# real-stanford/dgdm

Hardware: AMD Instinct MI355X
Metric: guided samples/sec (full DDIM chain) (higher is better)
Workload: dtype f32_split_f16x3; 1 GPU; 3d_guided BASELINE configs[2] (configs[3] at 8 GPUs): B=32 G=45 P=5 R=36000 sub_bs=512 N=512 T=15/S=5, fresh object per pair; contraction_flag=f32, fingers_per_pair=32, denoise_steps=5, rows_per_cond_fn=36000, cond_fn_per_chain_step=1, eps_net_form=f32_f16x3 batched, parallelism=pairs-sharded x1

## Files before the change

dgdm_amd/csrc/debug.hip:

```cpp
#include "common.h"
#include "mfma_chain.h"
#include "models.h"
#include "smallnet.h"

namespace dgdm {
__global__ __launch_bounds__(64, 1) void debug_chain_kernel(const float4 *__restrict__ Wimg, const float *__restrict__ bias,
                                                           const float *__restrict__ X, float *__restrict__ Y) {
    const int lane = threadIdx.x & 63, n = lane & 31, h4 = (lane >> 5) * 4;
    f32x16 in[8], out[8];
#pragma unroll
    for (int o = 0; o < 8; ++o)
#pragma unroll
        for (int q = 0; q < 4; ++q) {
            const float4 v = feat4(X + n * 256, o, q, h4);
            in[o][4 * q + 0] = v.x; in[o][4 * q + 1] = v.y; in[o][4 * q + 2] = v.z; in[o][4 * q + 3] = v.w;
        }
    chain_layer<8, 8, CHAIN_BIAS>(Wimg, bias, in, out, lane);
#pragma unroll
    for (int o = 0; o < 8; ++o)
#pragma unroll
        for (int q = 0; q < 4; ++q) {
            float4 v;
            v.x = out[o][4 * q + 0]; v.y = out[o][4 * q + 1]; v.z = out[o][4 * q + 2]; v.w = out[o][4 * q + 3];
            *reinterpret_cast<float4 *>(Y + n * 256 + 32 * o + 8 * q + h4) = v;
        }
}
}

extern "C" int dgdm_debug_chain_layer(const float *W_host, const float *bias_host, const float *X_dev, float *Y_dev, void *stream) {
    using namespace dgdm;
    std::vector<float> img = pack_chain(W_host, 256, 256);
    DevBuf dw, db;
    int rc;
    if ((rc = dw.upload(img.data(), img.size() * 4)) || (rc = db.upload(bias_host, 256 * 4))) return rc;
    hipLaunchKernelGGL(debug_chain_kernel, dim3(1), dim3(64), 0, (hipStream_t)stream, dw.as<float4>(), db.as<float>(), X_dev, Y_dev);
    DGDM_HIP_CHECK(hipGetLastError());
    DGDM_HIP_CHECK(hipStreamSynchronize((hipStream_t)stream));
    return DGDM_OK;
}

extern "C" int dgdm_debug_pointnet_indices(DgdmDynamics *m, const float *xyz_dev, int N, const int32_t *perm_dev, int perm_len,
                                           int32_t *fps512_dev, int32_t *fps128_dev, int32_t *fps128_flags_dev, int32_t *ball1_dev,
                                           int32_t *ball2_dev, int32_t *ball2_count_dev, int32_t *crowded_dev, void *stream) {
    using namespace dgdm;
    DGDM_REQUIRE(m && xyz_dev && perm_dev && fps512_dev && fps128_dev && fps128_flags_dev && ball1_dev && ball2_dev && ball2_count_dev && crowded_dev,
                 DGDM_EINVAL, "dgdm_debug_pointnet_indices: null argument");
    if (m->kind != 3) { set_error("model type not supported: PointNet++ belongs to the 3-D model"); return DGDM_EMODE; }
    DGDM_REQUIRE(N >= 128 && N <= 1024 && perm_len > 0 && perm_len <= N, DGDM_EINVAL, "dgdm_debug_pointnet_indices: N %d / perm_len %d unsupported", N, perm_len);
    hipStream_t s = (hipStream_t)stream;
    int rc;
    if ((rc = pn_fps_table(xyz_dev, N, N, 512, fps512_dev, nullptr, s))) return rc;
    if ((rc = pn_fps_table(xyz_dev, N, N, 128, fps128_dev, fps128_flags_dev, s))) return rc;
    return pn_debug_indices(xyz_dev, N, m->pn(), perm_dev, perm_len, ball1_dev, ball2_dev, ball2_count_dev, crowded_dev, s);
}

extern "C" int dgdm_farthest_point_sample(const float *xyz_dev, const int64_t *start_host, int B, int N, int npoint, int32_t *out_dev, void *stream) {
    using namespace dgdm;
    DGDM_REQUIRE(xyz_dev && start_host && out_dev && B >= 0 && npoint > 0, DGDM_EINVAL, "dgdm_farthest_point_sample: bad argument");
    DGDM_REQUIRE(N > 0 && N <= 1024, DGDM_EINVAL, "clouds of %d points unsupported (1..1024)", N);
    if (B == 0) return DGDM_OK;
    std::vector<int> st(B);
    for (int i = 0; i < B; ++i) {
        DGDM_REQUIRE(start_host[i] >= 0 && start_host[i] < N, DGDM_EINVAL, "FPS start %lld outside [0, %d)", (long long)start_host[i], N);
        st[i] = (int)start_host[i];
    }
    DevBuf d;
    int rc;
    if ((rc = d.upload(st.data(), sizeof(int) * B))) return rc;
    if ((rc = pn_fps_rows(xyz_dev, d.as<int>(), B, N, npoint, out_dev, (hipStream_t)stream))) return rc;
    DGDM_HIP_CHECK(hipStreamSynchronize((hipStream_t)stream));
    return DGDM_OK;
}

extern "C" int dgdm_query_ball_point(float radius_squared, int nsample, const float *xyz_dev, const float *new_xyz_dev, int B, int N, int S, int32_t *out_dev,
                                     void *stream) {
    using namespace dgdm;
    DGDM_REQUIRE(xyz_dev && new_xyz_dev && out_dev && B >= 0 && N > 0 && S >= 0 && nsample > 0, DGDM_EINVAL, "dgdm_query_ball_point: bad argument");
    if (B == 0 || S == 0) return DGDM_OK;
    return pn_ball_rows(xyz_dev, new_xyz_dev, B, N, S, radius_squared, nsample, out_dev, (hipStream_t)stream);
}

extern "C" int dgdm_square_distance(const float *src_dev, const float *dst_dev, int B, int S, int N, float *out_dev, void *stream) {
    using namespace dgdm;
    DGDM_REQUIRE(src_dev && dst_dev && out_dev && B >= 0 && S >= 0 && N >= 0, DGDM_EINVAL, "dgdm_square_distance: bad argument");
    if (B == 0 || S == 0 || N == 0) return DGDM_OK;
    return pn_sqdist_rows(src_dev, dst_dev, B, S, N, out_dev, (hipStream_t)stream);
}

extern "C" int dgdm_index_points(const float *points_dev, const int32_t *idx_dev, int B, int N, int M, int C, float *out_dev, void *stream) {
    using namespace dgdm;
    DGDM_REQUIRE(points_dev && idx_dev && out_dev && B >= 0 && N > 0 && M >= 0 && C > 0, DGDM_EINVAL, "dgdm_index_points: bad argument");
    if (B == 0 || M == 0) return DGDM_OK;
    return pn_index_rows(points_dev, idx_dev, B, N, M, C, out_dev, (hipStream_t)stream);
}


namespace dgdm {
__global__ void group_max_kernel(const float *__restrict__ x, int64_t G, int ns, int C, float *__restrict__ out) {
    const int64_t e = (int64_t)blockIdx.x * blockDim.x + threadIdx.x;
    if (e >= G * C) return;
    const int64_t g = e / C;
    const int c = (int)(e - g * C);
    const float *p = x + g * ns * C + c;
    float best = p[0];
    for (int n = 1; n < ns; ++n) best = fmaxf(best, p[(int64_t)n * C]);
    out[e] = best;
}
}

extern "C" int dgdm_linear_act(const float *x_dev, int ldx, const float *wt_dev, const float *bias_dev, float *y_dev, int ldy, int rows, int K, int N, int act,
                               void *stream) {
    using namespace dgdm;
    DGDM_REQUIRE(x_dev && wt_dev && y_dev && rows >= 0 && K > 0 && N > 0 && ldx >= K && ldy >= N, DGDM_EINVAL, "dgdm_linear_act: bad argument");
    DGDM_REQUIRE(act == ACT_NONE || act == ACT_RELU || act == ACT_SILU, DGDM_EINVAL, "dgdm_linear_act: activation %d", act);
    return linear(x_dev, ldx, wt_dev, bias_dev, nullptr, 1, y_dev, ldy, rows, K, N, act, false, (hipStream_t)stream);
}

extern "C" int dgdm_group_max(const float *x_dev, int64_t groups, int nsample, int C, float *out_dev, void *stream) {
    using namespace dgdm;
    DGDM_REQUIRE(x_dev && out_dev && groups >= 0 && nsample > 0 && C > 0, DGDM_EINVAL, "dgdm_group_max: bad argument");
    if (groups == 0) return DGDM_OK;
    hipLaunchKernelGGL(group_max_kernel, dim3((unsigned)((groups * C + 255) / 256)), dim3(256), 0, (hipStream_t)stream, x_dev, groups, nsample, C, out_dev);
    DGDM_HIP_CHECK(hipGetLastError());
    return DGDM_OK;
}
```

dgdm_amd/csrc/guidance_api.hip:

```cpp
#include "common.h"
#include "models.h"
#include <algorithm>
#include <cstring>
#include <unordered_map>
#include <atomic>
#include <thread>

using namespace dgdm;

namespace {

std::vector<float> linspace_f32(float start, float end, int steps) {
    std::vector<float> v(steps);
    if (steps == 1) { v[0] = start; return v; }
    const float step = (end - start) / (float)(steps - 1);
    const int half = steps / 2;
    for (int i = 0; i < steps; ++i) v[i] = i < half ? start + step * (float)i : end - step * (float)(steps - i - 1);
    return v;
}

struct ObjectTables {
    const float *xyz = nullptr;
    const int   *fps1 = nullptr;
    const int   *fps2 = nullptr;
    const int   *flags = nullptr;
    DevBuf Z;
    bool   fast_ok = false;
    int *crowded = nullptr, *clist = nullptr;
    DevBuf M0, cl2, cnt2;
    DevBuf cl2s;
    DevBuf cl2o;
    DevBuf pcf;
    DevBuf X, X16;
    bool   has_x = false, has_x16 = false;
    int    ncr = 0;
    DevBuf Z16, M0_16;
    bool   has16 = false;
};

struct PoseGrid {
    DevBuf tab, tiled;
    DevBuf pmax;
    int cells = 0, tiles_per_b = 0;
    int64_t rows = 0;
};

}

struct DgdmGuidance {
    DgdmDynamics *m = nullptr;
    DgdmGuidanceConfig cfg{};
    int B = 0;
    PoseGrid grid, sweep;
    DevBuf objpart;
    DevBuf objtmp;
    std::vector<std::unique_ptr<ObjectTables>> tables;
    bool bf16 = false;
    bool f32_mfma = false;
    static constexpr int NBUILD = 3;
    DevBuf pool_crowded, pool_clist, pool_off, pool_pairs, pool_rank, pool_F1, pool_U;
    DevBuf pool_xyz, pool_fps1, pool_fps2, pool_flags, pool_ncr;
    DevBuf tmpY[NBUILD], tmpL2[NBUILD], vlist;
    hipStream_t bstream[NBUILD] = {}, fstream = nullptr;
    hipEvent_t bev[NBUILD] = {}, bstart = nullptr, fstart = nullptr, fdone = nullptr, ldone = nullptr;
    DevBuf V, genc, atab, chainbias, timepart, ttmp, ttmp64, partial, objdev, objidx, xobj, xobj16, starts, order, xchains, todo, groupoff;
    DevBuf loopx[2], loopeps, loopgrad, loopxrep, loopts;
    DevBuf scorelogits;
    DevBuf sweep_ori, rollstate, rolllogits, rolltiles, rollpmax;
    int rolltiles_chains = 0;
    DevBuf xidx, xidxchains, xtabptrs;
    bool xtab_enabled = true;
    int xtab_policy = 0;
    int grads_since_set = 0;
    static constexpr int XTAB_AFTER = 5;
    int l2_gather_mode = 0;
    int xobj_mode = 0;
    int n_objects = 0;
    bool force_slow_xobj = false;
    void *pinned = nullptr; size_t pinned_bytes = 0; hipEvent_t pinned_ev = nullptr;
    int64_t todo_capacity = 0;
    int *ro_host = nullptr; size_t ro_ints = 0; hipEvent_t ro_ev = nullptr; bool ro_pending = false;
    int finish_objects();
    hipStream_t cstream = nullptr; hipEvent_t up_ready = nullptr, up_consumed = nullptr; bool consumed_recorded = false;
    ~DgdmGuidance() {
        if (pinned) (void)hipHostFree(pinned);
        if (pinned_ev) (void)hipEventDestroy(pinned_ev);
        if (ro_host) (void)hipHostFree(ro_host);
        if (ro_ev) (void)hipEventDestroy(ro_ev);
        if (cstream) (void)hipStreamDestroy(cstream);
        if (up_ready) (void)hipEventDestroy(up_ready);
        if (up_consumed) (void)hipEventDestroy(up_consumed);
        for (int i = 0; i < NBUILD; ++i) {
            if (bstream[i]) (void)hipStreamDestroy(bstream[i]);
            if (bev[i]) (void)hipEventDestroy(bev[i]);
        }
        if (bstart) (void)hipEventDestroy(bstart);
        if (ldone) (void)hipEventDestroy(ldone);
        if (fstart) (void)hipEventDestroy(fstart);
        if (fdone) (void)hipEventDestroy(fdone);
        if (fstream) (void)hipStreamDestroy(fstream);
    }
    int build_pose_table(const std::vector<float> &ori, const std::vector<float> &pos, PoseGrid *dst, hipStream_t s);
    void set_grid(dgdm::TrunkParams *p, const PoseGrid &g, int n_chains) const;
    int check_objects(const int *oidx, int n_chains) const;
    bool tables_wanted() const { return xtab_enabled && !force_slow_xobj && xobj_mode == 0; }
    int common_pre(const float *x_dev, float t_scaled, const int *objidx_host, int n_chains, hipStream_t s);
    int upload_starts(const int64_t *starts_host, int n_chains, int64_t rows, hipStream_t s, bool need_order = true, int n_calls = 1,
                      int64_t call_stride = 0);
    int ensure_rows(int n_chains, int64_t rows_per_chain);
    int use_xtab(const int *objidx_host, int n_chains, int64_t rows, bool want16, hipStream_t s);
    int build_object(int oi, int slot, hipStream_t s);
    int build_xtab(int oi, hipStream_t s);
    int run_xobj(const int *objidx_host, int n_chains, int64_t rows, bool want16, bool *used16, hipStream_t s);
    struct Embedded {
        bool tab = false, used16 = false;
        int64_t rows_per_chain = 0;
        void point(dgdm::TrunkParams *p, const DgdmGuidance &g, int call, int64_t rows_per_call) const;
    };
    int embed_rows(const int *objidx_host, int n_chains, const int64_t *starts_host, int64_t rows_per_call, int n_calls, int64_t call_stride,
                   bool want16, Embedded *e, hipStream_t s);
    int embed(const int *objidx_host, int n_chains, const int64_t *starts_host, int n_calls, int64_t call_stride, Embedded *e, hipStream_t s);
    int trunk_front(int kind, const float *x_dev, int timestep, const int *objidx_host, const int64_t *starts_host, int n_chains, const Embedded *emb,
                    int call, dgdm::TrunkParams *p, hipStream_t s);
};

int DgdmGuidance::build_pose_table(const std::vector<float> &ori, const std::vector<float> &pos, PoseGrid *dst, hipStream_t s) {
    const int n = (int)ori.size(), W1 = m->W1;
    dst->cells = n; dst->tiles_per_b = (n + 31) / 32; dst->rows = (int64_t)B * n;
    DevBuf d_ori, d_pos, d_emb;
    int rc;
    if ((rc = d_ori.upload(ori.data(), sizeof(float) * n))) return rc;
    if ((rc = d_pos.upload(pos.data(), sizeof(float) * 2 * n))) return rc;
    if ((rc = d_emb.alloc(sizeof(float) * 27 * n))) return rc;
    if ((rc = dst->tab.alloc(sizeof(float) * (size_t)W1 * n))) return rc;
    if ((rc = pose_embed(d_ori.as<float>(), d_pos.as<float>(), d_emb.as<float>(), n, s))) return rc;
    if ((rc = linear64(d_emb.as<float>(), nullptr, 27, m->blob64.at(m->off64.w1p_wt), nullptr, nullptr, 1, nullptr, dst->tab.as<float>(), W1, n, 27, W1, ACT_NONE, s))) return rc;
    if ((rc = dst->tiled.alloc(sizeof(float) * (size_t)W1 * dst->tiles_per_b * 32))) return rc;
    if ((rc = tile_table(dst->tab.as<float>(), n, W1, dst->tiled.as<float>(), s))) return rc;
    DGDM_HIP_CHECK(hipStreamSynchronize(s));
    return DGDM_OK;
}

void DgdmGuidance::set_grid(TrunkParams *p, const PoseGrid &g, int n_chains) const {
    p->Atab = atab.as<float>(); p->Ptab = g.tab.as<float>(); p->PtabT = g.tiled.as<float>(); p->Pmax = g.pmax.as<float>();
    p->B = B; p->C = g.cells; p->tiles_per_b = g.tiles_per_b; p->ntiles = n_chains * B * g.tiles_per_b; p->R = g.rows;
    p->xstride = g.rows;
}

int DgdmGuidance::check_objects(const int *oidx, int n_chains) const {
    DGDM_REQUIRE(n_objects > 0, DGDM_EINVAL, "dgdm_guidance_set_objects has not been called");
    for (int i = 0; i < n_chains; ++i)
        DGDM_REQUIRE(oidx[i] >= 0 && oidx[i] < n_objects, DGDM_EINVAL, "chain %d refers to object %d of %d", i, oidx[i], n_objects);
    return DGDM_OK;
}

extern "C" int dgdm_guidance_create(DgdmGuidance **out, DgdmDynamics *model, const DgdmGuidanceConfig *cfg) {
    DGDM_REQUIRE(out && model && cfg, DGDM_EINVAL, "dgdm_guidance_create: null argument");
    DGDM_REQUIRE(cfg->batch > 0 && cfg->grid_size > 0 && cfg->num_pos > 0 && cfg->max_chains > 0 && cfg->num_train_timesteps > 0,
                 DGDM_EINVAL, "dgdm_guidance_create: bad config");
    DGDM_REQUIRE(cfg->max_chains <= DGDM_MAX_CHAINS, DGDM_EINVAL, "max_chains %d > %d", cfg->max_chains, DGDM_MAX_CHAINS);
    if (model->kind == 3) {
        DGDM_REQUIRE(cfg->sub_batch_size > 0, DGDM_EINVAL, "3-D guidance needs sub_batch_size (it partitions the FPS start draws)");
        DGDM_REQUIRE(cfg->num_object_points > 0 && cfg->num_object_points <= 1024, DGDM_EINVAL, "object clouds of %d points unsupported (1..1024)", cfg->num_object_points);
    } else {
        DGDM_REQUIRE(2 * cfg->num_object_points == model->object_ch, DGDM_EINVAL, "2*num_object_points (%d) != object_ch (%d)", 2 * cfg->num_object_points, model->object_ch);
    }
    std::unique_ptr<DgdmGuidance> g(new DgdmGuidance());
    g->m = model; g->cfg = *cfg;
    g->B = cfg->batch;
    const int G = cfg->grid_size, P = cfg->num_pos, C = G * P * P;
    const std::vector<float> lo = linspace_f32(cfg->ori_lo, cfg->ori_hi, G), lp = linspace_f32(-1.f, 1.f, P);
    std::vector<float> ori(C), pos(2 * (size_t)C);
    for (int gi = 0; gi < G; ++gi)
        for (int a = 0; a < P; ++a)
            for (int b = 0; b < P; ++b) {
                const int c = (gi * P + a) * P + b;
                ori[c] = lo[gi]; pos[2 * c] = lp[a]; pos[2 * c + 1] = lp[b];
            }
    int rc;
    if ((rc = g->build_pose_table(ori, pos, &g->grid, nullptr))) return rc;
    {
        std::vector<float> tab((size_t)C * model->W1), mx(C, 0.f);
        DGDM_HIP_CHECK(hipMemcpy(tab.data(), g->grid.tab.p, tab.size() * sizeof(float), hipMemcpyDeviceToHost));
        for (int c = 0; c < C; ++c)
            for (int j = 0; j < model->W1; ++j) mx[c] = std::max(mx[c], std::fabs(tab[(size_t)c * model->W1 + j]));
        if ((rc = g->grid.pmax.upload(mx.data(), mx.size() * sizeof(float)))) return rc;
    }
    std::vector<float> pos0(2 * (size_t)G, 0.f);
    if ((rc = g->build_pose_table(lo, pos0, &g->sweep, nullptr))) return rc;
    if ((rc = g->sweep_ori.upload(lo.data(), lo.size() * sizeof(float)))) return rc;
    const int W1 = model->W1, nc = cfg->max_chains;
    const size_t rows = (size_t)nc * g->B;
    const int64_t R = g->grid.rows;
    if ((rc = g->V.alloc(rows * 256 * 8)) || (rc = g->genc.alloc(rows * 256 * 8)) || (rc = g->atab.alloc(rows * W1 * 4)) ||
        (rc = g->chainbias.alloc((size_t)nc * W1 * 8)) || (rc = g->timepart.alloc((size_t)W1 * 8)) || (rc = g->ttmp.alloc(768 * 4)) ||
        (rc = g->ttmp64.alloc(512 * 8)) ||
        (rc = g->partial.alloc(rows * g->grid.tiles_per_b * W1 * 4)) || (rc = g->objdev.alloc(sizeof(TrunkObjective) * nc)) ||
        (rc = g->objidx.alloc(sizeof(int) * nc)))
        return rc;
    if (model->kind == 2) {
        if ((rc = g->objpart.alloc((size_t)std::max(1, cfg->max_objects) * W1 * 8))) return rc;
    } else {
        if ((rc = g->starts.alloc((size_t)nc * R * 2 * sizeof(int))) ||
            (rc = g->order.alloc((size_t)nc * R * sizeof(int))) || (rc = g->xchains.alloc(sizeof(XobjChain) * nc)) ||
            (rc = g->todo.alloc(((size_t)nc * R + 1) * sizeof(int))))
            return rc;
        g->todo_capacity = (int64_t)nc * R;
        g->pinned_bytes = ((size_t)nc * R * 3 + (size_t)nc * (cfg->num_object_points + 1)) * sizeof(int);
        if ((rc = g->groupoff.alloc((size_t)nc * (cfg->num_object_points + 1) * sizeof(int))) || (rc = g->xidx.alloc((size_t)nc * R * sizeof(int))) ||
            (rc = g->xidxchains.alloc(sizeof(XidxChain) * nc)) || (rc = g->xtabptrs.alloc(sizeof(void *) * nc)))
            return rc;
        DGDM_HIP_CHECK(hipHostMalloc(&g->pinned, g->pinned_bytes, hipHostMallocDefault));
        DGDM_HIP_CHECK(hipEventCreateWithFlags(&g->pinned_ev, hipEventDisableTiming));
    }
    *out = g.release();
    return DGDM_OK;
}

extern "C" void dgdm_guidance_destroy(DgdmGuidance *g) { delete g; }

extern "C" int dgdm_guidance_set_contraction_dtype(DgdmGuidance *g, int dtype) {
    DGDM_REQUIRE(g, DGDM_EINVAL, "dgdm_guidance_set_contraction_dtype: null handle");
    DGDM_REQUIRE(dtype >= DGDM_DTYPE_F32 && dtype <= DGDM_DTYPE_F32_F16X3, DGDM_EINVAL,
                 "contraction dtype %d unsupported (0 = f32 (default form), 1 = bf16, 2 = f32 on the float32 MFMA, 3 = f32 as 3 f16 products = the default form)", dtype);
    g->bf16 = dtype == DGDM_DTYPE_BF16;
    g->f32_mfma = dtype == DGDM_DTYPE_F32_MFMA;
    return DGDM_OK;
}

extern "C" int dgdm_guidance_debug_fps_path(DgdmGuidance *g, int force_per_row, int32_t *out_fast_ok) {
    DGDM_REQUIRE(g, DGDM_EINVAL, "dgdm_guidance_debug_fps_path: null handle");
    g->force_slow_xobj = force_per_row == 1;
    g->xobj_mode = force_per_row == 2 ? 2 : 0;
    g->l2_gather_mode = force_per_row == 4 ? 1 : 0;
    g->xtab_enabled = force_per_row == 0 || force_per_row == 4 || force_per_row == 5;
    g->xtab_policy = force_per_row == 5 ? 1 : 0;
    if (force_per_row == 3) g->xobj_mode = 0;
    if (out_fast_ok) {
        int rc = g->finish_objects();
        if (rc) return rc;
        for (int i = 0; i < g->n_objects && i < (int)g->tables.size(); ++i) out_fast_ok[i] = g->tables[i]->fast_ok ? 1 : 0;
    }
    return DGDM_OK;
}
__global__ void partials_true_units_kernel(float *p, const float *unit, size_t n, int W1) {
    const size_t i = (size_t)blockIdx.x * blockDim.x + threadIdx.x;
    if (i < n) p[i] *= unit[i % W1];
}
extern "C" int dgdm_guidance_debug_partials(DgdmGuidance *g, int n_chains, float *out_dev, int32_t *tiles_per_finger, int32_t *width, void *stream) {
    DGDM_REQUIRE(g && n_chains > 0 && n_chains <= g->cfg.max_chains, DGDM_EINVAL, "dgdm_guidance_debug_partials: bad argument");
    if (tiles_per_finger) *tiles_per_finger = g->grid.tiles_per_b;
    if (width) *width = g->m->W1;
    if (out_dev) {
        const size_t n = (size_t)n_chains * g->B * g->grid.tiles_per_b * g->m->W1;
        DGDM_HIP_CHECK(hipMemcpyAsync(out_dev, g->partial.p, n * sizeof(float), hipMemcpyDeviceToDevice, (hipStream_t)stream));
        hipLaunchKernelGGL(partials_true_units_kernel, dim3((unsigned)((n + 255) / 256)), dim3(256), 0, (hipStream_t)stream, out_dev, g->m->z1_unit.as<float>(), n, g->m->W1);
        DGDM_HIP_CHECK(hipGetLastError());
    }
    return DGDM_OK;
}
extern "C" int64_t dgdm_guidance_rows(const DgdmGuidance *g) { return g ? g->grid.rows : 0; }
extern "C" int64_t dgdm_guidance_starts_per_call(const DgdmGuidance *g) { return (g && g->m->kind == 3) ? 2 * g->grid.rows : 0; }

int DgdmGuidance::build_object(int oi, int slot, hipStream_t s) {
    const int N = cfg.num_object_points;
    ObjectTables &t = *tables[oi];
    const PnWeights w = m->pn();
    int rc;
    if ((rc = t.Z.alloc((size_t)N * N * 256 * 4)) ||
        (rc = t.M0.alloc((size_t)N * 256 * 4)) || (rc = t.cl2.alloc((size_t)N * 128 * sizeof(int))) || (rc = t.cnt2.alloc((size_t)N * sizeof(int))) ||
        (rc = t.cl2s.alloc((size_t)N * 128 * sizeof(int))) || (rc = t.cl2o.alloc((size_t)N * 256 * sizeof(unsigned short))) ||
        (rc = t.pcf.alloc((size_t)N * 512 * sizeof(int))))
        return rc;
    t.has16 = bf16;
    if (bf16 && ((rc = t.Z16.alloc((size_t)N * N * 128 * 4)) || (rc = t.M0_16.alloc((size_t)N * 128 * 4)))) return rc;
    uint32_t *z16 = bf16 ? t.Z16.as<uint32_t>() : nullptr;
    DevBuf &tY = tmpY[slot], &tL2 = tmpL2[slot];
    if ((rc = tY.alloc((size_t)N * N * 256 * 4)) || (rc = tL2.alloc((size_t)N * N * 256 * 4))) return rc;
    const float *xyz = t.xyz;
    const int *off = pool_off.as<int>() + (size_t)oi * (N + 1), *pairs = pool_pairs.as<int>() + (size_t)oi * N * N;
    const short *rank = pool_rank.as<short>() + (size_t)oi * N * N;
    const char *U = static_cast<const char *>(pool_U.p) + (size_t)oi * N * 128 * (bf16 ? 4 : 8);
    if (bf16) {
        if ((rc = pn_pairs(xyz, N, reinterpret_cast<const float *>(U), w, pairs, off, tY.as<float>(), tY.as<uint32_t>(), s))) return rc;
        if ((rc = pn_l2(xyz, N, w, t.fps1, vlist.as<int>(), N, tY.as<float>(), tL2.as<float>(), t.clist, t.clist + N,
                        off, rank, true, s, l2_gather_mode ? 0 : 1))) return rc;
        if ((rc = pn_z16(xyz, N, N, w, tL2.as<uint32_t>(), t.Z.as<float>(), z16, t.clist, t.clist + N, s))) return rc;
    } else {
        const PnWeights64 w64 = m->pn64();
        if ((rc = pn_pairs64(xyz, N, reinterpret_cast<const double *>(U), w64, pairs, off, tY.as<float>(), s))) return rc;
        if ((rc = pn_l2(xyz, N, w, t.fps1, vlist.as<int>(), N, tY.as<float>(), tL2.as<float>(), t.clist, t.clist + N,
                        off, rank, false, s, l2_gather_mode ? 0 : 1))) return rc;
        if ((rc = pn_z64(xyz, N, N, w64, tL2.as<float>(), t.Z.as<float>(), t.clist, t.clist + N, s))) return rc;
    }
    DGDM_HIP_CHECK(hipStreamWaitEvent(s, fdone, 0));
    if ((rc = pn_m0(t.fps2, t.crowded, N, t.Z.as<float>(), t.M0.as<float>(), t.cl2.as<int>(), t.cnt2.as<int>(), z16,
                    bf16 ? t.M0_16.as<uint32_t>() : nullptr, t.clist, t.clist + N, t.cl2s.as<int>(), t.cl2o.as<unsigned short>(), s))) return rc;
    if ((rc = pn_pcf(t.fps1, t.cnt2.as<int>(), t.flags, N, t.pcf.as<int>(), s))) return rc;
    t.has_x = t.has_x16 = false;
    return xtab_policy == 1 ? build_xtab(oi, s) : DGDM_OK;
}

int DgdmGuidance::build_xtab(int oi, hipStream_t s) {
    const int N = cfg.num_object_points;
    ObjectTables &t = *tables[oi];
    if (N < 128) return DGDM_OK;
    const bool b16 = t.has16;
    int rc;
    if (b16) { if ((rc = t.X16.alloc((size_t)N * N * 128 * 4))) return rc; }
    else if ((rc = t.X.alloc((size_t)N * N * 256 * 4))) return rc;
    XtabObj xo{};
    xo.xyz = t.xyz; xo.fps1 = t.fps1; xo.Z = t.Z.as<float>(); xo.M0 = t.M0.as<float>();
    xo.Z16 = b16 ? t.Z16.as<uint32_t>() : nullptr; xo.M0_16 = b16 ? t.M0_16.as<uint32_t>() : nullptr;
    xo.clist = t.clist; xo.ncr = t.clist + N; xo.cl2s = t.cl2s.as<int>(); xo.cnt2 = t.cnt2.as<int>(); xo.flags = t.flags;
    xo.crowded = t.crowded; xo.X = b16 ? nullptr : t.X.as<float>(); xo.X16 = b16 ? t.X16.as<uint32_t>() : nullptr; xo.N = N;
    if ((rc = pn_xtab(xo, b16, s))) return rc;
    (b16 ? t.has_x16 : t.has_x) = true;
    return DGDM_OK;
}

extern "C" int dgdm_guidance_set_objects(DgdmGuidance *g, const float *objects_dev, int n_objects, void *stream) {
    DGDM_REQUIRE(g && objects_dev && n_objects > 0, DGDM_EINVAL, "dgdm_guidance_set_objects: bad argument");
    DGDM_REQUIRE(n_objects <= std::max(1, g->cfg.max_objects), DGDM_EINVAL, "%d objects > max_objects %d", n_objects, g->cfg.max_objects);
    hipStream_t s = (hipStream_t)stream;
    int rc;
    prof_begin(s, DGDM_STAGE_TABLES);
    if (g->m->kind == 2) {
        if ((rc = g->objtmp.alloc((size_t)n_objects * 512 * 8))) return rc;
        if ((rc = g->m->object_part_2d64(objects_dev, g->objtmp.as<double>(), g->objpart.as<double>(), n_objects, s))) return rc;
        prof_end(s, DGDM_STAGE_TABLES, 0.0);
    } else {
        while ((int)g->tables.size() < n_objects) g->tables.emplace_back(new ObjectTables());
        const int N = g->cfg.num_object_points;
        if (g->vlist.bytes < (size_t)N * sizeof(int)) {
            std::vector<int> v(N);
            for (int i = 0; i < N; ++i) v[i] = i;
            if ((rc = g->vlist.upload(v.data(), sizeof(int) * N))) return rc;
        }
        const int nb = std::min<int>(DgdmGuidance::NBUILD, n_objects);
        if (!g->bstart) DGDM_HIP_CHECK(hipEventCreateWithFlags(&g->bstart, hipEventDisableTiming));
        if (!g->ldone) DGDM_HIP_CHECK(hipEventCreateWithFlags(&g->ldone, hipEventDisableTiming));
        for (int i = 0; i < nb; ++i) {
            if (!g->bstream[i]) DGDM_HIP_CHECK(hipStreamCreateWithFlags(&g->bstream[i], hipStreamNonBlocking));
            if (!g->bev[i]) DGDM_HIP_CHECK(hipEventCreateWithFlags(&g->bev[i], hipEventDisableTiming));
        }
        const size_t no = (size_t)n_objects;
        if ((rc = g->pool_xyz.alloc(no * N * 3 * 4)) || (rc = g->pool_fps1.alloc(no * N * 512 * sizeof(int))) ||
            (rc = g->pool_fps2.alloc(no * N * 128 * sizeof(int))) || (rc = g->pool_flags.alloc(no * N * sizeof(int))) ||
            (rc = g->pool_ncr.alloc(no * sizeof(int))) || (rc = g->pool_crowded.alloc(no * N * sizeof(int))) ||
            (rc = g->pool_clist.alloc(no * (N + 1) * sizeof(int))) || (rc = g->pool_off.alloc(no * (N + 1) * sizeof(int))) ||
            (rc = g->pool_pairs.alloc(no * N * N * sizeof(int))) || (rc = g->pool_rank.alloc(no * N * N * sizeof(short))) ||
            (rc = g->pool_F1.alloc(no * N * 128 * 8)) || (rc = g->pool_U.alloc(no * N * 128 * 8)))
            return rc;
        if (!g->fstream) {
            DGDM_HIP_CHECK(hipStreamCreateWithFlags(&g->fstream, hipStreamNonBlocking));
            DGDM_HIP_CHECK(hipEventCreateWithFlags(&g->fstart, hipEventDisableTiming));
            DGDM_HIP_CHECK(hipEventCreateWithFlags(&g->fdone, hipEventDisableTiming));
        }
        DGDM_HIP_CHECK(hipMemcpyAsync(g->pool_xyz.p, objects_dev, no * N * 3 * 4, hipMemcpyDeviceToDevice, s));
        DGDM_HIP_CHECK(hipEventRecord(g->fstart, s));
        DGDM_HIP_CHECK(hipStreamWaitEvent(g->fstream, g->fstart, 0));
        if ((rc = pn_fps_table(g->pool_xyz.as<float>(), N, N, 128, g->pool_fps2.as<int>(), g->pool_flags.as<int>(), g->fstream, n_objects))) return rc;
        DGDM_HIP_CHECK(hipEventRecord(g->fdone, g->fstream));
        if ((rc = pn_fps_table(g->pool_xyz.as<float>(), N, N, 512, g->pool_fps1.as<int>(), nullptr, s, n_objects))) return rc;
        for (int i = 0; i < n_objects; ++i) {
            ObjectTables &t = *g->tables[i];
            t.xyz = g->pool_xyz.as<float>() + (size_t)i * N * 3; t.fps1 = g->pool_fps1.as<int>() + (size_t)i * N * 512;
            t.fps2 = g->pool_fps2.as<int>() + (size_t)i * N * 128; t.flags = g->pool_flags.as<int>() + (size_t)i * N;
            t.crowded = g->pool_crowded.as<int>() + (size_t)i * N; t.clist = g->pool_clist.as<int>() + (size_t)i * (N + 1);
        }
        {
            hipStream_t ls = g->bstream[0];
            DGDM_HIP_CHECK(hipStreamWaitEvent(ls, g->fstart, 0));
            const PnWeights w = g->m->pn();
            if ((rc = pn_crowd(g->pool_xyz.as<float>(), N, w, g->pool_crowded.as<int>(), g->pool_clist.as<int>(), g->pool_clist.as<int>() + N,
                               g->pool_off.as<int>(), g->pool_pairs.as<int>(), g->pool_rank.as<short>(), ls, g->pool_ncr.as<int>(), n_objects)))
                return rc;
            if (g->bf16) {
                if ((rc = pn_sa1(g->pool_xyz.as<float>(), N, w, g->pool_F1.as<float>(), ls, n_objects))) return rc;
                if ((rc = linear(g->pool_F1.as<float>(), 128, w.sa2_wf_t, w.sa2_b0, nullptr, 1, g->pool_U.as<float>(), 128, n_objects * N, 128, 128,
                                 ACT_NONE, false, ls))) return rc;
            } else {
                const PnWeights64 w64 = g->m->pn64();
                if ((rc = pn_sa1_64(g->pool_xyz.as<float>(), N, w.r1sq, w64, g->pool_F1.as<double>(), ls, n_objects))) return rc;
                if ((rc = linear64(nullptr, g->pool_F1.as<double>(), 128, w64.sa2_wf_t, w64.sa2_b0, nullptr, 1, g->pool_U.as<double>(), nullptr, 128,
                                   n_objects * N, 128, 128, ACT_NONE, ls))) return rc;
            }
            DGDM_HIP_CHECK(hipEventRecord(g->ldone, ls));
        }
        DGDM_HIP_CHECK(hipEventRecord(g->bstart, s));
        for (int i = 0; i < nb; ++i) {
            DGDM_HIP_CHECK(hipStreamWaitEvent(g->bstream[i], g->bstart, 0));
            DGDM_HIP_CHECK(hipStreamWaitEvent(g->bstream[i], g->ldone, 0));
        }
        for (int i = 0; i < n_objects; ++i)
            if ((rc = g->build_object(i, i % nb, g->bstream[i % nb]))) return rc;
        for (int i = 0; i < nb; ++i) {
            DGDM_HIP_CHECK(hipEventRecord(g->bev[i], g->bstream[i]));
            DGDM_HIP_CHECK(hipStreamWaitEvent(s, g->bev[i], 0));
        }
        DGDM_HIP_CHECK(hipStreamWaitEvent(s, g->fdone, 0));
        prof_end(s, DGDM_STAGE_TABLES, 0.0);
        const size_t need = no * N + no;
        if (need > g->ro_ints) {
            if (g->ro_host) DGDM_HIP_CHECK(hipHostFree(g->ro_host));
            g->ro_host = nullptr;
            DGDM_HIP_CHECK(hipHostMalloc(reinterpret_cast<void **>(&g->ro_host), need * sizeof(int), hipHostMallocDefault));
            g->ro_ints = need;
        }
        if (!g->ro_ev) DGDM_HIP_CHECK(hipEventCreateWithFlags(&g->ro_ev, hipEventDisableTiming));
        DGDM_HIP_CHECK(hipMemcpyAsync(g->ro_host, g->pool_flags.p, sizeof(int) * no * N, hipMemcpyDeviceToHost, s));
        DGDM_HIP_CHECK(hipMemcpyAsync(g->ro_host + no * N, g->pool_ncr.p, sizeof(int) * no, hipMemcpyDeviceToHost, s));
        DGDM_HIP_CHECK(hipEventRecord(g->ro_ev, s));
        g->ro_pending = true;
    }
    g->n_objects = n_objects;
    g->grads_since_set = 0;
    return DGDM_OK;
}

int DgdmGuidance::common_pre(const float *x_dev, float t_scaled, const int *objidx_host, int n_chains, hipStream_t s) {
    const int rows = n_chains * B, W1 = m->W1;
    int rc;
    if ((rc = m->gripper_forward64(x_dev, m->L, V.as<double>(), genc.as<double>(), rows, s))) return rc;
    if ((rc = m->time_part64(t_scaled, ttmp.as<float>(), ttmp64.as<double>(), timepart.as<double>(), s))) return rc;
    if (m->kind == 2) {
        DGDM_HIP_CHECK(hipMemcpyAsync(objidx.p, objidx_host, sizeof(int) * n_chains, hipMemcpyHostToDevice, s));
        if ((rc = gather_add64(objpart.as<double>(), objidx.as<int>(), timepart.as<double>(), chainbias.as<double>(), n_chains, W1, s))) return rc;
        return linear64(nullptr, genc.as<double>(), 256, m->blob64.at(m->off64.w1c_wt), nullptr, chainbias.as<double>(), B, nullptr, atab.as<float>(), W1, rows, 256, W1,
                        ACT_NONE, s);
    }
    return linear64(nullptr, genc.as<double>(), 256, m->blob64.at(m->off64.w1c_wt), timepart.as<double>(), nullptr, 1, nullptr, atab.as<float>(), W1, rows, 256, W1,
                    ACT_NONE, s);
}

int DgdmGuidance::finish_objects() {
    if (!ro_pending) return DGDM_OK;
    DGDM_HIP_CHECK(hipEventSynchronize(ro_ev));
    const int N = cfg.num_object_points;
    for (int i = 0; i < n_objects; ++i) {
        bool ok = N >= 128;
        for (int k = 0; k < N; ++k) ok = ok && ro_host[(size_t)i * N + k] == 0;
        tables[i]->fast_ok = ok;
        tables[i]->ncr = ro_host[(size_t)n_objects * N + i];
    }
    ro_pending = false;
    return DGDM_OK;
}

int DgdmGuidance::ensure_rows(int n_chains, int64_t rows_per_chain) {
    const int N = cfg.num_object_points;
    const size_t nr = (size_t)n_chains * rows_per_chain;
    int rc;
    if ((rc = starts.alloc(nr * 2 * sizeof(int))) || (rc = order.alloc(nr * sizeof(int))) ||
        (rc = todo.alloc((nr + 1) * sizeof(int))) || (rc = xidx.alloc(nr * sizeof(int))))
        return rc;
    todo_capacity = (int64_t)nr;
    const size_t need = (nr * 3 + (size_t)n_chains * (N + 1)) * sizeof(int);
    if (need > pinned_bytes) {
        if (pinned) { DGDM_HIP_CHECK(hipEventSynchronize(pinned_ev)); DGDM_HIP_CHECK(hipHostFree(pinned)); pinned = nullptr; pinned_bytes = 0; }
        DGDM_HIP_CHECK(hipHostMalloc(&pinned, need, hipHostMallocDefault));
        pinned_bytes = need;
    }
    return DGDM_OK;
}

int DgdmGuidance::upload_starts(const int64_t *starts_host, int n_chains, int64_t rows, hipStream_t s, bool need_order, int n_calls,
                                int64_t call_stride) {
    const int N = cfg.num_object_points;
    const int64_t sb = cfg.sub_batch_size;
    const int64_t rt = rows * n_calls;
    int rc;
    DGDM_REQUIRE(!need_order || rt < ((int64_t)1 << 22), DGDM_EINVAL, "%lld rows per chain in one gather launch (limit 4194303)", (long long)rt);
    if ((rc = ensure_rows(n_chains, rt))) return rc;
    DGDM_HIP_CHECK(hipEventSynchronize(pinned_ev));
    int *dst = static_cast<int *>(pinned);
    int *ord = dst + (size_t)n_chains * 2 * rt;
    int *goff = ord + (size_t)n_chains * rt;
    std::atomic<int> bad{0};
    auto work = [&](int c0, int c1) {
        std::vector<int> cnt(N + 1), cnt2(513), tmp;
        for (int c = c0; c < c1; ++c) {
            int *d = dst + (size_t)c * 2 * rt;
            for (int k = 0; k < n_calls; ++k) {
                const int64_t *src = starts_host + (size_t)k * call_stride + (size_t)c * 2 * rows;
                int *dk = d + 2 * (size_t)k * rows;
                for (int64_t r0 = 0; r0 < rows; r0 += sb) {
                    const int64_t n = std::min(sb, rows - r0);
                    const int64_t *s1 = src + 2 * r0, *s2 = s1 + n;
                    for (int64_t i = 0; i < n; ++i) {
                        const int64_t a = s1[i], b = s2[i];
                        if (!(a >= 0 && a < N && b >= 0 && b < 512)) { bad.store(1); return; }
                        dk[2 * (r0 + i)] = (int)a; dk[2 * (r0 + i) + 1] = (int)b;
                    }
                }
            }
            if (!need_order) continue;
            int *o = ord + (size_t)c * rt;
            tmp.resize((size_t)rt);
            std::fill(cnt2.begin(), cnt2.end(), 0);
            for (int64_t r = 0; r < rt; ++r) ++cnt2[d[2 * r + 1] + 1];
            for (int k = 0; k < 512; ++k) cnt2[k + 1] += cnt2[k];
            for (int64_t r = 0; r < rt; ++r) tmp[cnt2[d[2 * r + 1]]++] = (int)r;
            std::fill(cnt.begin(), cnt.end(), 0);
            for (int64_t r = 0; r < rt; ++r) ++cnt[d[2 * r] + 1];
            for (int k = 0; k < N; ++k) cnt[k + 1] += cnt[k];
            memcpy(goff + (size_t)c * (N + 1), cnt.data(), sizeof(int) * (N + 1));
            for (int64_t i = 0; i < rt; ++i) { const int r = tmp[i]; o[cnt[d[2 * r]]++] = r | (d[2 * r + 1] << 22); }
        }
    };
    const int hw = (int)std::max(2u, std::thread::hardware_concurrency());
    const int nthreads = (int)std::min<int64_t>(std::min(16, hw / 2), std::max<int64_t>(1, std::min<int64_t>(n_chains, (int64_t)n_chains * rt / 65536)));
    if (nthreads <= 1) {
        work(0, n_chains);
    } else {
        std::vector<std::thread> pool;
        for (int t = 0; t < nthreads; ++t) pool.emplace_back(work, (int)((int64_t)n_chains * t / nthreads), (int)((int64_t)n_chains * (t + 1) / nthreads));
        for (auto &th : pool) th.join();
    }
    DGDM_REQUIRE(!bad.load(), DGDM_EINVAL, "FPS start out of range (sa1 must be in [0, %d), sa2 in [0, 512))", N);
    if (!cstream) {
        DGDM_HIP_CHECK(hipStreamCreateWithFlags(&cstream, hipStreamNonBlocking));
        DGDM_HIP_CHECK(hipEventCreateWithFlags(&up_ready, hipEventDisableTiming));
        DGDM_HIP_CHECK(hipEventCreateWithFlags(&up_consumed, hipEventDisableTiming));
    }
    if (consumed_recorded) DGDM_HIP_CHECK(hipStreamWaitEvent(cstream, up_consumed, 0));
    DGDM_HIP_CHECK(hipMemcpyAsync(starts.p, pinned, (size_t)n_chains * rt * 2 * sizeof(int), hipMemcpyHostToDevice, cstream));
    if (need_order) {
        DGDM_HIP_CHECK(hipMemcpyAsync(order.p, ord, (size_t)n_chains * rt * sizeof(int), hipMemcpyHostToDevice, cstream));
        DGDM_HIP_CHECK(hipMemcpyAsync(groupoff.p, goff, (size_t)n_chains * (N + 1) * sizeof(int), hipMemcpyHostToDevice, cstream));
    }
    DGDM_HIP_CHECK(hipEventRecord(pinned_ev, cstream));
    DGDM_HIP_CHECK(hipEventRecord(up_ready, cstream));
    DGDM_HIP_CHECK(hipStreamWaitEvent(s, up_ready, 0));
    return DGDM_OK;
}

int DgdmGuidance::use_xtab(const int *objidx_host, int n_chains, int64_t rows, bool want16, hipStream_t s) {
    std::vector<XidxChain> xc(n_chains);
    std::vector<const void *> base(n_chains);
    for (int i = 0; i < n_chains; ++i) {
        const ObjectTables &t = *tables[objidx_host[i]];
        xc[i].fps1 = t.fps1; xc[i].N = cfg.num_object_points; xc[i].m0_only = t.ncr == 0;
        base[i] = want16 ? (t.ncr == 0 ? (const void *)t.M0_16.p : (const void *)t.X16.p) : (t.ncr == 0 ? (const void *)t.M0.p : (const void *)t.X.p);
    }
    DGDM_HIP_CHECK(hipMemcpyAsync(xidxchains.p, xc.data(), sizeof(XidxChain) * n_chains, hipMemcpyHostToDevice, s));
    DGDM_HIP_CHECK(hipMemcpyAsync(xtabptrs.p, base.data(), sizeof(void *) * n_chains, hipMemcpyHostToDevice, s));
    return pn_xidx(xidxchains.as<XidxChain>(), starts.as<int>(), rows, n_chains, xidx.as<int>(), s);
}

int DgdmGuidance::run_xobj(const int *objidx_host, int n_chains, int64_t rows, bool want16, bool *used16, hipStream_t s) {
    std::vector<XobjChain> ch(n_chains);
    for (int i = 0; i < n_chains; ++i) {
        const ObjectTables &t = *tables[objidx_host[i]];
        ch[i].xyz = t.xyz; ch[i].fps1 = t.fps1; ch[i].slot_of_start = nullptr; ch[i].Z = t.Z.as<float>();
        ch[i].fps2 = t.fps2; ch[i].flags = t.flags; ch[i].crowded = t.crowded; ch[i].N = cfg.num_object_points;
        ch[i].M0 = t.M0.as<float>(); ch[i].cl2 = t.cl2.as<int>(); ch[i].cnt2 = t.cnt2.as<int>();
        ch[i].Z16 = t.has16 ? t.Z16.as<uint32_t>() : nullptr; ch[i].M0_16 = t.has16 ? t.M0_16.as<uint32_t>() : nullptr;
        want16 = want16 && t.has16;
    }
    {
        const size_t nrows = (size_t)n_chains * rows;
        int rc = want16 ? xobj16.alloc(nrows * 512) : xobj.alloc(nrows * 256 * 4);
        if (rc) return rc;
    }
    *used16 = want16;
    XobjParams xp{};
    xp.chains = xchains.as<XobjChain>(); xp.starts = starts.as<int>(); xp.order = order.as<int>(); xp.xobj = xobj.as<float>();
    xp.xobj16 = want16 ? xobj16.as<uint32_t>() : nullptr;
    xp.R = rows; xp.total_rows = rows * n_chains; xp.use_table = force_slow_xobj ? 0 : 1;
    xp.todo = todo.as<int>(); xp.todo_count = todo.as<int>() + todo_capacity; xp.todo_capacity = todo_capacity;
    bool all_fast = true;
    for (int i = 0; i < n_chains; ++i) all_fast = all_fast && tables[objidx_host[i]]->fast_ok;
    bool groups = !force_slow_xobj && xobj_mode == 0 && cfg.num_object_points >= 128;
    for (int i = 0; i < n_chains && groups; ++i) {
        const ObjectTables &t = *tables[objidx_host[i]];
        const int lpr = xobj_rows_lpr(t.ncr, want16);
        groups = lpr > 0 && want16 == t.has16;
        ch[i].clist = t.clist; ch[i].cl2s = t.cl2s.as<int>(); ch[i].cl2o = t.cl2o.as<unsigned short>(); ch[i].pcf = t.pcf.as<int>(); ch[i].ncr = t.ncr; ch[i].lpr = lpr;
    }
    DGDM_HIP_CHECK(hipMemcpyAsync(xchains.p, ch.data(), sizeof(XobjChain) * n_chains, hipMemcpyHostToDevice, s));
    if (groups) {
        xp.group_off = groupoff.as<int>(); xp.nchain = n_chains; xp.group_N = cfg.num_object_points; xp.total_items = n_chains * xp.group_N; xp.use_table = 1;
        std::vector<int> rank(n_chains);
        for (int i = 0; i < n_chains; ++i) rank[i] = i;
        std::stable_sort(rank.begin(), rank.end(), [&](int a, int b) { return ch[a].ncr > ch[b].ncr; });
        for (int i = 0; i < n_chains; ++i) xp.chain_of_rank[i] = (unsigned char)rank[i];
        return pn_xobj_groups(xp, s);
    }
    return pn_xobj(xp, all_fast, s);
}

int DgdmGuidance::embed_rows(const int *oidx, int n_chains, const int64_t *starts_host, int64_t rows_per_call, int n_calls, int64_t call_stride,
                             bool want16, Embedded *e, hipStream_t s) {
    bool tab = tables_wanted();
    for (int i = 0; i < n_chains && tab; ++i) tab = want16 ? tables[oidx[i]]->has_x16 : tables[oidx[i]]->has_x;
    const int64_t rt = rows_per_call * n_calls;
    int rc;
    if ((rc = upload_starts(starts_host, n_chains, rows_per_call, s, !tab, n_calls, call_stride))) return rc;
    if ((rc = finish_objects())) return rc;
    e->tab = tab; e->used16 = want16; e->rows_per_chain = rt;
    if ((rc = tab ? use_xtab(oidx, n_chains, rt, want16, s) : run_xobj(oidx, n_chains, rt, want16, &e->used16, s))) return rc;
    DGDM_HIP_CHECK(hipEventRecord(up_consumed, s));
    consumed_recorded = true;
    return DGDM_OK;
}

void DgdmGuidance::Embedded::point(TrunkParams *p, const DgdmGuidance &g, int call, int64_t rows_per_call) const {
    const size_t row0 = (size_t)call * rows_per_call;
    p->xstride = rows_per_chain;
    if (tab) {
        p->xidx = g.xidx.as<int>() + row0;
        if (used16) p->xtab16 = g.xtabptrs.as<const uint32_t *>();
        else p->xtab = g.xtabptrs.as<const float *>();
    } else {
        p->xobj = g.xobj.as<float>() + row0 * 256;
        p->xobj16 = used16 ? g.xobj16.as<uint32_t>() + row0 * 128 : nullptr;
    }
}

int DgdmGuidance::embed(const int *oidx, int n_chains, const int64_t *starts_host, int n_calls, int64_t call_stride, Embedded *e, hipStream_t s) {
    DGDM_REQUIRE(starts_host, DGDM_EINVAL, "3-D guidance needs the FPS start indices");
    int rc;
    prof_begin(s, DGDM_STAGE_XOBJ);
    if (tables_wanted()) {
        const bool crosses = grads_since_set <= XTAB_AFTER && grads_since_set + n_calls > XTAB_AFTER;
        grads_since_set += n_calls;
        if (crosses)
            for (int i = 0; i < n_objects; ++i) {
                ObjectTables &t = *tables[i];
                if (!(t.has16 ? t.has_x16 : t.has_x) && (rc = build_xtab(i, s))) return rc;
            }
    }
    if ((rc = embed_rows(oidx, n_chains, starts_host, grid.rows, n_calls, call_stride, bf16, e, s))) return rc;
    prof_end(s, DGDM_STAGE_XOBJ, 0.0);
    return DGDM_OK;
}

int DgdmGuidance::trunk_front(int kind, const float *x_dev, int timestep, const int *oidx, const int64_t *starts_host, int n_chains, const Embedded *emb,
                              int call, TrunkParams *pp, hipStream_t s) {
    const float t_scaled = (float)timestep / (float)cfg.num_train_timesteps;
    int rc;
    if ((rc = check_objects(oidx, n_chains))) return rc;
    prof_begin(s, DGDM_STAGE_GUIDE_MISC);
    if ((rc = common_pre(x_dev, t_scaled, oidx, n_chains, s))) return rc;
    prof_end(s, DGDM_STAGE_GUIDE_MISC, 0.0);
    m->fill_trunk(pp);
    set_grid(pp, grid, n_chains);
    if (kind == 3) {
        Embedded own;
        if (!emb) {
            if ((rc = embed(oidx, n_chains, starts_host, 1, 0, &own, s))) return rc;
            emb = &own;
            call = 0;
        }
        emb->point(pp, *this, call, grid.rows);
    }
    return DGDM_OK;
}

static int guidance_grad(DgdmGuidance *g, int kind, const float *x_dev, int timestep, const DgdmObjective *objectives, const float *rowcoef_dev,
                         const int64_t *starts_host, int n_chains, float *grad_dev, hipStream_t s, const DgdmGuidance::Embedded *emb = nullptr,
                         int call = 0) {
    DGDM_REQUIRE(g && x_dev && objectives && grad_dev, DGDM_EINVAL, "guidance_grad: null argument");
    if (g->m->kind != kind) { set_error("model type not supported: %d-D entry point on a %d-D model", kind, g->m->kind); return DGDM_EMODE; }
    DGDM_REQUIRE(n_chains > 0 && n_chains <= g->cfg.max_chains, DGDM_EINVAL, "n_chains %d outside 1..%d", n_chains, g->cfg.max_chains);
    std::vector<int> oidx(n_chains);
    std::vector<TrunkObjective> tob(n_chains);
    for (int i = 0; i < n_chains; ++i) {
        oidx[i] = objectives[i].object;
        for (int j = 0; j < 3; ++j) { tob[i].lin[j] = objectives[i].lin[j]; tob[i].quad[j] = objectives[i].quad[j]; }
        tob[i].use_rowcoef = objectives[i].use_rowcoef; tob[i].pad = 0;
        DGDM_REQUIRE(!tob[i].use_rowcoef || rowcoef_dev, DGDM_EINVAL, "chain %d uses rowcoef but rowcoef_dev is null", i);
    }
    int rc;
    TrunkParams p;
    if ((rc = g->trunk_front(kind, x_dev, timestep, oidx.data(), starts_host, n_chains, emb, call, &p, s))) return rc;
    DGDM_HIP_CHECK(hipMemcpyAsync(g->objdev.p, tob.data(), sizeof(TrunkObjective) * n_chains, hipMemcpyHostToDevice, s));
    p.obj = g->objdev.as<TrunkObjective>(); p.rowcoef = rowcoef_dev;
    p.partial = g->partial.as<float>();
    if (g->bf16) {
        g->m->fill_trunk_bf16(&p);
        if ((rc = trunk_bf16_launch(kind, p, s))) return rc;
    } else if (g->f32_mfma) {
        if ((rc = trunk_launch(kind, false, false, p, s))) return rc;
    } else {
        TrunkF16Scales sc;
        g->m->fill_trunk_f16(&p, &sc);
        if ((rc = trunk_f16l_launch(kind, TrunkF16Mode::Grad, p, sc, s))) return rc;
    }
    prof_begin(s, DGDM_STAGE_GUIDE_MISC);
    rc = dyn_post64(g->m->W1, g->partial.as<float>(), g->grid.tiles_per_b, g->m->blob64.at(g->m->off64.w1c_w), g->m->blob64.at(g->m->off64.g2_w),
                    g->m->blob64.at(g->m->off64.g0_w), g->V.as<double>(), grad_dev, n_chains * g->B, g->m->L, s);
    prof_end(s, DGDM_STAGE_GUIDE_MISC, 0.0);
    return rc;
}

extern "C" int dgdm_dyn2d_guidance_grad(DgdmGuidance *g, const float *x_dev, int timestep, const DgdmObjective *objectives,
                                        const float *rowcoef_dev, int n_chains, float *grad_dev, void *stream) {
    return guidance_grad(g, 2, x_dev, timestep, objectives, rowcoef_dev, nullptr, n_chains, grad_dev, (hipStream_t)stream);
}

extern "C" int dgdm_dyn3d_guidance_grad(DgdmGuidance *g, const float *x_dev, int timestep, const DgdmObjective *objectives,
                                        const float *rowcoef_dev, const int64_t *starts_host, int n_chains, float *grad_dev, void *stream) {
    return guidance_grad(g, 3, x_dev, timestep, objectives, rowcoef_dev, starts_host, n_chains, grad_dev, (hipStream_t)stream);
}

extern "C" int dgdm_guidance_score(DgdmGuidance *g, const float *x_dev, int timestep, const int32_t *object_of_chain, const int64_t *starts_host,
                                   const float thr[3], int n_chains, float *logits_dev, int32_t *counts_dev, float *sums_dev, void *stream) {
    DGDM_REQUIRE(g && x_dev && object_of_chain && thr && counts_dev && sums_dev, DGDM_EINVAL, "dgdm_guidance_score: null argument");
    DGDM_REQUIRE(!g->bf16, DGDM_EINVAL, "dgdm_guidance_score: the bf16 trunk has no forward-only form (contraction dtypes f32 / f32_f16x3 / f32_mfma)");
    hipStream_t s = (hipStream_t)stream;
    const int kind = g->m->kind;
    DGDM_REQUIRE(kind == 2 || starts_host, DGDM_EINVAL, "3-D scoring needs the FPS start indices");
    DGDM_REQUIRE(n_chains > 0 && n_chains <= g->cfg.max_chains, DGDM_EINVAL, "n_chains %d outside 1..%d", n_chains, g->cfg.max_chains);
    int rc;
    if (!logits_dev) {
        if ((rc = g->scorelogits.alloc((size_t)n_chains * g->grid.rows * 3 * sizeof(float)))) return rc;
        logits_dev = g->scorelogits.as<float>();
    }
    const std::vector<int> oidx(object_of_chain, object_of_chain + n_chains);
    TrunkParams p;
    if ((rc = g->trunk_front(kind, x_dev, timestep, oidx.data(), starts_host, n_chains, nullptr, 0, &p, s))) return rc;
    p.logits = logits_dev;
    if (g->f32_mfma) {
        if ((rc = trunk_launch(kind, false, true, p, s))) return rc;
    } else {
        TrunkF16Scales sc;
        g->m->fill_trunk_f16(&p, &sc);
        if ((rc = trunk_f16l_launch(kind, TrunkF16Mode::Forward, p, sc, s))) return rc;
    }
    return score_tally(logits_dev, n_chains, g->B, g->grid.cells, thr, counts_dev, sums_dev, s);
}

namespace {
__global__ void fill_i32_kernel(int *p, int v, int n) {
    const int i = blockIdx.x * blockDim.x + threadIdx.x;
    if (i < n) p[i] = v;
}
__global__ void repeat_rows_kernel(const float *__restrict__ src, float *__restrict__ dst, int64_t n_src, int reps) {
    const int64_t i = (int64_t)blockIdx.x * blockDim.x + threadIdx.x;
    if (i < n_src * reps) dst[i] = src[i % n_src];
}
}

extern "C" int dgdm_guided_chains_run(DgdmUnet1d *unet, DgdmGuidance *g, const float *noise_dev, int n_chains, int n_grad,
                                      const DgdmObjective *objectives, const float *rowcoef_dev, const int64_t *starts_host,
                                      const int32_t *timesteps, const float *coef, const float *scales, int n_steps, float *x_out_dev,
                                      void *stream) {
    DGDM_REQUIRE(unet && g && noise_dev && objectives && timesteps && coef && scales && x_out_dev, DGDM_EINVAL, "dgdm_guided_chains_run: null argument");
    DGDM_REQUIRE(n_chains > 0 && n_grad > 0 && n_chains * n_grad <= g->cfg.max_chains && n_steps > 0, DGDM_EINVAL,
                 "dgdm_guided_chains_run: %d chains x %d gradients outside 1..%d", n_chains, n_grad, g->cfg.max_chains);
    hipStream_t s = (hipStream_t)stream;
    const int B = g->B, L = g->m->L, kind = g->m->kind;
    const size_t per_chain = (size_t)B * L, nx = per_chain * n_chains, ng = nx * n_grad;
    DGDM_REQUIRE(kind == 2 || starts_host, DGDM_EINVAL, "3-D guidance needs the FPS start indices");
    int rc;
    if ((rc = g->loopx[0].alloc(nx * 4)) || (rc = g->loopx[1].alloc(nx * 4)) || (rc = g->loopeps.alloc(nx * 4)) || (rc = g->loopgrad.alloc(ng * 4)) ||
        (rc = g->loopxrep.alloc(ng * 4)) || (rc = g->loopts.alloc((size_t)n_chains * B * sizeof(int))))
        return rc;
    hipLaunchKernelGGL(repeat_rows_kernel, dim3((unsigned)((nx + 255) / 256)), dim3(256), 0, s, noise_dev, g->loopx[0].as<float>(), (int64_t)per_chain, n_chains);
    bool same_scale = true;
    for (int c = 1; c < n_chains; ++c) same_scale = same_scale && scales[c] == scales[0];
    const int64_t spc = kind == 3 ? 2 * g->grid.rows : 0;
    DgdmGuidance::Embedded emb;
    std::vector<int> oidx(n_chains * n_grad);
    const int64_t call_stride = (int64_t)n_chains * n_grad * spc;
    int cpe = kind == 3 ? (int)std::min<int64_t>(n_steps, std::max<int64_t>(1, (((int64_t)1 << 22) - 1) / std::max<int64_t>(1, g->grid.rows))) : n_steps;
    if (const char *e = getenv("DGDM_EMBED_CALLS")) cpe = std::max(1, std::min(cpe, atoi(e)));
    if (kind == 3) {
        for (int i = 0; i < n_chains * n_grad; ++i) oidx[i] = objectives[i].object;
        if ((rc = g->check_objects(oidx.data(), n_chains * n_grad))) return rc;
    }
    for (int si = 0; si < n_steps; ++si) {
        float *x = g->loopx[si & 1].as<float>(), *xn = (si + 1 == n_steps) ? x_out_dev : g->loopx[(si + 1) & 1].as<float>();
        const int t = timesteps[si];
        if (kind == 3 && si % cpe == 0 &&
            (rc = g->embed(oidx.data(), n_chains * n_grad, starts_host + (size_t)si * call_stride, std::min(cpe, n_steps - si), call_stride, &emb, s))) return rc;
        const int nb = (si == 0 && n_chains > 1) ? B : n_chains * B;
        hipLaunchKernelGGL(fill_i32_kernel, dim3((nb + 255) / 256), dim3(256), 0, s, g->loopts.as<int>(), t, nb);
        if ((rc = dgdm_unet1d_forward(unet, x, g->loopts.as<int>(), g->loopeps.as<float>(), nb, L, s))) return rc;
        if (nb != n_chains * B) {
            hipLaunchKernelGGL(repeat_rows_kernel, dim3((unsigned)((nx + 255) / 256)), dim3(256), 0, s, g->loopeps.as<float>(), g->loopgrad.as<float>(), (int64_t)per_chain, n_chains);
            DGDM_HIP_CHECK(hipMemcpyAsync(g->loopeps.p, g->loopgrad.p, nx * 4, hipMemcpyDeviceToDevice, s));
        }
        const float *xg = x;
        if (n_grad > 1) {
            hipLaunchKernelGGL(repeat_rows_kernel, dim3((unsigned)((ng + 255) / 256)), dim3(256), 0, s, x, g->loopxrep.as<float>(), (int64_t)nx, n_grad);
            xg = g->loopxrep.as<float>();
        }
        if ((rc = guidance_grad(g, kind, xg, t, objectives, rowcoef_dev, nullptr, n_chains * n_grad, g->loopgrad.as<float>(), s,
                                kind == 3 ? &emb : nullptr, si % cpe))) return rc;
        const float *cf = coef + 4 * si;
        if (same_scale) {
            if ((rc = dgdm_ddim_guided_step(x, g->loopeps.as<float>(), g->loopgrad.as<float>(), n_grad, xn, (int64_t)nx, cf[0], cf[1], cf[2], cf[3], scales[0], s))) return rc;
        } else {
            DGDM_REQUIRE(n_grad == 1, DGDM_EINVAL, "per-chain guidance scales with averaged gradients are not supported");
            for (int c = 0; c < n_chains; ++c)
                if ((rc = dgdm_ddim_guided_step(x + c * per_chain, g->loopeps.as<float>() + c * per_chain, g->loopgrad.as<float>() + c * per_chain, 1,
                                                xn + c * per_chain, (int64_t)per_chain, cf[0], cf[1], cf[2], cf[3], scales[c], s))) return rc;
        }
    }
    DGDM_HIP_CHECK(hipGetLastError());
    return DGDM_OK;
}

extern "C" int dgdm_guidance_orientation_sweep(DgdmGuidance *g, const float *x_dev, const int32_t *object_of_chain, const int64_t *starts_host,
                                               int n_chains, float *logits_dev, void *stream) {
    DGDM_REQUIRE(g && x_dev && object_of_chain && logits_dev, DGDM_EINVAL, "dgdm_guidance_orientation_sweep: null argument");
    DGDM_REQUIRE(n_chains > 0 && n_chains <= g->cfg.max_chains, DGDM_EINVAL, "n_chains %d outside 1..%d", n_chains, g->cfg.max_chains);
    hipStream_t s = (hipStream_t)stream;
    const int kind = g->m->kind;
    int rc;
    if ((rc = g->check_objects(object_of_chain, n_chains))) return rc;
    if ((rc = g->common_pre(x_dev, 0.f, object_of_chain, n_chains, s))) return rc;
    TrunkParams p;
    g->m->fill_trunk(&p);
    g->set_grid(&p, g->sweep, n_chains);
    if (kind == 3) {
        DGDM_REQUIRE(starts_host, DGDM_EINVAL, "3-D sweep needs the FPS start indices");
        DgdmGuidance::Embedded emb;
        if ((rc = g->embed_rows(object_of_chain, n_chains, starts_host, g->sweep.rows, 1, 0, false, &emb, s))) return rc;
        emb.point(&p, *g, 0, g->sweep.rows);
    }
    p.logits = logits_dev;
    return trunk_launch(kind, false, true, p, s);
}

extern "C" int dgdm_guidance_rollout(DgdmGuidance *g, const float *x_dev, const int32_t *object_of_chain, const int64_t *starts_host,
                                     const double scale[3], int n_interactions, int n_chains, double *final_dev, float *first_logits_dev,
                                     int32_t *left_dev, double *traj_pose_dev, float *traj_logits_dev, void *stream) {
    DGDM_REQUIRE(g && x_dev && object_of_chain && scale && final_dev && first_logits_dev && left_dev, DGDM_EINVAL, "dgdm_guidance_rollout: null argument");
    DGDM_REQUIRE(!g->bf16, DGDM_EINVAL, "dgdm_guidance_rollout: the bf16 trunk has no forward-only form (contraction dtypes f32 / f32_f16x3)");
    DGDM_REQUIRE(!g->f32_mfma, DGDM_EINVAL, "dgdm_guidance_rollout: the float32 MFMA trunk has no per-row pose form (contraction dtypes f32 / f32_f16x3)");
    DGDM_REQUIRE(n_interactions >= 1, DGDM_EINVAL, "dgdm_guidance_rollout: %d interactions (at least 1)", n_interactions);
    DGDM_REQUIRE(n_chains > 0 && n_chains <= g->cfg.max_chains, DGDM_EINVAL, "n_chains %d outside 1..%d", n_chains, g->cfg.max_chains);
    int rc;
    if ((rc = g->check_objects(object_of_chain, n_chains))) return rc;
    hipStream_t s = (hipStream_t)stream;
    const int kind = g->m->kind, K = n_interactions, W1 = g->m->W1, G = g->sweep.cells;
    DGDM_REQUIRE(kind == 2 || starts_host, DGDM_EINVAL, "3-D roll-out needs the FPS start indices");
    const int64_t Rs = g->sweep.rows, rows = (int64_t)n_chains * Rs;
    const int ntiles = n_chains * g->B * g->sweep.tiles_per_b;
    if ((rc = g->rollstate.alloc((size_t)rows * 3 * sizeof(double))) || (rc = g->rolltiles.alloc((size_t)ntiles * 32 * W1 * sizeof(float))) ||
        (kind == 3 && (rc = g->rollpmax.alloc((size_t)ntiles * 32 * sizeof(float)))) ||
        (!traj_logits_dev && (rc = g->rolllogits.alloc((size_t)rows * 3 * sizeof(float)))))
        return rc;
    if ((rc = g->common_pre(x_dev, 0.f, object_of_chain, n_chains, s))) return rc;
    TrunkParams p;
    g->m->fill_trunk(&p);
    DgdmGuidance::Embedded emb;
    if (kind == 3 && (rc = g->embed_rows(object_of_chain, n_chains, starts_host, Rs, K, (int64_t)n_chains * 2 * Rs, false, &emb, s))) return rc;
    TrunkF16Scales sc;
    g->m->fill_trunk_f16(&p, &sc);
    g->set_grid(&p, g->sweep, n_chains);
    p.Ptab = nullptr; p.PtabT = g->rolltiles.as<float>(); p.Pmax = kind == 3 ? g->rollpmax.as<float>() : nullptr;
    double *state = g->rollstate.as<double>();
    if ((rc = rollout_start(g->sweep_ori.as<float>(), n_chains, g->B, G, state, left_dev, traj_pose_dev, s))) return rc;
    g->rolltiles_chains = n_chains;
    for (int k = 0; k < K; ++k) {
        if ((rc = rollout_pose_table(state, g->m->blob64.at(g->m->off64.w1p_wt), W1, n_chains, g->B, G, g->rolltiles.as<float>(), p.Pmax ? g->rollpmax.as<float>() : nullptr, s)))
            return rc;
        p.logits = traj_logits_dev ? traj_logits_dev + (size_t)k * rows * 3 : g->rolllogits.as<float>();
        if (kind == 3) emb.point(&p, *g, k, Rs);
        if ((rc = trunk_f16l_launch(kind, TrunkF16Mode::ForwardRowPose, p, sc, s))) return rc;
        if ((rc = rollout_update(p.logits, scale, k, rows, state, left_dev, traj_pose_dev ? traj_pose_dev + (size_t)(k + 1) * rows * 3 : nullptr,
                                 k == K - 1 ? final_dev : nullptr, k == 0 ? first_logits_dev : nullptr, s)))
            return rc;
    }
    return DGDM_OK;
}

extern "C" int dgdm_guidance_debug_rollout_table(DgdmGuidance *g, int n_chains, float *rollout_tiles_dev, float *sweep_tiles_dev,
                                                 int32_t *tiles_per_finger, int32_t *width, void *stream) {
    DGDM_REQUIRE(g && n_chains > 0 && n_chains <= g->cfg.max_chains, DGDM_EINVAL, "dgdm_guidance_debug_rollout_table: bad argument");
    if (tiles_per_finger) *tiles_per_finger = g->sweep.tiles_per_b;
    if (width) *width = g->m->W1;
    const size_t per_tile = (size_t)g->m->W1 * 32 * sizeof(float);
    if (rollout_tiles_dev) {
        DGDM_REQUIRE(n_chains <= g->rolltiles_chains, DGDM_EINVAL, "dgdm_guidance_debug_rollout_table: the last roll-out had %d chains", g->rolltiles_chains);
        DGDM_HIP_CHECK(hipMemcpyAsync(rollout_tiles_dev, g->rolltiles.p, (size_t)n_chains * g->B * g->sweep.tiles_per_b * per_tile, hipMemcpyDeviceToDevice, (hipStream_t)stream));
    }
    if (sweep_tiles_dev)
        DGDM_HIP_CHECK(hipMemcpyAsync(sweep_tiles_dev, g->sweep.tiled.p, (size_t)g->sweep.tiles_per_b * per_tile, hipMemcpyDeviceToDevice, (hipStream_t)stream));
    return DGDM_OK;
}

namespace {

struct CloudGroup { std::vector<int> rows; };

int pointnet_rows(DgdmDynamics *m, const float *xyz_dev , const int64_t *s1, const int64_t *s2, float *emb_dev, int rows,
                  int N, hipStream_t s) {
    DGDM_REQUIRE(N > 0 && N <= 1024, DGDM_EINVAL, "clouds of %d points unsupported (1..1024)", N);
    std::vector<float> host((size_t)rows * 3 * N);
    DGDM_HIP_CHECK(hipMemcpyAsync(host.data(), xyz_dev, host.size() * 4, hipMemcpyDeviceToHost, s));
    DGDM_HIP_CHECK(hipStreamSynchronize(s));
    std::unordered_map<std::string, int> seen;
    std::vector<CloudGroup> groups;
    std::vector<int> rep;
    for (int r = 0; r < rows; ++r) {
        std::string key(reinterpret_cast<const char *>(host.data() + (size_t)r * 3 * N), (size_t)3 * N * 4);
        auto it = seen.find(key);
        int gid;
        if (it == seen.end()) {
            gid = (int)groups.size();
            seen.emplace(std::move(key), gid);
            groups.emplace_back();
            rep.push_back(r);
        } else {
            gid = it->second;
        }
        groups[gid].rows.push_back(r);
    }
    const PnWeights w = m->pn();
    DevBuf xyz, fps1, F1, U, Y, L2, Z, vlist, slotmap, starts, chains, out, crowded, clist, poff, pairs, prank;
    int rc;
    const PnWeights64 w64 = m->pn64();
    if ((rc = xyz.alloc((size_t)N * 12)) || (rc = fps1.alloc((size_t)N * 512 * 4)) || (rc = F1.alloc((size_t)N * 128 * 8)) || (rc = U.alloc((size_t)N * 128 * 8)) ||
        (rc = Y.alloc((size_t)N * N * 1024)) || (rc = chains.alloc(sizeof(XobjChain))) || (rc = crowded.alloc((size_t)N * 4)) ||
        (rc = clist.alloc((size_t)(N + 1) * 4)) || (rc = poff.alloc((size_t)(N + 1) * 4)) || (rc = pairs.alloc((size_t)N * N * 4)) ||
        (rc = prank.alloc((size_t)N * N * 2)))
        return rc;
    for (size_t gi = 0; gi < groups.size(); ++gi) {
        const std::vector<int> &rws = groups[gi].rows;
        std::vector<float> pts((size_t)N * 3);
        const float *src = host.data() + (size_t)rep[gi] * 3 * N;
        for (int i = 0; i < N; ++i) { pts[3 * i] = src[i]; pts[3 * i + 1] = src[N + i]; pts[3 * i + 2] = src[2 * N + i]; }
        std::vector<int> slot_of(N, -1), vl, st(2 * rws.size());
        for (size_t k = 0; k < rws.size(); ++k) {
            const int64_t a = s1[rws[k]], b = s2[rws[k]];
            DGDM_REQUIRE(a >= 0 && a < N && b >= 0 && b < 512, DGDM_EINVAL, "FPS start out of range");
            if (slot_of[a] < 0) { slot_of[a] = (int)vl.size(); vl.push_back((int)a); }
            st[2 * k] = (int)a; st[2 * k + 1] = (int)b;
        }
        const int nv = (int)vl.size();
        if ((rc = xyz.upload(pts.data(), pts.size() * 4)) || (rc = vlist.upload(vl.data(), vl.size() * 4)) ||
            (rc = slotmap.upload(slot_of.data(), slot_of.size() * 4)) || (rc = starts.upload(st.data(), st.size() * 4)) ||
            (rc = L2.alloc((size_t)nv * N * 1024)) || (rc = Z.alloc((size_t)nv * N * 1024)) || (rc = out.alloc(rws.size() * 1024)))
            return rc;
        const float *x = xyz.as<float>();
        if ((rc = pn_fps_table(x, N, N, 512, fps1.as<int>(), nullptr, s))) return rc;
        if ((rc = pn_sa1_64(x, N, w.r1sq, w64, F1.as<double>(), s))) return rc;
        if ((rc = linear64(nullptr, F1.as<double>(), 128, w64.sa2_wf_t, w64.sa2_b0, nullptr, 1, U.as<double>(), nullptr, 128, N, 128, 128, ACT_NONE, s))) return rc;
        if ((rc = pn_crowd(x, N, w, crowded.as<int>(), clist.as<int>(), clist.as<int>() + N, poff.as<int>(), pairs.as<int>(), prank.as<short>(), s))) return rc;
        if ((rc = pn_pairs64(x, N, U.as<double>(), w64, pairs.as<int>(), poff.as<int>(), Y.as<float>(), s))) return rc;
        if ((rc = pn_l2(x, N, w, fps1.as<int>(), vlist.as<int>(), nv, Y.as<float>(), L2.as<float>(), clist.as<int>(), clist.as<int>() + N,
                        poff.as<int>(), prank.as<short>(), false, s))) return rc;
        if ((rc = pn_z64(x, N, nv, w64, L2.as<float>(), Z.as<float>(), clist.as<int>(), clist.as<int>() + N, s))) return rc;
        XobjChain ch{};
        ch.xyz = x; ch.fps1 = fps1.as<int>(); ch.slot_of_start = slotmap.as<int>(); ch.Z = Z.as<float>(); ch.fps2 = nullptr; ch.flags = nullptr; ch.crowded = crowded.as<int>(); ch.N = N;
        DGDM_HIP_CHECK(hipMemcpyAsync(chains.p, &ch, sizeof ch, hipMemcpyHostToDevice, s));
        XobjParams xp{};
        xp.chains = chains.as<XobjChain>(); xp.starts = starts.as<int>(); xp.xobj = out.as<float>(); xp.R = (int64_t)rws.size(); xp.total_rows = xp.R;
        if ((rc = pn_xobj(xp, false, s))) return rc;
        bool contiguous = true;
        for (size_t k = 1; k < rws.size(); ++k) contiguous = contiguous && rws[k] == rws[k - 1] + 1;
        if (contiguous) {
            DGDM_HIP_CHECK(hipMemcpyAsync(emb_dev + (size_t)rws[0] * 256, out.p, rws.size() * 1024, hipMemcpyDeviceToDevice, s));
        } else {
            for (size_t k = 0; k < rws.size(); ++k)
                DGDM_HIP_CHECK(hipMemcpyAsync(emb_dev + (size_t)rws[k] * 256, out.as<float>() + k * 256, 1024, hipMemcpyDeviceToDevice, s));
        }
        DGDM_HIP_CHECK(hipStreamSynchronize(s));
    }
    return DGDM_OK;
}

}

extern "C" int dgdm_pointnet2_forward(DgdmDynamics *m, const float *xyz_dev, const int64_t *start_sa1_host, const int64_t *start_sa2_host,
                                      float *emb_dev, int rows, int N, void *stream) {
    DGDM_REQUIRE(m && xyz_dev && start_sa1_host && start_sa2_host && emb_dev && rows >= 0, DGDM_EINVAL, "dgdm_pointnet2_forward: bad argument");
    if (m->kind != 3) { set_error("model type not supported: PointNet++ belongs to the 3-D model"); return DGDM_EMODE; }
    if (rows == 0) return DGDM_OK;
    return pointnet_rows(m, xyz_dev, start_sa1_host, start_sa2_host, emb_dev, rows, N, (hipStream_t)stream);
}

extern "C" int dgdm_dyn3d_forward(DgdmDynamics *m, const float *x_ctrl, const float *x_ori, const float *x_pos, const float *t,
                                  const float *xyz, const int64_t *start_sa1_host, const int64_t *start_sa2_host, float *logits, int rows,
                                  int N, void *stream) {
    DGDM_REQUIRE(m && x_ctrl && x_ori && x_pos && t && xyz && start_sa1_host && start_sa2_host && logits && rows >= 0, DGDM_EINVAL,
                 "dgdm_dyn3d_forward: bad argument");
    if (m->kind != 3) { set_error("model type not supported: dgdm_dyn3d_forward on a 2-D model"); return DGDM_EMODE; }
    if (rows == 0) return DGDM_OK;
    hipStream_t s = (hipStream_t)stream;
    int rc;
    const size_t need = (size_t)rows * (256 + 256 + 32 + 768 + 512 + 256) * sizeof(float);
    if ((rc = m->ws.alloc(need))) return rc;
    float *V = m->ws.as<float>(), *genc = V + (size_t)rows * 256, *pose = genc + (size_t)rows * 256, *tmp = pose + (size_t)rows * 32,
          *z1 = tmp + (size_t)rows * 768, *xo = z1 + (size_t)rows * 512;
    if ((rc = pointnet_rows(m, xyz, start_sa1_host, start_sa2_host, xo, rows, N, s))) return rc;
    if ((rc = m->time_part(t, 0.f, tmp, z1, rows, s))) return rc;
    if ((rc = m->gripper_forward(x_ctrl + m->L, 3 * m->L, V, genc, rows, s))) return rc;
    if ((rc = linear(genc, 256, m->blob.at(m->off.w1c_wt), nullptr, nullptr, 1, z1, 512, rows, 256, 512, ACT_NONE, true, s))) return rc;
    if ((rc = pose_embed(x_ori, x_pos, pose, rows, s))) return rc;
    if ((rc = linear(pose, 27, m->blob.at(m->off.w1p_wt), nullptr, nullptr, 1, z1, 512, rows, 27, 512, ACT_NONE, true, s))) return rc;
    TrunkParams p;
    m->fill_trunk(&p);
    p.Atab = z1; p.xobj = xo; p.logits = logits; p.C = rows; p.R = rows; p.xstride = rows; p.B = 1; p.tiles_per_b = 1; p.ntiles = (rows + 31) / 32;
    return trunk_launch(3, true, true, p, s);
}
```

dgdm_amd/csrc/pointnet.h:

```cpp
#pragma once
#include "common.h"

namespace dgdm {

struct PnWeights {
    float r1sq, r2sq;
    const float *sa1_w0t;
    const float *sa1_b0;
    const float *sa1_w1;
    const float *sa1_b1;
    const float *sa2_wf_t;
    const float *sa2_b0;
    const float *sa2_vx;
    const float4 *sa2_w1_img;
    const float *sa2_b1;
    const float4 *sa3_w_img16;
    const float *sa3_wx;
    const float *sa3_b;
};

struct PnWeights64 {
    const double *sa1_w0t, *sa1_b0, *sa1_w1, *sa1_b1;
    const double *sa2_wf_t, *sa2_b0, *sa2_vx;
    const double *sa2_w1_img, *sa2_b1;
    const double *sa3_w_img, *sa3_wx, *sa3_b;
};

struct XobjChain {
    const float *xyz;
    const int   *fps1;
    const int   *slot_of_start;
    const float *Z;
    const uint32_t *Z16, *M0_16;
    const int   *fps2;
    const int   *flags;
    const int   *crowded;
    const float *M0;
    const int   *cl2;
    const int   *cnt2;
    int          N;
    const int   *clist;
    const int   *cl2s;
    const unsigned short *cl2o;
    int          ncr;
    const int   *pcf;
    int          lpr;
};

struct XobjParams {
    const XobjChain *chains;
    const int       *starts;
    const int       *order;
    float           *xobj;
    uint32_t        *xobj16;
    int64_t          R, total_rows;
    int              use_table;
    int              skip_fast;
    int             *todo;
    int             *todo_count;
    int64_t          todo_capacity;
    const int       *group_off;
    int              nchain, total_items;
    int              group_N;
    unsigned char    chain_of_rank[DGDM_MAX_CHAINS];
};

struct XtabObj {
    const float *xyz; const int *fps1;
    const float *Z, *M0; const uint32_t *Z16, *M0_16;
    const int *clist, *ncr;
    const int *cl2s, *cnt2, *flags, *crowded;
    float *X; uint32_t *X16;
    int N;
};
int pn_xtab(const XtabObj &o, bool bf16, hipStream_t s);
struct XidxChain { const int *fps1; int N; int m0_only; };
int pn_xidx(const XidxChain *chains_dev, const int *starts, int64_t R, int nchain, int *idx, hipStream_t s);

int pn_fps_rows(const float *xyz, const int *start, int B, int N, int npoint, int *out, hipStream_t s);
int pn_ball_rows(const float *xyz, const float *centres, int B, int N, int S, float r2, int nsample, int *out, hipStream_t s);
int pn_sqdist_rows(const float *src, const float *dst, int B, int S, int N, float *out, hipStream_t s);
int pn_index_rows(const float *points, const int *idx, int B, int N, int M, int C, float *out, hipStream_t s);

int pn_fps_table(const float *xyz, int N, int nv, int npoint, int *out, int *flags, hipStream_t s, int nobj = 1);
int pn_sa1(const float *xyz, int N, const PnWeights &w, float *F1, hipStream_t s, int nobj = 1);
int pn_crowd(const float *xyz, int N, const PnWeights &w, int *crowded, int *clist, int *ncr, int *off, int *pairs, short *rank, hipStream_t s,
             int *ncr_copy = nullptr, int nobj = 1);
int pn_pairs(const float *xyz, int N, const float *U, const PnWeights &w, const int *pairs, const int *off, float *Y, uint32_t *Y16, hipStream_t s);
int pn_l2(const float *xyz, int N, const PnWeights &w, const int *fps1, const int *vlist, int nv, const float *Y, float *L2,
          const int *clist, const int *ncr, const int *off, const short *rank, bool bf16 , hipStream_t s,
          int crowded_mode = 0);
int pn_z16(const float *xyz, int N, int nv, const PnWeights &w, const uint32_t *L2_16, float *Z, uint32_t *Z16, const int *clist, const int *ncr,
           hipStream_t s);
int pn_sa1_64(const float *xyz, int N, float r1sq, const PnWeights64 &w, double *F1_64, hipStream_t s, int nobj = 1);
int pn_pairs64(const float *xyz, int N, const double *U64, const PnWeights64 &w, const int *pairs, const int *off, float *Y, hipStream_t s);
int pn_z64(const float *xyz, int N, int nv, const PnWeights64 &w, const float *L2, float *Z, const int *clist, const int *ncr, hipStream_t s);
int pn_m0(const int *fps2, const int *crowded, int N, const float *Z0, float *M0, int *cl2, int *cnt2, const uint32_t *Z0_16, uint32_t *M0_16,
          const int *clist, const int *ncr, int *cl2s, unsigned short *cl2o, hipStream_t s);
__host__ __device__ inline int xobj_rows_lpr(int ncr, bool bf16) {
    for (int lpr = bf16 ? 32 : 64; lpr >= 8; lpr >>= 1)
        if (ncr * lpr * 16 <= 65536) return lpr;
    return 0;
}
int pn_xobj_groups(const XobjParams &p, hipStream_t s);
int pn_pcf(const int *fps1, const int *cnt2, const int *flags, int N, int *pcf, hipStream_t s);
int pn_debug_indices(const float *xyz, int N, const PnWeights &w, const int *perm, int M, int *ball1, int *ball2, int *ball2_cnt, int *crowded,
                     hipStream_t s);
int pn_xobj(const XobjParams &p, bool all_fast, hipStream_t s);

}
```

dgdm_amd/csrc/pointnet.hip:

```cpp
#include "common.h"
#include "mfma_chain.h"
#include <type_traits>
#include "pointnet.h"
#include "pointnet_dev.h"

#pragma clang fp contract(off)

namespace dgdm {

template <class T, class Op>
__device__ __forceinline__ T dpp_reduce(T v, Op op) {
    auto step = [&](auto ctrl, auto rmask) {
        constexpr int C = decltype(ctrl)::value, M = decltype(rmask)::value;
        const int o = __builtin_amdgcn_update_dpp(__builtin_bit_cast(int, v), __builtin_bit_cast(int, v), C, M, 0xf, false);
        v = op(v, __builtin_bit_cast(T, o));
    };
    step(std::integral_constant<int, 0xB1>{}, std::integral_constant<int, 0xf>{});
    step(std::integral_constant<int, 0x4E>{}, std::integral_constant<int, 0xf>{});
    step(std::integral_constant<int, 0x141>{}, std::integral_constant<int, 0xf>{});
    step(std::integral_constant<int, 0x140>{}, std::integral_constant<int, 0xf>{});
    step(std::integral_constant<int, 0x142>{}, std::integral_constant<int, 0xa>{});
    step(std::integral_constant<int, 0x143>{}, std::integral_constant<int, 0xc>{});
    return __builtin_bit_cast(T, __builtin_amdgcn_readlane(__builtin_bit_cast(int, v), 63));
}

__device__ __forceinline__ void wave_argmax(float &v, int &i) {
    const float m = dpp_reduce(v, [](float a, float b) { return fmaxf(a, b); });
    const unsigned cand = (v == m) ? (unsigned)i : 0xffffffffu;
    i = (int)dpp_reduce(cand, [](unsigned a, unsigned b) { return a < b ? a : b; });
    v = m;
}

template <int PPL, bool TIES>
__device__ bool fps_wave(const float *lx, const float *ly, const float *lz, int M, int start, int npoint, int *out, int lane) {
    float px[PPL], py[PPL], pz[PPL], dist[PPL];
#pragma unroll
    for (int i = 0; i < PPL; ++i) {
        const int j = lane + 64 * i;
        const bool ok = j < M;
        px[i] = ok ? lx[j] : 0.f; py[i] = ok ? ly[j] : 0.f; pz[i] = ok ? lz[j] : 0.f;
        dist[i] = ok ? 1e10f : -1.f;
    }
    int far = start;
    bool ambiguous = false;
    for (int it = 0; it < npoint; ++it) {
        if (lane == 0) out[it] = far;
        const float cx = lx[far], cy = ly[far], cz = lz[far];
        float bv = -2.f;
        int bi = 0;
#pragma unroll
        for (int i = 0; i < PPL; ++i) {
            const float d = sq3(px[i] - cx, py[i] - cy, pz[i] - cz);
            if (d < dist[i]) dist[i] = d;
            if (dist[i] > bv) { bv = dist[i]; bi = lane + 64 * i; }
        }
        wave_argmax(bv, bi);
        far = bi;
        if (TIES && it + 1 < npoint) {
            const float wx = lx[far], wy = ly[far], wz = lz[far];
            bool t = bv == 0.f;
#pragma unroll
            for (int i = 0; i < PPL; ++i) t = t || (dist[i] == bv && (px[i] != wx || py[i] != wy || pz[i] != wz));
            ambiguous = ambiguous || t;
        }
    }
    return TIES ? (__ballot(ambiguous) != 0ull) : false;
}

__global__ __launch_bounds__(256) void fps_table_kernel(const float *__restrict__ xyz, int N, int nv, int npoint, int *__restrict__ out,
                                                        int *__restrict__ flags) {
    extern __shared__ float lds[];
    float *lx = lds, *ly = lds + N, *lz = lds + 2 * N;
    xyz += (size_t)blockIdx.y * N * 3;
    out += (size_t)blockIdx.y * nv * npoint;
    if (flags) flags += (size_t)blockIdx.y * nv;
    for (int i = threadIdx.x; i < N; i += blockDim.x) { lx[i] = xyz[3 * i]; ly[i] = xyz[3 * i + 1]; lz[i] = xyz[3 * i + 2]; }
    __syncthreads();
    const int v = blockIdx.x * 4 + (threadIdx.x >> 6), lane = threadIdx.x & 63;
    if (v >= nv) return;
    bool amb;
    if (flags) {
        amb = N <= 512 ? fps_wave<8, true>(lx, ly, lz, N, v, npoint, out + (size_t)v * npoint, lane)
                       : fps_wave<16, true>(lx, ly, lz, N, v, npoint, out + (size_t)v * npoint, lane);
        if (lane == 0) flags[v] = amb ? 1 : 0;
    } else {
        if (N <= 512) fps_wave<8, false>(lx, ly, lz, N, v, npoint, out + (size_t)v * npoint, lane);
        else fps_wave<16, false>(lx, ly, lz, N, v, npoint, out + (size_t)v * npoint, lane);
    }
}

__global__ __launch_bounds__(128) void sa1_kernel(const float *xyz, int N, float r2, const float *__restrict__ w0t ,
                                                  const float *__restrict__ b0, const float *__restrict__ w1 ,
                                                  const float *__restrict__ b1, float *F1 ) {
    __shared__ int nbr[32];
    __shared__ __attribute__((aligned(16))) float h1[32][64];
    const int t = threadIdx.x, lane = t & 63;
    xyz += (size_t)blockIdx.y * 3 * N; F1 += (size_t)blockIdx.y * N * 128;
    float wrow[64];
#pragma unroll
    for (int k = 0; k < 64; ++k) wrow[k] = w1[t * 64 + k];
    const float bias1 = b1[t];
    for (int p = blockIdx.x; p < N; p += gridDim.x) {
        const float cx = xyz[3 * p], cy = xyz[3 * p + 1], cz = xyz[3 * p + 2];
        const float cn = sq3(cx, cy, cz);
        if (t < 64) ball_first32(xyz, N, p, cx, cy, cz, cn, r2, nbr, lane);
        __syncthreads();
        for (int i = t; i < 32 * 64; i += 128) {
            const int s = i >> 6, c = i & 63, k = nbr[s];
            const float dx = xyz[3 * k] - cx, dy = xyz[3 * k + 1] - cy, dz = xyz[3 * k + 2] - cz;
            const float v = fmaf(w0t[128 + c], dz, fmaf(w0t[64 + c], dy, fmaf(w0t[c], dx, 0.f))) + b0[c];
            h1[s][c] = fmaxf(v, 0.f);
        }
        __syncthreads();
        float best = 0.f;
        for (int s = 0; s < 32; ++s) {
            float acc = 0.f;
#pragma unroll
            for (int k = 0; k < 64; k += 4) {
                const float4 h = *reinterpret_cast<const float4 *>(&h1[s][k]);
                acc = fmaf(wrow[k + 3], h.w, fmaf(wrow[k + 2], h.z, fmaf(wrow[k + 1], h.y, fmaf(wrow[k], h.x, acc))));
            }
            best = fmaxf(best, fmaxf(acc + bias1, 0.f));
        }
        F1[(size_t)p * 128 + t] = best;
        __syncthreads();
    }
}

__global__ __launch_bounds__(256, 1) void pair_kernel(const float *__restrict__ xyz, int N, const float *__restrict__ U ,
                                                      const float *__restrict__ vx , const float4 *__restrict__ Wimg,
                                                      const float *__restrict__ bias, const int *__restrict__ pairs,
                                                      const int *__restrict__ off , float *__restrict__ Y, uint32_t *__restrict__ Y16) {
    const int lane = threadIdx.x & 63, n = lane & 31, h4 = (lane >> 5) * 4;
    const int wave = __builtin_amdgcn_readfirstlane(threadIdx.x >> 6);
    const int total = off[N];
    const int tile = blockIdx.x * 4 + wave;
    if (tile * 32 >= total) return;
    const int p = min(tile * 32 + n, total - 1);
    const int ck = pairs[p], c = ck >> 16, k = ck & 0xffff;
    const float dx = xyz[3 * k] - xyz[3 * c], dy = xyz[3 * k + 1] - xyz[3 * c + 1], dz = xyz[3 * k + 2] - xyz[3 * c + 2];
    f32x16 in[4], out[8];
    const float *urow = U + (size_t)k * 128;
#pragma unroll
    for (int o = 0; o < 4; ++o) {
#pragma unroll
        for (int q = 0; q < 4; ++q) {
            const float4 u = feat4(urow, o, q, h4);
            const float4 a = feat4(vx, o, q, h4), b = feat4(vx + 128, o, q, h4), d = feat4(vx + 256, o, q, h4);
            in[o][4 * q + 0] = fmaxf(fmaf(d.x, dz, fmaf(b.x, dy, fmaf(a.x, dx, u.x))), 0.f);
            in[o][4 * q + 1] = fmaxf(fmaf(d.y, dz, fmaf(b.y, dy, fmaf(a.y, dx, u.y))), 0.f);
            in[o][4 * q + 2] = fmaxf(fmaf(d.z, dz, fmaf(b.z, dy, fmaf(a.z, dx, u.z))), 0.f);
            in[o][4 * q + 3] = fmaxf(fmaf(d.w, dz, fmaf(b.w, dy, fmaf(a.w, dx, u.w))), 0.f);
        }
    }
    chain_layer<4, 8, CHAIN_BIAS>(Wimg, bias, in, out, lane);
    if (Y16) {
        if (tile * 32 + n < total) {
            uint4 *d16 = reinterpret_cast<uint4 *>(Y16 + (size_t)p * 128) + (h4 >> 1);
#pragma unroll
            for (int o = 0; o < 8; ++o) {
                uint32_t pk[8];
#pragma unroll
                for (int d = 0; d < 8; ++d) pk[d] = pack_bf16(fmaxf(out[o][2 * d], 0.f), fmaxf(out[o][2 * d + 1], 0.f));
                d16[4 * o] = make_uint4(pk[0], pk[1], pk[2], pk[3]);
                d16[4 * o + 1] = make_uint4(pk[4], pk[5], pk[6], pk[7]);
            }
        }
        return;
    }
    if (tile * 32 + n < total) {
        float *dst = Y + (size_t)p * 256;
#pragma unroll
        for (int o = 0; o < 8; ++o) {
#pragma unroll
            for (int q = 0; q < 4; ++q) {
                float4 v;
                v.x = fmaxf(out[o][4 * q + 0], 0.f); v.y = fmaxf(out[o][4 * q + 1], 0.f);
                v.z = fmaxf(out[o][4 * q + 2], 0.f); v.w = fmaxf(out[o][4 * q + 3], 0.f);
                *reinterpret_cast<float4 *>(dst + 32 * o + 8 * q + h4) = v;
            }
        }
    }
}

__global__ __launch_bounds__(1024) void crowd_kernel(const float *xyz, int N, float r2, int *crowded,
                                                     int *clist, int *ncr, int *off ,
                                                     int *ncr_copy ) {
    __shared__ int wcount[16], wsum[16];
    const int c = threadIdx.x, lane = c & 63, wave = c >> 6;
    const size_t ob = blockIdx.y;
    xyz += ob * 3 * N; crowded += ob * N; clist += ob * (N + 1); ncr += ob * (N + 1); off += ob * (N + 1);
    if (ncr_copy) ncr_copy += ob;
    bool cr = false;
    int cnt = 0;
    if (c < N) {
        const float cx = xyz[3 * c], cy = xyz[3 * c + 1], cz = xyz[3 * c + 2];
        const float cn = sq3(cx, cy, cz);
        for (int k = 0; k < N; ++k) {
            const float x = xyz[3 * k], y = xyz[3 * k + 1], z = xyz[3 * k + 2];
            cnt += !(sqdist_expanded(cx, cy, cz, cn, x, y, z, sq3(x, y, z)) > r2);
        }
        cr = cnt > 64;
        crowded[c] = cr ? 1 : 0;
    }
    const unsigned long long m = __ballot(cr);
    int incl = cnt;
#pragma unroll
    for (int d = 1; d < 64; d <<= 1) {
        const int t = __shfl_up(incl, d);
        if (lane >= d) incl += t;
    }
    if (lane == 63) wsum[wave] = incl;
    if (lane == 0) wcount[wave] = __popcll(m);
    __syncthreads();
    int base = 0, sbase = 0;
    for (int w = 0; w < wave; ++w) { base += wcount[w]; sbase += wsum[w]; }
    if (cr) clist[base + __popcll(m & ((1ull << lane) - 1ull))] = c;
    if (c < N) off[c] = sbase + incl - cnt;
    if (c == 0) {
        int tot = 0, stot = 0;
        for (int w = 0; w < 16; ++w) { tot += wcount[w]; stot += wsum[w]; }
        *ncr = tot;
        if (ncr_copy) *ncr_copy = tot;
        off[N] = stot;
    }
}

__global__ __launch_bounds__(256) void nbr_fill_kernel(const float *xyz, int N, float r2, const int *off,
                                                       int *pairs, short *rank ) {
    const int lane = threadIdx.x & 63, c = blockIdx.x * 4 + (threadIdx.x >> 6);
    if (c >= N) return;
    const size_t ob = blockIdx.y;
    xyz += ob * 3 * N; off += ob * (N + 1); pairs += ob * N * N; rank += ob * N * N;
    const float cx = xyz[3 * c], cy = xyz[3 * c + 1], cz = xyz[3 * c + 2];
    const float cn = sq3(cx, cy, cz);
    const int o = off[c];
    int seen = 0;
    for (int k0 = 0; k0 < N; k0 += 64) {
        const int k = k0 + lane;
        bool in = false;
        if (k < N) {
            const float x = xyz[3 * k], y = xyz[3 * k + 1], z = xyz[3 * k + 2];
            in = !(sqdist_expanded(cx, cy, cz, cn, x, y, z, sq3(x, y, z)) > r2);
        }
        const unsigned long long m = __ballot(in);
        const int r = seen + __popcll(m & ((1ull << lane) - 1ull));
        if (k < N) rank[(size_t)c * N + k] = in ? (short)r : (short)-1;
        if (in) pairs[o + r] = (c << 16) | k;
        seen += __popcll(m);
    }
}

__device__ __forceinline__ int l2_select(const short *rks, const int *__restrict__ perm, int M, int *sel, int lane) {
    int cnt = 0;
    for (int base = 0; base < M && cnt < 64; base += 64) {
        const int j = base + lane;
        const int r = j < M ? rks[perm[j]] : -1;
        const bool in = r >= 0;
        const unsigned long long m = __ballot(in);
        const int pos = cnt + __popcll(m & ((1ull << lane) - 1ull));
        if (in && pos < 64) sel[pos] = r;
        cnt += __popcll(m);
    }
    __builtin_amdgcn_wave_barrier();
    return min(cnt, 64);
}

template <bool BF16>
__global__ __launch_bounds__(256) void l2_kernel(const float *__restrict__ xyz, int N, float r2, const int *__restrict__ fps1 ,
                                                 const int *__restrict__ vlist, int nv, const float *__restrict__ Y,
                                                 float *__restrict__ L2 , int mode, const int *__restrict__ clist,
                                                 const int *__restrict__ ncr, const int *__restrict__ off, const short *__restrict__ rank) {
    __shared__ int sel[4][64];
    __shared__ short rks[4][1024];
    const int lane = threadIdx.x & 63, wave = threadIdx.x >> 6;
    int c, slot;
    if (mode == 0) {
        c = blockIdx.y * 4 + wave;
        slot = 0;
        if (c >= N) return;
    } else {
        const int nvg = (nv - 1 + 3) / 4;
        const int xcd = blockIdx.x & 7, j = blockIdx.x >> 3;
        const int ci = (j / nvg) * 8 + xcd;
        if (ci >= *ncr) return;
        c = clist[ci];
        slot = 1 + (j % nvg) * 4 + wave;
        if (slot >= nv) return;
    }
    const int *perm = fps1 + (size_t)vlist[slot] * 512;
    const short *rk = rank + (size_t)c * N;
    for (int i = lane; i < N; i += 64) rks[wave][i] = rk[i];
    __builtin_amdgcn_wave_barrier();
    const int cnt = l2_select(rks[wave], perm, 512, sel[wave], lane);
    if (BF16) {
        const uint2 *slab = reinterpret_cast<const uint2 *>(reinterpret_cast<const uint32_t *>(Y) + (size_t)off[c] * 128) + lane;
        uint2 best = make_uint2(0u, 0u);
        int i = 0;
        for (; i + 8 <= cnt; i += 8) {
            uint2 v[8];
#pragma unroll
            for (int k = 0; k < 8; ++k) v[k] = slab[(size_t)sel[wave][i + k] * 64];
#pragma unroll
            for (int k = 0; k < 8; ++k) { best.x = pkmax_u16(best.x, v[k].x); best.y = pkmax_u16(best.y, v[k].y); }
        }
        for (; i < cnt; ++i) {
            const uint2 a = slab[(size_t)sel[wave][i] * 64];
            best.x = pkmax_u16(best.x, a.x); best.y = pkmax_u16(best.y, a.y);
        }
        reinterpret_cast<uint2 *>(reinterpret_cast<uint32_t *>(L2) + ((size_t)slot * N + c) * 128)[lane] = best;
        return;
    }
    const float *slab = Y + (size_t)off[c] * 256 + lane * 4;
    float4 best = make_float4(0.f, 0.f, 0.f, 0.f);
    int i = 0;
    for (; i + 8 <= cnt; i += 8) {
        float4 v[8];
#pragma unroll
        for (int k = 0; k < 8; ++k) v[k] = *reinterpret_cast<const float4 *>(slab + (size_t)sel[wave][i + k] * 256);
#pragma unroll
        for (int k = 0; k < 8; ++k) {
            best.x = fmaxf(best.x, v[k].x); best.y = fmaxf(best.y, v[k].y); best.z = fmaxf(best.z, v[k].z); best.w = fmaxf(best.w, v[k].w);
        }
    }
    for (; i < cnt; ++i) {
        const float4 a = *reinterpret_cast<const float4 *>(slab + (size_t)sel[wave][i] * 256);
        best.x = fmaxf(best.x, a.x); best.y = fmaxf(best.y, a.y); best.z = fmaxf(best.z, a.z); best.w = fmaxf(best.w, a.w);
    }
    *reinterpret_cast<float4 *>(L2 + ((size_t)slot * N + c) * 256 + lane * 4) = best;
}

constexpr int L2C_YBYTES = 120 * 1024, L2C_THREADS = 1024;

template <bool BF16, int LPR>
__device__ __forceinline__ void l2c_reduce(const uint32_t *ych, const unsigned char *selv, int cnt, uint32_t *dst, int lane) {
    typedef uint32_t u4 __attribute__((ext_vector_type(4)));
    constexpr int RPW = 64 / LPR;
    const int sg = lane / LPR, fl = lane % LPR;
    u4 best = {0u, 0u, 0u, 0u};
    auto vmax4 = [](u4 a, u4 b) {
        u4 o;
        if (BF16) { o.x = pkmax_u16(a.x, b.x); o.y = pkmax_u16(a.y, b.y); o.z = pkmax_u16(a.z, b.z); o.w = pkmax_u16(a.w, b.w); }
        else {
            o.x = __float_as_uint(fmaxf(__uint_as_float(a.x), __uint_as_float(b.x))); o.y = __float_as_uint(fmaxf(__uint_as_float(a.y), __uint_as_float(b.y)));
            o.z = __float_as_uint(fmaxf(__uint_as_float(a.z), __uint_as_float(b.z))); o.w = __float_as_uint(fmaxf(__uint_as_float(a.w), __uint_as_float(b.w)));
        }
        return o;
    };
    for (int j = 0; j < cnt; j += 4 * RPW) {
        const uint32_t four = *reinterpret_cast<const uint32_t *>(selv + min(j + 4 * sg, 60));
        u4 v[4];
#pragma unroll
        for (int e = 0; e < 4; ++e) v[e] = *reinterpret_cast<const u4 *>(ych + ((size_t)((four >> (8 * e)) & 255u) * LPR + fl) * 4);
        if (BF16) {
#pragma unroll
            for (int e = 0; e < 4; ++e) best = vmax4(best, v[e]);
        } else {
#pragma unroll
            for (int e = 0; e < 4; e += 2) {
                best.x = max(max(best.x, v[e].x), v[e + 1].x); best.y = max(max(best.y, v[e].y), v[e + 1].y);
                best.z = max(max(best.z, v[e].z), v[e + 1].z); best.w = max(max(best.w, v[e].w), v[e + 1].w);
            }
        }
    }
    if (RPW > 1) {
#pragma unroll
        for (int o = 32; o >= LPR; o >>= 1) {
            u4 t;
            t.x = __shfl_xor(best.x, o); t.y = __shfl_xor(best.y, o); t.z = __shfl_xor(best.z, o); t.w = __shfl_xor(best.w, o);
            best = vmax4(best, t);
        }
    }
    if (sg == 0) *reinterpret_cast<u4 *>(dst + fl * 4) = best;
}

template <bool BF16>
__device__ __forceinline__ void l2c_centre(int c, int N, const int *__restrict__ fps1 , int nv, const uint32_t *__restrict__ Y,
                                           uint32_t *__restrict__ L2 , const int *__restrict__ off, const short *__restrict__ rank,
                                           int (*selw)[64]) {
    constexpr int W = BF16 ? 128 : 256;
    extern __shared__ uint32_t l2c_lds[];
    short *rks = reinterpret_cast<short *>(l2c_lds);
    unsigned char *sel = reinterpret_cast<unsigned char *>(l2c_lds + 512);
    unsigned char *cnts = sel + 512 * 64;
    uint32_t *ych = l2c_lds + 512 + 512 * 16 + 128;
    const int K = off[c + 1] - off[c];
    const int lane = threadIdx.x & 63, wave = threadIdx.x >> 6, nwave = L2C_THREADS / 64;
    const int vlo = 1 + (int)(((int64_t)(nv - 1) * blockIdx.y) / gridDim.y), vhi = 1 + (int)(((int64_t)(nv - 1) * (blockIdx.y + 1)) / gridDim.y);
    for (int i = threadIdx.x; i < N; i += L2C_THREADS) rks[i] = rank[(size_t)c * N + i];
    __syncthreads();
    if (K > 255) {
        constexpr int D = W / 64;
        for (int v = vlo + wave; v < vhi; v += nwave) {
            const int cnt = l2_select(rks, fps1 + (size_t)v * 512, 512, selw[wave], lane);
            uint32_t best[D];
#pragma unroll
            for (int d = 0; d < D; ++d) best[d] = 0u;
            for (int i = 0; i < cnt; ++i) {
                const uint32_t *row = Y + ((size_t)off[c] + selw[wave][i]) * W + lane * D;
#pragma unroll
                for (int d = 0; d < D; ++d)
                    best[d] = BF16 ? pkmax_u16(best[d], row[d]) : __float_as_uint(fmaxf(__uint_as_float(best[d]), __uint_as_float(row[d])));
            }
            uint32_t *dst = L2 + ((size_t)v * N + c) * W + lane * D;
#pragma unroll
            for (int d = 0; d < D; ++d) dst[d] = best[d];
            __builtin_amdgcn_wave_barrier();
        }
        return;
    }
    {
        int pv[8], pn[8];
        const int v0 = vlo + wave;
#pragma unroll
        for (int i = 0; i < 8; ++i) pn[i] = v0 < vhi ? fps1[(size_t)v0 * 512 + 64 * i + lane] : 0;
        for (int v = v0; v < vhi; v += nwave) {
#pragma unroll
            for (int i = 0; i < 8; ++i) pv[i] = pn[i];
            const int vn = v + nwave;
            if (vn < vhi) {
#pragma unroll
                for (int i = 0; i < 8; ++i) pn[i] = fps1[(size_t)vn * 512 + 64 * i + lane];
            }
            int cnt = 0;
#pragma unroll
            for (int i = 0; i < 8; ++i) {
                if (cnt >= 64) break;
                const int r = rks[pv[i]];
                const bool in = r >= 0;
                const unsigned long long m = __ballot(in);
                const int pos = cnt + __popcll(m & ((1ull << lane) - 1ull));
                if (in && pos < 64) selw[wave][pos] = r;
                cnt += __popcll(m);
            }
            cnt = min(cnt, 64);
            __builtin_amdgcn_wave_barrier();
            sel[(size_t)v * 64 + lane] = (unsigned char)selw[wave][lane < cnt ? lane : max(cnt - 1, 0)];
            if (lane == 0) cnts[v] = (unsigned char)cnt;
            __builtin_amdgcn_wave_barrier();
        }
    }
    int lpr = W / 4;
    while ((size_t)K * lpr * 16 > (size_t)L2C_YBYTES) lpr >>= 1;
    const uint32_t *Yc = Y + (size_t)off[c] * W;
    for (int f0 = 0; f0 < W; f0 += 4 * lpr) {
        __syncthreads();
        const int pieces = K * lpr;
        for (int i = threadIdx.x; i < pieces; i += L2C_THREADS)
            *reinterpret_cast<uint4 *>(ych + (size_t)i * 4) = *reinterpret_cast<const uint4 *>(Yc + (size_t)(i / lpr) * W + f0 + (i % lpr) * 4);
        __syncthreads();
        for (int v = vlo + wave; v < vhi; v += nwave) {
            uint32_t *dst = L2 + ((size_t)v * N + c) * W + f0;
            const unsigned char *sv = sel + (size_t)v * 64;
            const int cnt = cnts[v];
            switch (lpr) {
                case 64: if (!BF16) l2c_reduce<BF16, (BF16 ? 32 : 64)>(ych, sv, cnt, dst, lane); break;
                case 32: l2c_reduce<BF16, 32>(ych, sv, cnt, dst, lane); break;
                case 16: l2c_reduce<BF16, 16>(ych, sv, cnt, dst, lane); break;
                default: l2c_reduce<BF16, 8>(ych, sv, cnt, dst, lane); break;
            }
        }
    }
}

template <bool BF16>
__global__ __launch_bounds__(L2C_THREADS, 1) void l2c_kernel(int N, const int *__restrict__ fps1 , int nv, const uint32_t *__restrict__ Y,
                                                             uint32_t *__restrict__ L2 , const int *__restrict__ clist,
                                                             const int *__restrict__ ncr, const int *__restrict__ off,
                                                             const short *__restrict__ rank) {
    __shared__ int selw[L2C_THREADS / 64][64];
    const int n = *ncr;
    for (int ci = blockIdx.x; ci < n; ci += gridDim.x) {
        l2c_centre<BF16>(clist[ci], N, fps1, nv, Y, L2, off, rank, selw);
        __syncthreads();
    }
}

typedef __bf16 zbf16x8 __attribute__((ext_vector_type(8)));
__global__ __launch_bounds__(256, 1) void z16_kernel(const float *__restrict__ xyz, int N, int nv, const uint32_t *__restrict__ L2_16,
                                                     const float4 *__restrict__ Wimg16, const float *__restrict__ w3x ,
                                                     const float *__restrict__ bias, float *__restrict__ Z, uint32_t *__restrict__ Z16,
                                                     int mode, const int *__restrict__ clist, const int *__restrict__ ncr) {
    const int lane = threadIdx.x & 63, n = lane & 31, h4 = (lane >> 5) * 4;
    const int wave = __builtin_amdgcn_readfirstlane(threadIdx.x >> 6);
    const int64_t tile0 = ((int64_t)blockIdx.x * 4 + wave) * 2;
    const int ncrv = mode ? *ncr : N;
    const int64_t items = mode ? (int64_t)(nv - 1) * ncrv : N;
    if (tile0 * 32 >= items) return;
    int64_t row[2];
    float cx[2], cy[2], cz[2];
    bool live[2];
    typedef uint32_t u4 __attribute__((ext_vector_type(4)));
    u4 in[2][8][2];
#pragma unroll
    for (int t = 0; t < 2; ++t) {
        const int64_t idx = (tile0 + t) * 32 + n;
        live[t] = idx < items;
        const int64_t item = min(idx, items - 1);
        const int c = mode ? clist[item % ncrv] : (int)item;
        row[t] = mode ? (1 + item / ncrv) * N + c : c;
        cx[t] = xyz[3 * c]; cy[t] = xyz[3 * c + 1]; cz[t] = xyz[3 * c + 2];
        const u4 *src = reinterpret_cast<const u4 *>(L2_16 + (size_t)row[t] * 128) + (h4 >> 1);
#pragma unroll
        for (int o = 0; o < 8; ++o) { in[t][o][0] = src[4 * o]; in[t][o][1] = src[4 * o + 1]; }
    }
    const wrsrc_t rs = weight_rsrc(Wimg16, 128 * 1024);
    float4 ring[CONT_DEPTH];
    ring_fill(rs, lane * 16, 0, ring);
#pragma unroll
    for (int o = 0; o < 8; ++o) {
        f32x16 acc[2];
#pragma unroll
        for (int q = 0; q < 4; ++q) {
            const float4 b = feat4(bias, o, q, h4);
            const float4 a0 = feat4(w3x, o, q, h4), a1 = feat4(w3x + 256, o, q, h4), a2 = feat4(w3x + 512, o, q, h4);
#pragma unroll
            for (int t = 0; t < 2; ++t) {
                acc[t][4 * q + 0] = fmaf(a2.x, cz[t], fmaf(a1.x, cy[t], fmaf(a0.x, cx[t], b.x)));
                acc[t][4 * q + 1] = fmaf(a2.y, cz[t], fmaf(a1.y, cy[t], fmaf(a0.y, cx[t], b.y)));
                acc[t][4 * q + 2] = fmaf(a2.z, cz[t], fmaf(a1.z, cy[t], fmaf(a0.z, cx[t], b.z)));
                acc[t][4 * q + 3] = fmaf(a2.w, cz[t], fmaf(a1.w, cy[t], fmaf(a0.w, cx[t], b.w)));
            }
        }
#pragma unroll
        for (int i = 0; i < 16; ++i) {
            const int e = o * 16 + i;
            const float4 a = ring[e % CONT_DEPTH];
            ring[e % CONT_DEPTH] = wload(rs, lane * 16, (e + CONT_DEPTH) * 1024);
            const zbf16x8 av = __builtin_bit_cast(zbf16x8, a);
            acc[0] = __builtin_amdgcn_mfma_f32_32x32x16_bf16(av, __builtin_bit_cast(zbf16x8, in[0][i / 2][i % 2]), acc[0], 0, 0, 0);
            acc[1] = __builtin_amdgcn_mfma_f32_32x32x16_bf16(av, __builtin_bit_cast(zbf16x8, in[1][i / 2][i % 2]), acc[1], 0, 0, 0);
            __builtin_amdgcn_sched_barrier(0);
            asm volatile("" ::: "memory");
        }
#pragma unroll
        for (int t = 0; t < 2; ++t) {
            if (!live[t]) continue;
            float *dst = Z + (size_t)row[t] * 256;
            uint32_t pk[8];
#pragma unroll
            for (int q = 0; q < 4; ++q) {
                float4 v;
                v.x = fmaxf(acc[t][4 * q + 0], 0.f); v.y = fmaxf(acc[t][4 * q + 1], 0.f);
                v.z = fmaxf(acc[t][4 * q + 2], 0.f); v.w = fmaxf(acc[t][4 * q + 3], 0.f);
                *reinterpret_cast<float4 *>(dst + 32 * o + 8 * q + h4) = v;
                pk[2 * q] = pack_bf16(v.x, v.y); pk[2 * q + 1] = pack_bf16(v.z, v.w);
            }
            uint4 *d16 = reinterpret_cast<uint4 *>(Z16 + (size_t)row[t] * 128) + (h4 >> 1);
            d16[4 * o] = make_uint4(pk[0], pk[1], pk[2], pk[3]);
            d16[4 * o + 1] = make_uint4(pk[4], pk[5], pk[6], pk[7]);
        }
    }
}

__global__ __launch_bounds__(256) void m0_kernel(const int *__restrict__ fps2 , const int *__restrict__ crowded, int N,
                                                 const float *__restrict__ Z0 , float *__restrict__ M0, int *__restrict__ cl2,
                                                 int *__restrict__ cnt2, const uint32_t *__restrict__ Z0_16, uint32_t *__restrict__ M0_16,
                                                 const int *__restrict__ clist, const int *__restrict__ ncr, int *__restrict__ cl2s,
                                                 unsigned short *__restrict__ cl2o, int bf16) {
    __shared__ short slot_of[1024];
    for (int i = threadIdx.x; i < *ncr; i += blockDim.x) slot_of[clist[i]] = (short)i;
    __syncthreads();
    const int lane = threadIdx.x & 63, q = blockIdx.x * 4 + (threadIdx.x >> 6);
    if (q >= N) return;
    const int idA = fps2[(size_t)q * 128 + lane], idB = fps2[(size_t)q * 128 + 64 + lane];
    const bool crA = crowded[idA] != 0, crB = crowded[idB] != 0;
    const unsigned long long mA = __ballot(crA), mB = __ballot(crB);
    const int nA = __popcll(mA), cnt = nA + __popcll(mB);
    int *dst = cl2 + (size_t)q * 128;
    const unsigned long long below = (1ull << lane) - 1ull;
    if (crA) dst[__popcll(mA & below)] = idA;
    if (crB) dst[nA + __popcll(mB & below)] = idB;
    int last = 0;
    if (cnt > 0) last = mB ? __shfl(idB, 63 - __clzll(mB)) : __shfl(idA, 63 - __clzll(mA));
    for (int j = cnt + lane; j < 128; j += 64) dst[j] = last;
    if (lane == 0) cnt2[q] = cnt;
    {
        int *ds = cl2s + (size_t)q * 128;
        if (crA) ds[__popcll(mA & below)] = slot_of[idA];
        if (crB) ds[nA + __popcll(mB & below)] = slot_of[idB];
        const int ls = cnt > 0 ? slot_of[last] : 0;
        for (int j = cnt + lane; j < 128; j += 64) ds[j] = ls;
        const int sc = xobj_rows_lpr(*ncr, bf16 != 0) * 16;
        const int sA = crA ? slot_of[idA] : 0, sB = crB ? slot_of[idB] : 0;
        const unsigned long long mAe = __ballot(crA && !(sA & 1)), mAo = __ballot(crA && (sA & 1)), mBe = __ballot(crB && !(sB & 1)), mBo = __ballot(crB && (sB & 1));
        const int ne = __popcll(mAe) + __popcll(mBe), no = cnt - ne;
        unsigned short *dz = cl2o + (size_t)q * 256;
        if (crA) {
            const int pe = (sA & 1) ? ne + __popcll(mAo & below) : __popcll(mAe & below);
            dz[pe] = (unsigned short)(sA * sc);
            dz[128 + ((sA & 1) ? pe - ne : no + pe)] = (unsigned short)(sA * sc);
        }
        if (crB) {
            const int pe = (sB & 1) ? ne + __popcll(mAo) + __popcll(mBo & below) : __popcll(mAe) + __popcll(mBe & below);
            dz[pe] = (unsigned short)(sB * sc);
            dz[128 + ((sB & 1) ? pe - ne : no + pe)] = (unsigned short)(sB * sc);
        }
        for (int j = cnt + lane; j < 128; j += 64) { dz[j] = (unsigned short)(ls * sc); dz[128 + j] = (unsigned short)(ls * sc); }
    }
    __shared__ int nlist[4][136];
    int *nl = nlist[threadIdx.x >> 6];
    const int nnA = 64 - nA, nn = 128 - cnt;
    if (!crA) nl[__popcll(~mA & below)] = idA;
    if (!crB) nl[nnA + __popcll(~mB & below)] = idB;
    __builtin_amdgcn_wave_barrier();
    if (nn > 0 && lane < 8) nl[nn + lane] = nl[0];
    __builtin_amdgcn_wave_barrier();
    const float *zt = Z0 + lane * 4;
    float4 best = make_float4(0.f, 0.f, 0.f, 0.f);
    for (int i = 0; i < nn; i += 8) {
        float4 v[8];
#pragma unroll
        for (int k = 0; k < 8; ++k) v[k] = *reinterpret_cast<const float4 *>(zt + (size_t)nl[i + k] * 256);
#pragma unroll
        for (int k = 0; k < 8; ++k) { best.x = fmaxf(best.x, v[k].x); best.y = fmaxf(best.y, v[k].y); best.z = fmaxf(best.z, v[k].z); best.w = fmaxf(best.w, v[k].w); }
    }
    *reinterpret_cast<float4 *>(M0 + (size_t)q * 256 + lane * 4) = best;
    if (M0_16) {
        uint2 b16 = make_uint2(0u, 0u);
        for (int i = 0; i < nn; i += 8) {
            uint2 v[8];
#pragma unroll
            for (int k = 0; k < 8; ++k) v[k] = reinterpret_cast<const uint2 *>(Z0_16 + (size_t)nl[i + k] * 128)[lane];
#pragma unroll
            for (int k = 0; k < 8; ++k) { b16.x = pkmax_u16(b16.x, v[k].x); b16.y = pkmax_u16(b16.y, v[k].y); }
        }
        reinterpret_cast<uint2 *>(M0_16 + (size_t)q * 128)[lane] = b16;
    }
}

__device__ __forceinline__ int64_t xcd_contiguous(int64_t block, int64_t nblocks) {
    const int64_t q = nblocks / 8, rem = nblocks % 8, x = block % 8, i = block / 8;
    return (x < rem ? x * (q + 1) : rem * (q + 1) + (x - rem) * q) + i;
}

template <bool BF16> struct RowOps;
template <> struct RowOps<false> {
    typedef float4 V;
    static __device__ __forceinline__ V zero() { return make_float4(0.f, 0.f, 0.f, 0.f); }
    static __device__ __forceinline__ V load(const XobjChain &ch, bool m0, size_t row, int lane) {
        return reinterpret_cast<const float4 *>((m0 ? ch.M0 : ch.Z) + row * 256)[lane];
    }
    static __device__ __forceinline__ V vmax(V a, V b) { return make_float4(fmaxf(a.x, b.x), fmaxf(a.y, b.y), fmaxf(a.z, b.z), fmaxf(a.w, b.w)); }
    static __device__ __forceinline__ void store(const XobjParams &p, size_t row, int lane, V v) { reinterpret_cast<float4 *>(p.xobj + row * 256)[lane] = v; }
};
template <> struct RowOps<true> {
    typedef uint2 V;
    static __device__ __forceinline__ V zero() { return make_uint2(0u, 0u); }
    static __device__ __forceinline__ V load(const XobjChain &ch, bool m0, size_t row, int lane) {
        return reinterpret_cast<const uint2 *>((m0 ? ch.M0_16 : ch.Z16) + row * 128)[lane];
    }
    static __device__ __forceinline__ V vmax(V a, V b) { return make_uint2(pkmax_u16(a.x, b.x), pkmax_u16(a.y, b.y)); }
    static __device__ __forceinline__ void store(const XobjParams &p, size_t row, int lane, V v) { reinterpret_cast<uint2 *>(p.xobj16 + row * 128)[lane] = v; }
};

template <bool BF16>
__global__ __launch_bounds__(256) void xobj_fast_kernel(const XobjParams p) {
    typedef RowOps<BF16> R;
    const int lane = threadIdx.x & 63, wave = threadIdx.x >> 6;
    int64_t w = xcd_contiguous(blockIdx.x, gridDim.x) * 4 + wave;
    if (w >= p.total_rows) return;
    if (p.order) w = (w / p.R) * p.R + (p.order[w] & 0x3fffff);
    const int chain = (int)(w / p.R);
    const int64_t r = w - (int64_t)chain * p.R;
    const XobjChain ch = p.chains[chain];
    auto leave = [&]() {
        if (lane == 0) p.todo[atomicAdd(p.todo_count, 1)] = w;
    };
    if (!ch.M0 || !ch.fps2) { leave(); return; }
    const int *st = p.starts + (size_t)chain * 2 * p.R;
    const int s1 = __builtin_amdgcn_readfirstlane(st[2 * r]), s2 = __builtin_amdgcn_readfirstlane(st[2 * r + 1]);
    const int slot = ch.slot_of_start ? ch.slot_of_start[s1] : s1;
    const int q = __builtin_amdgcn_readfirstlane(ch.fps1[(size_t)s1 * 512 + s2]);
    if (ch.flags[q] != 0) { leave(); return; }
    const int cnt = __builtin_amdgcn_readfirstlane(ch.cnt2[q]);
    const int rowA = slot * ch.N + ch.cl2[(size_t)q * 128 + lane], rowB = slot * ch.N + ch.cl2[(size_t)q * 128 + 64 + lane];
    typename R::V best = R::load(ch, true, (size_t)q, lane);
    for (int i = 0; i < cnt; i += 8) {
        const int src = i < 64 ? rowA : rowB, j = i & 63;
        typename R::V v[8];
#pragma unroll
        for (int k = 0; k < 8; ++k) v[k] = R::load(ch, false, (size_t)__builtin_amdgcn_readlane(src, j + k), lane);
#pragma unroll
        for (int k = 0; k < 8; ++k) best = R::vmax(best, v[k]);
    }
    R::store(p, (size_t)w, lane, best);
}

template <bool BF16>
__device__ __forceinline__ void xobj_row(const XobjParams &p, int64_t w, float (*coords)[3][512], int (*centres)[128], int lane, int wave) {
    typedef RowOps<BF16> R;
    const int chain = (int)(w / p.R);
    const int64_t r = w - (int64_t)chain * p.R;
    const XobjChain ch = p.chains[chain];
    const int *st = p.starts + (size_t)chain * 2 * p.R;
    const int s1 = __builtin_amdgcn_readfirstlane(st[2 * r]), s2 = __builtin_amdgcn_readfirstlane(st[2 * r + 1]);
    const int slot = ch.slot_of_start ? ch.slot_of_start[s1] : s1;
    const int *perm = ch.fps1 + (size_t)s1 * 512;
    int idA, idB;
    const int q = __builtin_amdgcn_readfirstlane(perm[s2]);
    if (p.use_table && ch.fps2 && ch.flags[q] == 0) {
        if (ch.M0) {
            const int cnt = __builtin_amdgcn_readfirstlane(ch.cnt2[q]);
            const int rowA = slot * ch.N + ch.cl2[(size_t)q * 128 + lane], rowB = slot * ch.N + ch.cl2[(size_t)q * 128 + 64 + lane];
            typename R::V best = R::load(ch, true, (size_t)q, lane);
            for (int i = 0; i < cnt; i += 4) {
                const int src = i < 64 ? rowA : rowB, j = i & 63;
                const int c0 = __shfl(src, j), c1 = __shfl(src, j + 1), c2 = __shfl(src, j + 2), c3 = __shfl(src, j + 3);
                const typename R::V a = R::load(ch, false, (size_t)c0, lane), b = R::load(ch, false, (size_t)c1, lane);
                const typename R::V d = R::load(ch, false, (size_t)c2, lane), e = R::load(ch, false, (size_t)c3, lane);
                best = R::vmax(R::vmax(best, R::vmax(a, b)), R::vmax(d, e));
            }
            R::store(p, (size_t)w, lane, best);
            return;
        }
        idA = ch.fps2[(size_t)q * 128 + lane];
        idB = ch.fps2[(size_t)q * 128 + 64 + lane];
    } else {
        float *lx = coords[wave][0], *ly = coords[wave][1], *lz = coords[wave][2];
#pragma unroll
        for (int i = 0; i < 8; ++i) {
            const int j = lane + 64 * i, pid = perm[j];
            lx[j] = ch.xyz[3 * pid]; ly[j] = ch.xyz[3 * pid + 1]; lz[j] = ch.xyz[3 * pid + 2];
        }
        __builtin_amdgcn_wave_barrier();
        fps_wave<8, false>(lx, ly, lz, 512, s2, 128, centres[wave], lane);
        __builtin_amdgcn_wave_barrier();
        idA = perm[centres[wave][lane]];
        idB = perm[centres[wave][64 + lane]];
    }
    const int rowA = (ch.crowded[idA] ? slot * ch.N : 0) + idA, rowB = (ch.crowded[idB] ? slot * ch.N : 0) + idB;
    typename R::V best = R::zero();
#pragma unroll 4
    for (int i = 0; i < 64; i += 2) {
        const int c0 = __shfl(rowA, i), c1 = __shfl(rowA, i + 1), c2 = __shfl(rowB, i), c3 = __shfl(rowB, i + 1);
        const typename R::V a = R::load(ch, false, (size_t)c0, lane), b = R::load(ch, false, (size_t)c1, lane);
        const typename R::V d = R::load(ch, false, (size_t)c2, lane), e = R::load(ch, false, (size_t)c3, lane);
        best = R::vmax(R::vmax(best, R::vmax(a, b)), R::vmax(d, e));
    }
    R::store(p, (size_t)w, lane, best);
}

template <bool BF16>
__global__ __launch_bounds__(256) void xobj_kernel(const XobjParams p) {
    __shared__ float coords[4][3][512];
    __shared__ int centres[4][128];
    const int lane = threadIdx.x & 63, wave = threadIdx.x >> 6;
    if (p.skip_fast) {
        const int n = *p.todo_count;
        for (int i = blockIdx.x * 4 + wave; i < n; i += gridDim.x * 4) xobj_row<BF16>(p, p.todo[i], coords, centres, lane, wave);
        return;
    }
    int64_t w = xcd_contiguous(blockIdx.x, gridDim.x) * 4 + wave;
    if (w >= p.total_rows) return;
    if (p.order) w = (w / p.R) * p.R + (p.order[w] & 0x3fffff);
    xobj_row<BF16>(p, w, coords, centres, lane, wave);
}

template <class T> __device__ __forceinline__ __attribute__((address_space(1))) T *as_global(T *p) {
    return (__attribute__((address_space(1))) T *)p;
}

constexpr int XR_WAVES = 8;
constexpr int XR_PASS = 1024;
constexpr int XR_SLAB_BYTES = 64 * 1024;
constexpr int XR_LDS_BYTES = XR_SLAB_BYTES + XR_PASS * 10 + 16;

__global__ __launch_bounds__(256) void pcf_kernel(const int *__restrict__ fps1, const int *__restrict__ cnt2, const int *__restrict__ flags, int N,
                                                  int *__restrict__ pcf) {
    const int i = blockIdx.x * 256 + threadIdx.x;
    if (i >= N * 512) return;
    const int q = fps1[i];
    pcf[i] = q | (cnt2[q] << 10) | (flags[q] ? 1 << 18 : 0);
}

template <bool BF16, int LPR>
__device__ __forceinline__ void xobj_rows_body(const XobjParams &p, const XobjChain &ch, int chain, int s1, unsigned char *lds) {
    typedef uint32_t u4 __attribute__((ext_vector_type(4)));
    typedef const __attribute__((address_space(1))) u4 *gu4;
    constexpr int W = BF16 ? 128 : 256, F = 4 * LPR, RPW = 64 / LPR, NG = XR_WAVES * RPW, NT = 64 * XR_WAVES, RPT = XR_PASS / NT, NCHUNK = W / F;
    int *rid = reinterpret_cast<int *>(lds + XR_SLAB_BYTES);
    unsigned short *qs = reinterpret_cast<unsigned short *>(rid + XR_PASS);
    unsigned short *cfs = qs + XR_PASS, *lead = cfs + XR_PASS;
    int *nlead = reinterpret_cast<int *>(lead + XR_PASS);
    const int tid = threadIdx.x, lane = tid & 63, wave = tid >> 6;
    const int *goff = p.group_off + (size_t)chain * (ch.N + 1);
    const int g0 = goff[s1], gn = goff[s1 + 1] - g0;
    if (gn == 0) return;
    const auto *Zg = as_global((BF16 ? ch.Z16 : reinterpret_cast<const uint32_t *>(ch.Z)) + ((size_t)(ch.slot_of_start ? ch.slot_of_start[s1] : s1) * ch.N) * W);
    const auto *clist = as_global(ch.clist);
    const auto *ord = as_global(p.order + (size_t)chain * p.R + g0);
    const int sg = lane / LPR, fl = lane % LPR;
    const auto *M0 = as_global((BF16 ? ch.M0_16 : reinterpret_cast<const uint32_t *>(ch.M0)) + fl * 4);
    auto *out = as_global((BF16 ? p.xobj16 : reinterpret_cast<uint32_t *>(p.xobj)) + (size_t)chain * p.R * W + fl * 4);
    const unsigned char *mine = lds + fl * 16;
    const auto *pcf = as_global(ch.pcf + (size_t)s1 * 512);
    const gu4 lists = reinterpret_cast<gu4>(as_global(ch.cl2o)) + (LPR == 8 ? ((sg >> 1) & 1) * 16 : 0);
    const int pieces = ch.ncr * LPR;
    auto mx3 = [](u4 a, u4 b, u4 c) {
        u4 o;
        if (BF16) { o.x = pkmax_u16(pkmax_u16(a.x, b.x), c.x); o.y = pkmax_u16(pkmax_u16(a.y, b.y), c.y); o.z = pkmax_u16(pkmax_u16(a.z, b.z), c.z); o.w = pkmax_u16(pkmax_u16(a.w, b.w), c.w); }
        else { o.x = max(max(a.x, b.x), c.x); o.y = max(max(a.y, b.y), c.y); o.z = max(max(a.z, b.z), c.z); o.w = max(max(a.w, b.w), c.w); }
        return o;
    };
    for (int kb = 0; kb < gn; kb += XR_PASS) {
        const int np = min(XR_PASS, gn - kb);
        int o_v[RPT], op_v[RPT];
#pragma unroll
        for (int u = 0; u < RPT; ++u) {
            const int k = tid + NT * u;
            o_v[u] = 0; op_v[u] = -1;
            if (k < np) { o_v[u] = ord[kb + k]; if (k) op_v[u] = ord[kb + k - 1]; }
        }
        int n = 0;
        for (int chunk = 0; chunk < NCHUNK; ++chunk) {
            const int f0 = chunk * F;
            int ci[8];
#pragma unroll
            for (int k = 0; k < 8; ++k) {
                const int i = tid + NT * k;
                ci[k] = i < pieces ? clist[i / LPR] : 0;
            }
            int pc_v[RPT];
#pragma unroll
            for (int u = 0; u < RPT; ++u) pc_v[u] = chunk == 0 ? pcf[(unsigned)o_v[u] >> 22] : 0;
            u4 v[8];
#pragma unroll
            for (int k = 0; k < 8; ++k) {
                const int i = tid + NT * k;
                if (i < pieces) v[k] = *reinterpret_cast<gu4>(Zg + (size_t)ci[k] * W + f0 + (i % LPR) * 4);
            }
            __syncthreads();
            if (chunk == 0) {
                if (tid == 0) *nlead = 0;
#pragma unroll
                for (int u = 0; u < RPT; ++u) {
                    const int k = tid + NT * u;
                    if (k < np) {
                        const bool head = ((unsigned)o_v[u] >> 22) != ((unsigned)op_v[u] >> 22);
                        rid[k] = o_v[u] & 0x3fffff; qs[k] = (unsigned short)(pc_v[u] & 1023);
                        cfs[k] = (unsigned short)(((pc_v[u] >> 10) & 511) | (head ? 512 : 0));
                    }
                }
            }
#pragma unroll
            for (int k = 0; k < 8; ++k) {
                const int i = tid + NT * k;
                if (i < pieces) *reinterpret_cast<u4 *>(lds + (size_t)i * 16) = v[k];
            }
            __syncthreads();
            if (chunk == 0) {
#pragma unroll
                for (int u = 0; u < RPT; ++u) {
                    const int k = tid + NT * u;
                    if (k < np && (cfs[k] & 512)) lead[atomicAdd(nlead, 1)] = (unsigned short)k;
                }
                __syncthreads();
                n = *nlead;
            }
            int li = wave * RPW + sg;
            bool have = li < n;
            int kk = have ? lead[li] : 0;
            int q = qs[kk], cf = cfs[kk];
            u4 m0 = *reinterpret_cast<gu4>(M0 + (size_t)q * W + f0);
            u4 cur = lists[q * 32], nx1 = lists[q * 32 + 1];
            while (have) {
                const int li2 = li + NG;
                const bool have2 = li2 < n;
                const int kk2 = have2 ? lead[li2] : kk;
                const int q2 = qs[kk2], cf2 = cfs[kk2];
                const u4 m02 = *reinterpret_cast<gu4>(M0 + (size_t)q2 * W + f0);
                const u4 cur2 = lists[q2 * 32], nx12 = lists[q2 * 32 + 1];
                const int cnt = cf & 255, slow = cf & 256;
                u4 best = m0;
                if (!slow) {
                    const gu4 lp = lists + q * 32;
                    for (int j = 0; j < cnt; j += 8) {
                        u4 nx2 = nx1;
                        if (j + 16 < cnt) nx2 = lp[(j >> 3) + 2];
                        const u4 a0 = *reinterpret_cast<const u4 *>(mine + (cur.x & 0xffffu)), a1 = *reinterpret_cast<const u4 *>(mine + (cur.x >> 16));
                        const u4 a2 = *reinterpret_cast<const u4 *>(mine + (cur.y & 0xffffu)), a3 = *reinterpret_cast<const u4 *>(mine + (cur.y >> 16));
                        if (j + 4 < cnt) {
                            const u4 b0 = *reinterpret_cast<const u4 *>(mine + (cur.z & 0xffffu)), b1 = *reinterpret_cast<const u4 *>(mine + (cur.z >> 16));
                            const u4 b2 = *reinterpret_cast<const u4 *>(mine + (cur.w & 0xffffu)), b3 = *reinterpret_cast<const u4 *>(mine + (cur.w >> 16));
                            best = mx3(best, b0, b1); best = mx3(best, b2, b3);
                        }
                        best = mx3(best, a0, a1); best = mx3(best, a2, a3);
                        cur = nx1; nx1 = nx2;
                    }
                }
                int k2 = kk;
                do {
                    const int r = rid[k2];
                    if (!slow) *reinterpret_cast<__attribute__((address_space(1))) u4 *>(out + (size_t)r * W + f0) = best;
                    else if (chunk == 0 && fl == 0) p.todo[atomicAdd(p.todo_count, 1)] = (int)((int64_t)chain * p.R + r);
                    ++k2;
                } while (k2 < np && !(cfs[k2] & 512));
                li = li2; have = have2; kk = kk2; q = q2; cf = cf2; m0 = m02; cur = cur2; nx1 = nx12;
            }
        }
    }
}

template <bool BF16>
__global__ __launch_bounds__(64 * XR_WAVES, 4) void xobj_rows_kernel(const XobjParams p) {
    extern __shared__ unsigned char xr_lds[];
    const int N = p.group_N;
    const int chain = p.chain_of_rank[blockIdx.x / N], s1 = blockIdx.x % N;
    const XobjChain ch = p.chains[chain];
    switch (ch.lpr) {
        case 64: if (!BF16) xobj_rows_body<BF16, (BF16 ? 32 : 64)>(p, ch, chain, s1, xr_lds); break;
        case 32: xobj_rows_body<BF16, 32>(p, ch, chain, s1, xr_lds); break;
        case 16: xobj_rows_body<BF16, 16>(p, ch, chain, s1, xr_lds); break;
        default: xobj_rows_body<BF16, 8>(p, ch, chain, s1, xr_lds); break;
    }
}

int pn_pcf(const int *fps1, const int *cnt2, const int *flags, int N, int *pcf, hipStream_t s) {
    hipLaunchKernelGGL(pcf_kernel, dim3((unsigned)((N * 512 + 255) / 256)), dim3(256), 0, s, fps1, cnt2, flags, N, pcf);
    DGDM_HIP_CHECK(hipGetLastError());
    return DGDM_OK;
}

int pn_xobj_groups(const XobjParams &p, hipStream_t s) {
    if (p.total_items <= 0) return DGDM_OK;
    static bool attr_set = false;
    if (!attr_set) {
        DGDM_HIP_CHECK(hipFuncSetAttribute((const void *)xobj_rows_kernel<false>, hipFuncAttributeMaxDynamicSharedMemorySize, XR_LDS_BYTES));
        DGDM_HIP_CHECK(hipFuncSetAttribute((const void *)xobj_rows_kernel<true>, hipFuncAttributeMaxDynamicSharedMemorySize, XR_LDS_BYTES));
        attr_set = true;
    }
    DGDM_HIP_CHECK(hipMemsetAsync(p.todo_count, 0, sizeof(int), s));
    if (p.xobj16) hipLaunchKernelGGL(xobj_rows_kernel<true>, dim3((unsigned)p.total_items), dim3(64 * XR_WAVES), XR_LDS_BYTES, s, p);
    else hipLaunchKernelGGL(xobj_rows_kernel<false>, dim3((unsigned)p.total_items), dim3(64 * XR_WAVES), XR_LDS_BYTES, s, p);
    DGDM_HIP_CHECK(hipGetLastError());
    XobjParams q = p;
    q.skip_fast = 1;
    const int64_t cap = std::min<int64_t>(std::min<int64_t>(p.total_rows, p.todo_capacity), 8192);
    if (p.xobj16) hipLaunchKernelGGL(xobj_kernel<true>, dim3((unsigned)((cap + 3) / 4)), dim3(256), 0, s, q);
    else hipLaunchKernelGGL(xobj_kernel<false>, dim3((unsigned)((cap + 3) / 4)), dim3(256), 0, s, q);
    DGDM_HIP_CHECK(hipGetLastError());
    return DGDM_OK;
}

constexpr int XG_LDS_BYTES = 78 * 1024;

template <bool BF16, int LPR>
__device__ __forceinline__ void xtab_body(const XtabObj &o, int ncr, int s1, int chunk, uint32_t *slab) {
    typedef uint32_t u4 __attribute__((ext_vector_type(4)));
    constexpr int W = BF16 ? 128 : 256, F = 4 * LPR, RPW = 64 / LPR;
    const int lane = threadIdx.x & 63, wave = __builtin_amdgcn_readfirstlane(threadIdx.x >> 6);
    const int f0 = chunk * F, N = o.N;
    const uint32_t *Zs = (BF16 ? o.Z16 : reinterpret_cast<const uint32_t *>(o.Z)) + ((size_t)s1 * N) * W + f0;
    const int pieces = ncr * LPR;
    for (int i0 = threadIdx.x; i0 < pieces; i0 += 256 * 8) {
        u4 v[8];
#pragma unroll
        for (int k = 0; k < 8; ++k) {
            const int i = i0 + 256 * k;
            if (i < pieces) v[k] = *reinterpret_cast<const u4 *>(Zs + (size_t)o.clist[i / LPR] * W + (i % LPR) * 4);
        }
#pragma unroll
        for (int k = 0; k < 8; ++k) {
            const int i = i0 + 256 * k;
            if (i < pieces) *reinterpret_cast<u4 *>(slab + (size_t)i * 4) = v[k];
        }
    }
    __syncthreads();
    const int sg = lane / LPR, fl = lane % LPR;
    const uint32_t *M0 = (BF16 ? o.M0_16 : reinterpret_cast<const uint32_t *>(o.M0)) + f0 + fl * 4;
    uint32_t *out = (BF16 ? o.X16 : reinterpret_cast<uint32_t *>(o.X)) + ((size_t)s1 * N) * W + f0 + fl * 4;
    auto vmax4 = [](u4 a, u4 b) {
        u4 r;
        if (BF16) { r.x = pkmax_u16(a.x, b.x); r.y = pkmax_u16(a.y, b.y); r.z = pkmax_u16(a.z, b.z); r.w = pkmax_u16(a.w, b.w); }
        else {
            r.x = __float_as_uint(fmaxf(__uint_as_float(a.x), __uint_as_float(b.x))); r.y = __float_as_uint(fmaxf(__uint_as_float(a.y), __uint_as_float(b.y)));
            r.z = __float_as_uint(fmaxf(__uint_as_float(a.z), __uint_as_float(b.z))); r.w = __float_as_uint(fmaxf(__uint_as_float(a.w), __uint_as_float(b.w)));
        }
        return r;
    };
    for (int kb = 0; kb < N; kb += 256) {
        const int myq = kb + wave + 4 * lane;
        const int cnt_v = myq < N ? o.cnt2[myq] : 0;
        const int slow_v = myq < N ? o.flags[myq] : 1;
        const int nmine = min(64, (N - kb - wave + 3) / 4);
        for (int i0 = 0; i0 < nmine; i0 += 4) {
            int SA[4], SB[4];
            u4 m0[4];
#pragma unroll
            for (int u = 0; u < 4; ++u) {
                const int qn = kb + wave + 4 * min(i0 + u, nmine - 1);
                SA[u] = o.cl2s[(size_t)qn * 128 + lane]; SB[u] = o.cl2s[(size_t)qn * 128 + 64 + lane];
                m0[u] = *reinterpret_cast<const u4 *>(M0 + (size_t)qn * W);
            }
#pragma unroll
            for (int u = 0; u < 4; ++u) {
                const int i = i0 + u;
                if (i >= nmine) break;
                const int q = kb + wave + 4 * i;
                const int cnt = __builtin_amdgcn_readlane(cnt_v, i), slow = __builtin_amdgcn_readlane(slow_v, i);
                if (slow) continue;
                const int sa = SA[u], sb = SB[u];
                u4 best = m0[u];
                for (int j = 0; j < cnt; j += 4 * RPW) {
                    u4 v[4];
#pragma unroll
                    for (int e = 0; e < 4; ++e) {
                        const int jj = j + e * RPW;
                        int slot;
                        if (RPW == 1) slot = jj < 64 ? __builtin_amdgcn_readlane(sa, jj & 63) : __builtin_amdgcn_readlane(sb, jj & 63);
                        else slot = __shfl(jj < 64 ? sa : sb, (jj & 63) + sg);
                        v[e] = *reinterpret_cast<const u4 *>(slab + ((size_t)slot * LPR + fl) * 4);
                    }
#pragma unroll
                    for (int e = 0; e < 4; ++e) best = vmax4(best, v[e]);
                }
                if (RPW > 1 && cnt > 0) {
#pragma unroll
                    for (int x = 32; x >= LPR; x >>= 1) {
                        u4 t;
                        t.x = __shfl_xor(best.x, x); t.y = __shfl_xor(best.y, x); t.z = __shfl_xor(best.z, x); t.w = __shfl_xor(best.w, x);
                        best = vmax4(best, t);
                    }
                }
                if (sg == 0) *reinterpret_cast<u4 *>(out + (size_t)q * W) = best;
            }
        }
    }
}

template <bool BF16>
__global__ __launch_bounds__(256, 2) void xtab_kernel(const XtabObj o) {
    extern __shared__ uint32_t xt_slab[];
    constexpr int W = BF16 ? 128 : 256, MAXCH = W / 32;
    const int ncr = *o.ncr;
    if (ncr == 0) return;
    int lpr = W / 4;
    while (lpr > 8 && (size_t)ncr * lpr * 16 > (size_t)XG_LDS_BYTES) lpr >>= 1;
    const int nchunk = (W / 4) / lpr;
    const int s1 = blockIdx.x / MAXCH, chunk = blockIdx.x % MAXCH;
    if (chunk >= nchunk) return;
    switch (lpr) {
        case 64: if (!BF16) xtab_body<BF16, (BF16 ? 32 : 64)>(o, ncr, s1, chunk, xt_slab); break;
        case 32: xtab_body<BF16, 32>(o, ncr, s1, chunk, xt_slab); break;
        case 16: xtab_body<BF16, 16>(o, ncr, s1, chunk, xt_slab); break;
        default: xtab_body<BF16, 8>(o, ncr, s1, chunk, xt_slab); break;
    }
}

template <bool BF16>
__global__ __launch_bounds__(256) void xtab_slow_kernel(const XtabObj o) {
    typedef RowOps<BF16> R;
    __shared__ float coords[4][3][512];
    __shared__ int centres[4][128];
    const int lane = threadIdx.x & 63, wave = threadIdx.x >> 6, s1 = blockIdx.x, N = o.N;
    if (*o.ncr == 0) return;
    const int *perm = o.fps1 + (size_t)s1 * 512;
    XobjChain ch{};
    ch.Z = o.Z; ch.Z16 = o.Z16;
    int seen = 0;
    for (int q = 0; q < N; ++q) {
        if (o.flags[q] == 0) continue;
        if ((seen++ & 3) != wave) continue;
        int s2 = -1;
        for (int base = 0; base < 512 && s2 < 0; base += 64) {
            const unsigned long long m = __ballot(perm[base + lane] == q);
            if (m) s2 = base + __ffsll((long long)m) - 1;
        }
        if (s2 < 0) continue;
        float *lx = coords[wave][0], *ly = coords[wave][1], *lz = coords[wave][2];
#pragma unroll
        for (int i = 0; i < 8; ++i) {
            const int j = lane + 64 * i, pid = perm[j];
            lx[j] = o.xyz[3 * pid]; ly[j] = o.xyz[3 * pid + 1]; lz[j] = o.xyz[3 * pid + 2];
        }
        __builtin_amdgcn_wave_barrier();
        fps_wave<8, false>(lx, ly, lz, 512, s2, 128, centres[wave], lane);
        __builtin_amdgcn_wave_barrier();
        const int idA = perm[centres[wave][lane]], idB = perm[centres[wave][64 + lane]];
        const int rowA = (o.crowded[idA] ? s1 * N : 0) + idA, rowB = (o.crowded[idB] ? s1 * N : 0) + idB;
        typename R::V best = R::zero();
#pragma unroll 4
        for (int i = 0; i < 64; i += 2) {
            const int c0 = __shfl(rowA, i), c1 = __shfl(rowA, i + 1), c2 = __shfl(rowB, i), c3 = __shfl(rowB, i + 1);
            const typename R::V a = R::load(ch, false, (size_t)c0, lane), b = R::load(ch, false, (size_t)c1, lane);
            const typename R::V d = R::load(ch, false, (size_t)c2, lane), e = R::load(ch, false, (size_t)c3, lane);
            best = R::vmax(R::vmax(best, R::vmax(a, b)), R::vmax(d, e));
        }
        if (BF16) reinterpret_cast<uint2 *>(o.X16 + ((size_t)s1 * N + q) * 128)[lane] = *reinterpret_cast<uint2 *>(&best);
        else reinterpret_cast<float4 *>(o.X + ((size_t)s1 * N + q) * 256)[lane] = *reinterpret_cast<float4 *>(&best);
        __builtin_amdgcn_wave_barrier();
    }
}

int pn_xtab(const XtabObj &o, bool bf16, hipStream_t s) {
    static bool attr_set = false;
    if (!attr_set) {
        DGDM_HIP_CHECK(hipFuncSetAttribute((const void *)xtab_kernel<false>, hipFuncAttributeMaxDynamicSharedMemorySize, XG_LDS_BYTES));
        DGDM_HIP_CHECK(hipFuncSetAttribute((const void *)xtab_kernel<true>, hipFuncAttributeMaxDynamicSharedMemorySize, XG_LDS_BYTES));
        attr_set = true;
    }
    if (bf16) {
        hipLaunchKernelGGL(xtab_kernel<true>, dim3(o.N * 4), dim3(256), XG_LDS_BYTES, s, o);
        hipLaunchKernelGGL(xtab_slow_kernel<true>, dim3(o.N), dim3(256), 0, s, o);
    } else {
        hipLaunchKernelGGL(xtab_kernel<false>, dim3(o.N * 8), dim3(256), XG_LDS_BYTES, s, o);
        hipLaunchKernelGGL(xtab_slow_kernel<false>, dim3(o.N), dim3(256), 0, s, o);
    }
    DGDM_HIP_CHECK(hipGetLastError());
    return DGDM_OK;
}

__global__ __launch_bounds__(256) void xidx_kernel(const XidxChain *__restrict__ chains, const int *__restrict__ starts, int64_t R, int64_t total,
                                                   int *__restrict__ idx) {
    const int64_t w = (int64_t)blockIdx.x * 256 + threadIdx.x;
    if (w >= total) return;
    const int chain = (int)(w / R);
    const XidxChain ch = chains[chain];
    const int s1 = starts[2 * w], s2 = starts[2 * w + 1];
    const int q = ch.fps1[(size_t)s1 * 512 + s2];
    idx[w] = ch.m0_only ? q : s1 * ch.N + q;
}

int pn_xidx(const XidxChain *chains_dev, const int *starts, int64_t R, int nchain, int *idx, hipStream_t s) {
    const int64_t total = R * nchain;
    if (total <= 0) return DGDM_OK;
    hipLaunchKernelGGL(xidx_kernel, dim3((unsigned)((total + 255) / 256)), dim3(256), 0, s, chains_dev, starts, R, total, idx);
    DGDM_HIP_CHECK(hipGetLastError());
    return DGDM_OK;
}

__global__ __launch_bounds__(256) void fps_rows_kernel(const float *__restrict__ xyz , const int *__restrict__ start , int B, int N,
                                                       int npoint, int *__restrict__ out ) {
    extern __shared__ float lds[];
    const int wave = threadIdx.x >> 6, lane = threadIdx.x & 63;
    const int b = blockIdx.x * 4 + wave;
    float *lx = lds + (size_t)wave * 3 * N, *ly = lx + N, *lz = ly + N;
    if (b < B) {
        const float *c = xyz + (size_t)b * N * 3;
        for (int i = lane; i < N; i += 64) { lx[i] = c[3 * i]; ly[i] = c[3 * i + 1]; lz[i] = c[3 * i + 2]; }
    }
    __builtin_amdgcn_wave_barrier();
    if (b >= B) return;
    if (N <= 512) fps_wave<8, false>(lx, ly, lz, N, start[b], npoint, out + (size_t)b * npoint, lane);
    else fps_wave<16, false>(lx, ly, lz, N, start[b], npoint, out + (size_t)b * npoint, lane);
}

__global__ __launch_bounds__(256) void ball_rows_kernel(const float *__restrict__ xyz , const float *__restrict__ centres , int B,
                                                        int N, int S, float r2, int nsample, int *__restrict__ out ) {
    const int lane = threadIdx.x & 63;
    const int64_t g = (int64_t)blockIdx.x * 4 + (threadIdx.x >> 6);
    if (g >= (int64_t)B * S) return;
    const int b = (int)(g / S);
    const float *c = xyz + (size_t)b * N * 3;
    const float cx = centres[3 * g], cy = centres[3 * g + 1], cz = centres[3 * g + 2];
    const float cn = sq3(cx, cy, cz);
    int *dst = out + (size_t)g * nsample;
    int cnt = 0, first = N;
    for (int base = 0; base < N && cnt < nsample; base += 64) {
        const int k = base + lane;
        bool in = false;
        if (k < N) {
            const float x = c[3 * k], y = c[3 * k + 1], z = c[3 * k + 2];
            in = !(sqdist_expanded(cx, cy, cz, cn, x, y, z, sq3(x, y, z)) > r2);
        }
        const unsigned long long m = __ballot(in);
        if (m && first == N) first = base + __ffsll((long long)m) - 1;
        const int rank = cnt + __popcll(m & ((1ull << lane) - 1ull));
        if (in && rank < nsample) dst[rank] = k;
        cnt += __popcll(m);
    }
    cnt = min(cnt, nsample);
    for (int i = cnt + lane; i < nsample; i += 64) dst[i] = first;
}

__global__ void sqdist_rows_kernel(const float *__restrict__ src , const float *__restrict__ dst , int B, int S, int N,
                                   float *__restrict__ out ) {
    const int64_t i = (int64_t)blockIdx.x * blockDim.x + threadIdx.x;
    if (i >= (int64_t)B * S * N) return;
    const int n = (int)(i % N);
    const int64_t bs = i / N;
    const int b = (int)(bs / S);
    const float *a = src + 3 * bs, *p = dst + ((size_t)b * N + n) * 3;
    out[i] = sqdist_expanded(a[0], a[1], a[2], sq3(a[0], a[1], a[2]), p[0], p[1], p[2], sq3(p[0], p[1], p[2]));
}

__global__ void index_rows_kernel(const float *__restrict__ points , const int *__restrict__ idx , int B, int N, int M, int C,
                                  float *__restrict__ out ) {
    const int64_t i = (int64_t)blockIdx.x * blockDim.x + threadIdx.x;
    if (i >= (int64_t)B * M * C) return;
    const int c = (int)(i % C);
    const int64_t bm = i / C;
    const int b = (int)(bm / M);
    const int id = idx[bm];
    out[i] = (id >= 0 && id < N) ? points[((size_t)b * N + id) * C + c] : __builtin_nanf("");
}

int pn_fps_rows(const float *xyz, const int *start, int B, int N, int npoint, int *out, hipStream_t s) {
    hipLaunchKernelGGL(fps_rows_kernel, dim3((B + 3) / 4), dim3(256), (size_t)4 * 3 * N * sizeof(float), s, xyz, start, B, N, npoint, out);
    DGDM_HIP_CHECK(hipGetLastError());
    return DGDM_OK;
}
int pn_ball_rows(const float *xyz, const float *centres, int B, int N, int S, float r2, int nsample, int *out, hipStream_t s) {
    hipLaunchKernelGGL(ball_rows_kernel, dim3((unsigned)(((int64_t)B * S + 3) / 4)), dim3(256), 0, s, xyz, centres, B, N, S, r2, nsample, out);
    DGDM_HIP_CHECK(hipGetLastError());
    return DGDM_OK;
}
int pn_sqdist_rows(const float *src, const float *dst, int B, int S, int N, float *out, hipStream_t s) {
    const int64_t n = (int64_t)B * S * N;
    hipLaunchKernelGGL(sqdist_rows_kernel, dim3((unsigned)((n + 255) / 256)), dim3(256), 0, s, src, dst, B, S, N, out);
    DGDM_HIP_CHECK(hipGetLastError());
    return DGDM_OK;
}
int pn_index_rows(const float *points, const int *idx, int B, int N, int M, int C, float *out, hipStream_t s) {
    const int64_t n = (int64_t)B * M * C;
    hipLaunchKernelGGL(index_rows_kernel, dim3((unsigned)((n + 255) / 256)), dim3(256), 0, s, points, idx, B, N, M, C, out);
    DGDM_HIP_CHECK(hipGetLastError());
    return DGDM_OK;
}

int pn_fps_table(const float *xyz, int N, int nv, int npoint, int *out, int *flags, hipStream_t s, int nobj) {
    hipLaunchKernelGGL(fps_table_kernel, dim3((nv + 3) / 4, nobj), dim3(256), (size_t)3 * N * sizeof(float), s, xyz, N, nv, npoint, out, flags);
    DGDM_HIP_CHECK(hipGetLastError());
    return DGDM_OK;
}

int pn_sa1(const float *xyz, int N, const PnWeights &w, float *F1, hipStream_t s, int nobj) {
    hipLaunchKernelGGL(sa1_kernel, dim3(std::min(N, 1024), nobj), dim3(128), 0, s, xyz, N, w.r1sq, w.sa1_w0t, w.sa1_b0, w.sa1_w1, w.sa1_b1, F1);
    DGDM_HIP_CHECK(hipGetLastError());
    return DGDM_OK;
}

int pn_pairs(const float *xyz, int N, const float *U, const PnWeights &w, const int *pairs, const int *off, float *Y, uint32_t *Y16, hipStream_t s) {
    const int tiles = N * ((N + 31) / 32);
    hipLaunchKernelGGL(pair_kernel, dim3((tiles + 3) / 4), dim3(256), 0, s, xyz, N, U, w.sa2_vx, w.sa2_w1_img, w.sa2_b1, pairs, off, Y, Y16);
    DGDM_HIP_CHECK(hipGetLastError());
    return DGDM_OK;
}

int pn_crowd(const float *xyz, int N, const PnWeights &w, int *crowded, int *clist, int *ncr, int *off, int *pairs, short *rank, hipStream_t s,
             int *ncr_copy, int nobj) {
    hipLaunchKernelGGL(crowd_kernel, dim3(1, nobj), dim3(1024), 0, s, xyz, N, w.r2sq, crowded, clist, ncr, off, ncr_copy);
    hipLaunchKernelGGL(nbr_fill_kernel, dim3((N + 3) / 4, nobj), dim3(256), 0, s, xyz, N, w.r2sq, off, pairs, rank);
    DGDM_HIP_CHECK(hipGetLastError());
    return DGDM_OK;
}

int pn_l2c(int N, const int *fps1, int nv, const float *Y, float *L2, const int *clist, const int *ncr, const int *off, const short *rank, bool bf16,
           hipStream_t s) {
    static bool attr_set = false;
    const size_t lds = (size_t)(512 + 512 * 16 + 128) * 4 + L2C_YBYTES;
    if (!attr_set) {
        DGDM_HIP_CHECK(hipFuncSetAttribute((const void *)l2c_kernel<false>, hipFuncAttributeMaxDynamicSharedMemorySize, (int)lds));
        DGDM_HIP_CHECK(hipFuncSetAttribute((const void *)l2c_kernel<true>, hipFuncAttributeMaxDynamicSharedMemorySize, (int)lds));
        attr_set = true;
    }
    constexpr int split = 4, gx = 64;
    const dim3 grid(std::min(N, gx), std::min(split, std::max(nv - 1, 1)));
    if (bf16) hipLaunchKernelGGL(l2c_kernel<true>, grid, dim3(L2C_THREADS), lds, s, N, fps1, nv, reinterpret_cast<const uint32_t *>(Y),
                                 reinterpret_cast<uint32_t *>(L2), clist, ncr, off, rank);
    else hipLaunchKernelGGL(l2c_kernel<false>, grid, dim3(L2C_THREADS), lds, s, N, fps1, nv, reinterpret_cast<const uint32_t *>(Y),
                            reinterpret_cast<uint32_t *>(L2), clist, ncr, off, rank);
    DGDM_HIP_CHECK(hipGetLastError());
    return DGDM_OK;
}

int pn_l2(const float *xyz, int N, const PnWeights &w, const int *fps1, const int *vlist, int nv, const float *Y, float *L2,
          const int *clist, const int *ncr, const int *off, const short *rank, bool bf16, hipStream_t s, int crowded_mode) {
    const dim3 g0(1, (N + 3) / 4), g1((unsigned)(((nv - 1 + 3) / 4) * ((N + 7) / 8) * 8));
    if (crowded_mode == 1 && N <= 1024 && nv <= 512) {
        if (bf16) hipLaunchKernelGGL(l2_kernel<true>, g0, dim3(256), 0, s, xyz, N, w.r2sq, fps1, vlist, nv, Y, L2, 0, clist, ncr, off, rank);
        else hipLaunchKernelGGL(l2_kernel<false>, g0, dim3(256), 0, s, xyz, N, w.r2sq, fps1, vlist, nv, Y, L2, 0, clist, ncr, off, rank);
        DGDM_HIP_CHECK(hipGetLastError());
        return nv > 1 ? pn_l2c(N, fps1, nv, Y, L2, clist, ncr, off, rank, bf16, s) : DGDM_OK;
    }
    if (bf16) {
        hipLaunchKernelGGL(l2_kernel<true>, g0, dim3(256), 0, s, xyz, N, w.r2sq, fps1, vlist, nv, Y, L2, 0, clist, ncr, off, rank);
        if (nv > 1) hipLaunchKernelGGL(l2_kernel<true>, g1, dim3(256), 0, s, xyz, N, w.r2sq, fps1, vlist, nv, Y, L2, 1, clist, ncr, off, rank);
    } else {
        hipLaunchKernelGGL(l2_kernel<false>, g0, dim3(256), 0, s, xyz, N, w.r2sq, fps1, vlist, nv, Y, L2, 0, clist, ncr, off, rank);
        if (nv > 1) hipLaunchKernelGGL(l2_kernel<false>, g1, dim3(256), 0, s, xyz, N, w.r2sq, fps1, vlist, nv, Y, L2, 1, clist, ncr, off, rank);
    }
    DGDM_HIP_CHECK(hipGetLastError());
    return DGDM_OK;
}

int pn_z16(const float *xyz, int N, int nv, const PnWeights &w, const uint32_t *L2_16, float *Z, uint32_t *Z16, const int *clist, const int *ncr,
           hipStream_t s) {
    const int64_t t0 = (N + 63) / 64;
    hipLaunchKernelGGL(z16_kernel, dim3((unsigned)((t0 + 3) / 4)), dim3(256), 0, s, xyz, N, nv, L2_16, w.sa3_w_img16, w.sa3_wx, w.sa3_b, Z, Z16, 0, clist, ncr);
    if (nv > 1) {
        const int64_t t1 = ((int64_t)(nv - 1) * N + 63) / 64;
        hipLaunchKernelGGL(z16_kernel, dim3((unsigned)((t1 + 3) / 4)), dim3(256), 0, s, xyz, N, nv, L2_16, w.sa3_w_img16, w.sa3_wx, w.sa3_b, Z, Z16, 1, clist, ncr);
    }
    DGDM_HIP_CHECK(hipGetLastError());
    return DGDM_OK;
}

int pn_m0(const int *fps2, const int *crowded, int N, const float *Z0, float *M0, int *cl2, int *cnt2, const uint32_t *Z0_16, uint32_t *M0_16,
          const int *clist, const int *ncr, int *cl2s, unsigned short *cl2o, hipStream_t s) {
    hipLaunchKernelGGL(m0_kernel, dim3((N + 3) / 4), dim3(256), 0, s, fps2, crowded, N, Z0, M0, cl2, cnt2, Z0_16, M0_16, clist, ncr, cl2s, cl2o,
                       M0_16 ? 1 : 0);
    DGDM_HIP_CHECK(hipGetLastError());
    return DGDM_OK;
}

__global__ __launch_bounds__(64) void debug_ball1_kernel(const float *__restrict__ xyz, int N, float r2, int *__restrict__ out ) {
    __shared__ int nbr[32];
    const int p = blockIdx.x, lane = threadIdx.x;
    const float cx = xyz[3 * p], cy = xyz[3 * p + 1], cz = xyz[3 * p + 2];
    ball_first32(xyz, N, p, cx, cy, cz, sq3(cx, cy, cz), r2, nbr, lane);
    __builtin_amdgcn_wave_barrier();
    if (lane < 32) out[(size_t)p * 32 + lane] = nbr[lane];
}

__global__ __launch_bounds__(64) void debug_ball2_kernel(int N, const int *__restrict__ perm, int M, const int *__restrict__ off,
                                                         const int *__restrict__ pairs, const short *__restrict__ rank,
                                                         int *__restrict__ out , int *__restrict__ cnt_out ) {
    __shared__ int sel[64];
    __shared__ short rks[1024];
    const int c = blockIdx.x, lane = threadIdx.x;
    for (int i = lane; i < N; i += 64) rks[i] = rank[(size_t)c * N + i];
    __builtin_amdgcn_wave_barrier();
    const int cnt = l2_select(rks, perm, M, sel, lane);
    out[(size_t)c * 64 + lane] = lane < cnt ? (pairs[off[c] + sel[lane]] & 0xffff) : -1;
    if (lane == 0) cnt_out[c] = cnt;
}

int pn_debug_indices(const float *xyz, int N, const PnWeights &w, const int *perm, int M, int *ball1, int *ball2, int *ball2_cnt, int *crowded,
                     hipStream_t s) {
    DevBuf clist, off, pairs, rank;
    int rc;
    if ((rc = clist.alloc((size_t)(N + 1) * 4)) || (rc = off.alloc((size_t)(N + 1) * 4)) || (rc = pairs.alloc((size_t)N * N * 4)) ||
        (rc = rank.alloc((size_t)N * N * 2)))
        return rc;
    hipLaunchKernelGGL(debug_ball1_kernel, dim3(N), dim3(64), 0, s, xyz, N, w.r1sq, ball1);
    if ((rc = pn_crowd(xyz, N, w, crowded, clist.as<int>(), clist.as<int>() + N, off.as<int>(), pairs.as<int>(), rank.as<short>(), s))) return rc;
    hipLaunchKernelGGL(debug_ball2_kernel, dim3(N), dim3(64), 0, s, N, perm, M, off.as<int>(), pairs.as<int>(), rank.as<short>(), ball2, ball2_cnt);
    DGDM_HIP_CHECK(hipGetLastError());
    DGDM_HIP_CHECK(hipStreamSynchronize(s));
    return DGDM_OK;
}

template <bool BF16>
static int xobj_launch(XobjParams p, bool all_fast, hipStream_t s) {
    p.skip_fast = 0;
    if (p.use_table && p.todo) {
        DGDM_HIP_CHECK(hipMemsetAsync(p.todo_count, 0, sizeof(int), s));
        hipLaunchKernelGGL(xobj_fast_kernel<BF16>, dim3((unsigned)((p.total_rows + 3) / 4)), dim3(256), 0, s, p);
        DGDM_HIP_CHECK(hipGetLastError());
        if (all_fast) return DGDM_OK;
        p.skip_fast = 1;
        const int64_t cap = std::min<int64_t>(std::min<int64_t>(p.total_rows, p.todo_capacity), 65536);
        hipLaunchKernelGGL(xobj_kernel<BF16>, dim3((unsigned)((cap + 3) / 4)), dim3(256), 0, s, p);
        DGDM_HIP_CHECK(hipGetLastError());
        return DGDM_OK;
    }
    hipLaunchKernelGGL(xobj_kernel<BF16>, dim3((unsigned)((p.total_rows + 3) / 4)), dim3(256), 0, s, p);
    DGDM_HIP_CHECK(hipGetLastError());
    return DGDM_OK;
}

int pn_xobj(const XobjParams &p, bool all_fast, hipStream_t s) {
    if (p.total_rows <= 0) return DGDM_OK;
    return p.xobj16 ? xobj_launch<true>(p, all_fast, s) : xobj_launch<false>(p, all_fast, s);
}

}
```

dgdm_amd/csrc/pointnet64.hip:

```cpp
#include "common.h"
#include <algorithm>
#include <cstdlib>
#include "mfma_chain.h"
#include "pointnet.h"
#include "pointnet_dev.h"

#pragma clang fp contract(off)

namespace dgdm {

typedef double f64x4 __attribute__((ext_vector_type(4)));

template <int D>
__device__ __forceinline__ void ring64_fill(wrsrc_t rs, int voff, int base_off, float4 (&ring)[D]) {
#pragma unroll
    for (int i = 0; i < D; ++i) ring[i] = wload(rs, voff, base_off + i * 1024);
}

template <int TOTAL, int D, class Body>
__device__ __forceinline__ void ring64_stream(wrsrc_t rs, int voff, int base_off, float4 (&ring)[D], Body &&body) {
    static_assert(TOTAL % D == 0, "pass length must be a multiple of the ring depth");
#pragma unroll
    for (int i = 0; i < TOTAL; ++i) {
        const float4 a = ring[i % D];
        ring[i % D] = wload(rs, voff, base_off + (i + D) * 1024);
        body(i, a);
        __builtin_amdgcn_sched_barrier(0);
    }
}

constexpr int RING64 = 8;
constexpr int PN64_GRID = 1024;

template <int CTRL>
__device__ __forceinline__ double dpp_max64(double v) {
    const uint64_t b = __builtin_bit_cast(uint64_t, v);
    const uint32_t lo = (uint32_t)__builtin_amdgcn_update_dpp(0, (int)(uint32_t)b, CTRL, 0xf, 0xf, false);
    const uint32_t hi = (uint32_t)__builtin_amdgcn_update_dpp(0, (int)(uint32_t)(b >> 32), CTRL, 0xf, 0xf, false);
    return fmax(v, __builtin_bit_cast(double, ((uint64_t)hi << 32) | lo));
}

constexpr int SA1_LDS_BYTES = (128 * 64 + 128) * 8;
__global__ __launch_bounds__(256) void sa1_64_kernel(const float *xyz_all, int N, int nobj, float r2, const double *__restrict__ w0t ,
                                                     const double *__restrict__ b0, const double *__restrict__ w1 ,
                                                     const double *__restrict__ b1, double *F1_all ) {
    extern __shared__ __attribute__((aligned(16))) double sa1_w[];
    __shared__ int nbr_all[4][2][32];
    const int lane = threadIdx.x & 63, wave = __builtin_amdgcn_readfirstlane(threadIdx.x >> 6);
    for (int i = threadIdx.x; i < 128 * 64; i += 256) sa1_w[i] = w1[i];
    if (threadIdx.x < 128) sa1_w[128 * 64 + threadIdx.x] = b1[threadIdx.x];
    __syncthreads();
    int (*nbr)[32] = nbr_all[wave];
    const int half = lane >> 5, sl = lane & 31;
    const int ppo = (N + 1) / 2;
    for (int task = blockIdx.x * 4 + wave; task < nobj * ppo; task += gridDim.x * 4) {
        const int ob = task / ppo, pp = task - ob * ppo;
        const float *xyz = xyz_all + (size_t)ob * 3 * N;
        double *F1 = F1_all + (size_t)ob * N * 128;
        const int p0 = 2 * pp, p1 = min(2 * pp + 1, N - 1);
#pragma unroll
        for (int c = 0; c < 2; ++c) {
            const int pc = c ? p1 : p0;
            const float cx = xyz[3 * pc], cy = xyz[3 * pc + 1], cz = xyz[3 * pc + 2];
            ball_first32(xyz, N, pc, cx, cy, cz, sq3(cx, cy, cz), r2, nbr[c], lane);
        }
        __builtin_amdgcn_wave_barrier();
        const int p = half ? p1 : p0, k = nbr[half][sl];
        const double dx = (double)xyz[3 * k] - (double)xyz[3 * p], dy = (double)xyz[3 * k + 1] - (double)xyz[3 * p + 1],
                     dz = (double)xyz[3 * k + 2] - (double)xyz[3 * p + 2];
        double h[64];
#pragma unroll
        for (int c = 0; c < 64; ++c) h[c] = fmax(fma(w0t[128 + c], dz, fma(w0t[64 + c], dy, fma(w0t[c], dx, b0[c]))), 0.0);
        double res[4] = {0.0, 0.0, 0.0, 0.0};
#pragma nounroll
        for (int f = 0; f < 128; ++f) {
            const double *wf = sa1_w + f * 64;
            double acc = sa1_w[128 * 64 + f];
#pragma unroll
            for (int kk = 0; kk < 64; ++kk) acc = fma(wf[kk], h[kk], acc);
            acc = dpp_max64<0xB1>(acc); acc = dpp_max64<0x4E>(acc); acc = dpp_max64<0x141>(acc); acc = dpp_max64<0x140>(acc);
            acc = fmax(acc, __shfl_xor(acc, 16));
            acc = fmax(acc, 0.0);
            if (sl == (f & 31)) res[f >> 5] = acc;
        }
        if (half == 0 || 2 * pp + 1 < N) {
#pragma unroll
            for (int j = 0; j < 4; ++j) F1[(size_t)p * 128 + 32 * j + sl] = res[j];
        }
        __builtin_amdgcn_wave_barrier();
    }
}

__global__ __launch_bounds__(256, 2) void pair64_kernel(const float *__restrict__ xyz, int N, const double *__restrict__ U ,
                                                     const double *__restrict__ vx , const double *__restrict__ img,
                                                     const double *__restrict__ bias, const int *__restrict__ pairs,
                                                     const int *__restrict__ off , float *__restrict__ Y) {
    const int lane = threadIdx.x & 63, n = lane & 15, kq = lane >> 4;
    const int wave = __builtin_amdgcn_readfirstlane(threadIdx.x >> 6);
    const int total = off[N];
    struct D2 { double lo, hi; };
    const wrsrc_t rs = weight_rsrc(reinterpret_cast<const float4 *>(img), 256 * 1024);
    const double *v = vx + kq * 32;
#pragma nounroll
    for (int tile = blockIdx.x * 4 + wave; tile * 16 < total; tile += gridDim.x * 4) {
        asm volatile("" ::: "memory");
        const int p = min(tile * 16 + n, total - 1);
        const int ck = pairs[p], c = ck >> 16, k = ck & 0xffff;
        const double dx = (double)xyz[3 * k] - (double)xyz[3 * c], dy = (double)xyz[3 * k + 1] - (double)xyz[3 * c + 1],
                     dz = (double)xyz[3 * k + 2] - (double)xyz[3 * c + 2];
        const double *urow = U + (size_t)k * 128 + kq * 32;
        f64x4 acc[16];
#pragma unroll
        for (int mt = 0; mt < 16; ++mt) {
#pragma unroll
            for (int i = 0; i < 4; ++i) acc[mt][i] = bias[16 * mt + 4 * kq + i];
        }
        float4 ring[RING64];
        ring64_fill<RING64>(rs, lane * 16, 0, ring);
#pragma nounroll
        for (int ch = 0; ch < 2; ++ch) {
            double in[16];
#pragma unroll
            for (int j = 0; j < 16; ++j) {
                const int f = 16 * ch + j;
                in[j] = fmax(fma(v[256 + f], dz, fma(v[128 + f], dy, fma(v[f], dx, urow[f]))), 0.0);
            }
            ring64_stream<128, RING64>(rs, lane * 16, ch * 128 * 1024, ring, [&](int e, const float4 a) {
                const int ks = e / 8, mp = e % 8;
                const D2 w = __builtin_bit_cast(D2, a);
                const double b = in[ks];
                acc[2 * mp] = __builtin_amdgcn_mfma_f64_16x16x4f64(w.lo, b, acc[2 * mp], 0, 0, 0);
                acc[2 * mp + 1] = __builtin_amdgcn_mfma_f64_16x16x4f64(w.hi, b, acc[2 * mp + 1], 0, 0, 0);
            });
        }
        if (tile * 16 + n < total) {
            float *dst = Y + (size_t)p * 256 + 4 * kq;
#pragma unroll
            for (int mt = 0; mt < 16; ++mt)
                *reinterpret_cast<float4 *>(dst + 16 * mt) = make_float4(fmaxf((float)acc[mt][0], 0.f), fmaxf((float)acc[mt][1], 0.f),
                                                                          fmaxf((float)acc[mt][2], 0.f), fmaxf((float)acc[mt][3], 0.f));
        }
    }
}

__global__ __launch_bounds__(256, 2) void z64_kernel(const float *__restrict__ xyz, int N, int nv, const float *__restrict__ L2,
                                                  const double *__restrict__ img, const double *__restrict__ w3x ,
                                                  const double *__restrict__ bias, float *__restrict__ Z,
                                                  const int *__restrict__ clist, const int *__restrict__ ncr) {
    const int lane = threadIdx.x & 63, n = lane & 15, kq = lane >> 4;
    const int wave = __builtin_amdgcn_readfirstlane(threadIdx.x >> 6);
    const int ncrv = nv > 1 ? *ncr : 0;
    const int items = N + (nv - 1) * ncrv;
    struct D2 { double lo, hi; };
    const wrsrc_t rs = weight_rsrc(reinterpret_cast<const float4 *>(img), 512 * 1024);
#pragma nounroll
    for (int tile = blockIdx.x * 4 + wave; tile * 16 < items; tile += gridDim.x * 4) {
        asm volatile("" ::: "memory");
        const int item = min(tile * 16 + n, items - 1);
        const int j = item - N;
        const int c = j < 0 ? item : clist[j % ncrv];
        const int row = j < 0 ? c : (1 + j / ncrv) * N + c;
        const double x = xyz[3 * c], y = xyz[3 * c + 1], z = xyz[3 * c + 2];
        const float4 *src = reinterpret_cast<const float4 *>(L2 + (size_t)row * 256 + kq * 64);
        f64x4 acc[16];
#pragma unroll
        for (int mt = 0; mt < 16; ++mt) {
#pragma unroll
            for (int i = 0; i < 4; ++i) {
                const int f = 16 * mt + 4 * kq + i;
                acc[mt][i] = fma(w3x[512 + f], z, fma(w3x[256 + f], y, fma(w3x[f], x, bias[f])));
            }
        }
        float4 ring[RING64];
        ring64_fill<RING64>(rs, lane * 16, 0, ring);
        float4 cur[4], nxt[4];
#pragma unroll
        for (int j4 = 0; j4 < 4; ++j4) cur[j4] = src[j4];
#pragma nounroll
        for (int ch = 0; ch < 4; ++ch) {
            const int cn = min(ch + 1, 3);
#pragma unroll
            for (int j4 = 0; j4 < 4; ++j4) nxt[j4] = src[4 * cn + j4];
            float in[16];
#pragma unroll
            for (int j4 = 0; j4 < 4; ++j4) { in[4 * j4] = cur[j4].x; in[4 * j4 + 1] = cur[j4].y; in[4 * j4 + 2] = cur[j4].z; in[4 * j4 + 3] = cur[j4].w; }
            ring64_stream<128, RING64>(rs, lane * 16, ch * 128 * 1024, ring, [&](int e, const float4 a) {
                const int ks = e / 8, mp = e % 8;
                const D2 w = __builtin_bit_cast(D2, a);
                const double b = (double)in[ks];
                acc[2 * mp] = __builtin_amdgcn_mfma_f64_16x16x4f64(w.lo, b, acc[2 * mp], 0, 0, 0);
                acc[2 * mp + 1] = __builtin_amdgcn_mfma_f64_16x16x4f64(w.hi, b, acc[2 * mp + 1], 0, 0, 0);
            });
#pragma unroll
            for (int j4 = 0; j4 < 4; ++j4) cur[j4] = nxt[j4];
        }
        if (tile * 16 + n < items) {
            float *dst = Z + (size_t)row * 256 + 4 * kq;
#pragma unroll
            for (int mt = 0; mt < 16; ++mt)
                *reinterpret_cast<float4 *>(dst + 16 * mt) = make_float4(fmaxf((float)acc[mt][0], 0.f), fmaxf((float)acc[mt][1], 0.f),
                                                                          fmaxf((float)acc[mt][2], 0.f), fmaxf((float)acc[mt][3], 0.f));
        }
    }
}

int pn_sa1_64(const float *xyz, int N, float r1sq, const PnWeights64 &w, double *F1_64, hipStream_t s, int nobj) {
    static bool attr_set = false;
    if (!attr_set) {
        DGDM_HIP_CHECK(hipFuncSetAttribute((const void *)sa1_64_kernel, hipFuncAttributeMaxDynamicSharedMemorySize, SA1_LDS_BYTES));
        attr_set = true;
    }
    const int tasks = nobj * ((N + 1) / 2);
    hipLaunchKernelGGL(sa1_64_kernel, dim3(std::min((tasks + 3) / 4, 512)), dim3(256), SA1_LDS_BYTES, s, xyz, N, nobj, r1sq, w.sa1_w0t, w.sa1_b0, w.sa1_w1,
                       w.sa1_b1, F1_64);
    DGDM_HIP_CHECK(hipGetLastError());
    return DGDM_OK;
}

int pn_pairs64(const float *xyz, int N, const double *U64, const PnWeights64 &w, const int *pairs, const int *off, float *Y, hipStream_t s) {
    const int tiles = N * ((N + 15) / 16);
    hipLaunchKernelGGL(pair64_kernel, dim3(std::min((tiles + 3) / 4, PN64_GRID)), dim3(256), 0, s, xyz, N, U64, w.sa2_vx, w.sa2_w1_img, w.sa2_b1, pairs, off, Y);
    DGDM_HIP_CHECK(hipGetLastError());
    return DGDM_OK;
}

int pn_z64(const float *xyz, int N, int nv, const PnWeights64 &w, const float *L2, float *Z, const int *clist, const int *ncr, hipStream_t s) {
    const int64_t tiles = ((int64_t)nv * N + 15) / 16;
    hipLaunchKernelGGL(z64_kernel, dim3((unsigned)std::min<int64_t>((tiles + 3) / 4, PN64_GRID)), dim3(256), 0, s, xyz, N, nv, L2, w.sa3_w_img, w.sa3_wx,
                       w.sa3_b, Z, clist, ncr);
    DGDM_HIP_CHECK(hipGetLastError());
    return DGDM_OK;
}

}
```

Before: 18640 samples/s.

## Share crowded L2 selections, dedupe z64 work, fuse FPS tables, index M0 directly

Adds a selection kernel that finds crowded centres whose grouped L2 inputs repeat across viewpoints. The z64 pass then processes only the unique items, and a zfill kernel copies the results to the duplicate rows. FPS-512 and FPS-128 tables now come from one dual-output kernel instead of two kernels on separate streams. Chains with no crowded points read M0 tables directly through an index path instead of materialising xobj. This cuts redundant per-object table-building work at the cost of extra scratch buffers, a memset and more kernel launches.

Result: faster. 19380 samples/s (median of 6 runs) (+4.0%).

```diff
diff --git a/dgdm_amd/csrc/debug.hip b/dgdm_amd/csrc/debug.hip
--- a/dgdm_amd/csrc/debug.hip
+++ b/dgdm_amd/csrc/debug.hip
@@ -49,8 +49,7 @@
     DGDM_REQUIRE(N >= 128 && N <= 1024 && perm_len > 0 && perm_len <= N, DGDM_EINVAL, "dgdm_debug_pointnet_indices: N %d / perm_len %d unsupported", N, perm_len);
     hipStream_t s = (hipStream_t)stream;
     int rc;
-    if ((rc = pn_fps_table(xyz_dev, N, N, 512, fps512_dev, nullptr, s))) return rc;
-    if ((rc = pn_fps_table(xyz_dev, N, N, 128, fps128_dev, fps128_flags_dev, s))) return rc;
+    if ((rc = pn_fps_tables(xyz_dev, N, N, fps512_dev, fps128_dev, fps128_flags_dev, s))) return rc;
     return pn_debug_indices(xyz_dev, N, m->pn(), perm_dev, perm_len, ball1_dev, ball2_dev, ball2_count_dev, crowded_dev, s);
 }
 
diff --git a/dgdm_amd/csrc/guidance_api.hip b/dgdm_amd/csrc/guidance_api.hip
--- a/dgdm_amd/csrc/guidance_api.hip
+++ b/dgdm_amd/csrc/guidance_api.hip
@@ -61,8 +61,9 @@
     DevBuf pool_crowded, pool_clist, pool_off, pool_pairs, pool_rank, pool_F1, pool_U;
     DevBuf pool_xyz, pool_fps1, pool_fps2, pool_flags, pool_ncr;
     DevBuf tmpY[NBUILD], tmpL2[NBUILD], vlist;
-    hipStream_t bstream[NBUILD] = {}, fstream = nullptr;
-    hipEvent_t bev[NBUILD] = {}, bstart = nullptr, fstart = nullptr, fdone = nullptr, ldone = nullptr;
+    DevBuf tmpShare[NBUILD];
+    hipStream_t bstream[NBUILD] = {};
+    hipEvent_t bev[NBUILD] = {}, bstart = nullptr, pooled = nullptr, ldone = nullptr;
     DevBuf V, genc, atab, chainbias, timepart, ttmp, ttmp64, partial, objdev, objidx, xobj, xobj16, starts, order, xchains, todo, groupoff;
     DevBuf loopx[2], loopeps, loopgrad, loopxrep, loopts;
     DevBuf scorelogits;
@@ -96,9 +97,7 @@
         }
         if (bstart) (void)hipEventDestroy(bstart);
         if (ldone) (void)hipEventDestroy(ldone);
-        if (fstart) (void)hipEventDestroy(fstart);
-        if (fdone) (void)hipEventDestroy(fdone);
-        if (fstream) (void)hipStreamDestroy(fstream);
+        if (pooled) (void)hipEventDestroy(pooled);
     }
     int build_pose_table(const std::vector<float> &ori, const std::vector<float> &pos, PoseGrid *dst, hipStream_t s);
     void set_grid(dgdm::TrunkParams *p, const PoseGrid &g, int n_chains) const;
@@ -111,7 +110,7 @@
     int use_xtab(const int *objidx_host, int n_chains, int64_t rows, bool want16, hipStream_t s);
     int build_object(int oi, int slot, hipStream_t s);
     int build_xtab(int oi, hipStream_t s);
-    int run_xobj(const int *objidx_host, int n_chains, int64_t rows, bool want16, bool *used16, hipStream_t s);
+    int run_xobj(const int *objidx_host, int n_chains, int64_t rows, bool want16, bool *used16, bool *via_tab, hipStream_t s);
     struct Embedded {
         bool tab = false, used16 = false;
         int64_t rows_per_chain = 0;
@@ -289,11 +288,25 @@
     } else {
         const PnWeights64 w64 = m->pn64();
         if ((rc = pn_pairs64(xyz, N, reinterpret_cast<const double *>(U), w64, pairs, off, tY.as<float>(), s))) return rc;
+        const bool shared = !l2_gather_mode && N <= 512;
+        L2Share sh{};
+        if (shared) {
+            const size_t NN = (size_t)N * N;
+            if ((rc = tmpShare[slot].alloc(NN * 64 + NN + NN * sizeof(short) + NN * sizeof(int) + (2 * (size_t)N + 4) * sizeof(int)))) return rc;
+            char *b = static_cast<char *>(tmpShare[slot].p);
+            sh.sel = reinterpret_cast<unsigned char *>(b); b += NN * 64;
+            sh.items = reinterpret_cast<int *>(b); b += NN * sizeof(int);
+            sh.coff = reinterpret_cast<int *>(b); b += N * sizeof(int);
+            sh.ccnt = reinterpret_cast<int *>(b); b += N * sizeof(int);
+            sh.nitems = reinterpret_cast<int *>(b); b += 4 * sizeof(int);
+            sh.rep = reinterpret_cast<short *>(b); b += NN * sizeof(short);
+            sh.cnt = reinterpret_cast<unsigned char *>(b);
+        }
         if ((rc = pn_l2(xyz, N, w, t.fps1, vlist.as<int>(), N, tY.as<float>(), tL2.as<float>(), t.clist, t.clist + N,
-                        off, rank, false, s, l2_gather_mode ? 0 : 1))) return rc;
-        if ((rc = pn_z64(xyz, N, N, w64, tL2.as<float>(), t.Z.as<float>(), t.clist, t.clist + N, s))) return rc;
-    }
-    DGDM_HIP_CHECK(hipStreamWaitEvent(s, fdone, 0));
+                        off, rank, false, s, shared ? 1 : 0, shared ? &sh : nullptr))) return rc;
+        if ((rc = pn_z64(xyz, N, N, w64, tL2.as<float>(), t.Z.as<float>(), t.clist, t.clist + N, s, sh.items, sh.nitems))) return rc;
+        if (shared && N > 1 && (rc = pn_zfill(N, N, t.Z.as<float>(), t.clist, t.clist + N, sh.rep, s))) return rc;
+    }
     if ((rc = pn_m0(t.fps2, t.crowded, N, t.Z.as<float>(), t.M0.as<float>(), t.cl2.as<int>(), t.cnt2.as<int>(), z16,
                     bf16 ? t.M0_16.as<uint32_t>() : nullptr, t.clist, t.clist + N, t.cl2s.as<int>(), t.cl2o.as<unsigned short>(), s))) return rc;
     if ((rc = pn_pcf(t.fps1, t.cnt2.as<int>(), t.flags, N, t.pcf.as<int>(), s))) return rc;
@@ -352,17 +365,11 @@
             (rc = g->pool_pairs.alloc(no * N * N * sizeof(int))) || (rc = g->pool_rank.alloc(no * N * N * sizeof(short))) ||
             (rc = g->pool_F1.alloc(no * N * 128 * 8)) || (rc = g->pool_U.alloc(no * N * 128 * 8)))
             return rc;
-        if (!g->fstream) {
-            DGDM_HIP_CHECK(hipStreamCreateWithFlags(&g->fstream, hipStreamNonBlocking));
-            DGDM_HIP_CHECK(hipEventCreateWithFlags(&g->fstart, hipEventDisableTiming));
-            DGDM_HIP_CHECK(hipEventCreateWithFlags(&g->fdone, hipEventDisableTiming));
-        }
+        if (!g->pooled) DGDM_HIP_CHECK(hipEventCreateWithFlags(&g->pooled, hipEventDisableTiming));
         DGDM_HIP_CHECK(hipMemcpyAsync(g->pool_xyz.p, objects_dev, no * N * 3 * 4, hipMemcpyDeviceToDevice, s));
-        DGDM_HIP_CHECK(hipEventRecord(g->fstart, s));
-        DGDM_HIP_CHECK(hipStreamWaitEvent(g->fstream, g->fstart, 0));
-        if ((rc = pn_fps_table(g->pool_xyz.as<float>(), N, N, 128, g->pool_fps2.as<int>(), g->pool_flags.as<int>(), g->fstream, n_objects))) return rc;
-        DGDM_HIP_CHECK(hipEventRecord(g->fdone, g->fstream));
-        if ((rc = pn_fps_table(g->pool_xyz.as<float>(), N, N, 512, g->pool_fps1.as<int>(), nullptr, s, n_objects))) return rc;
+        DGDM_HIP_CHECK(hipEventRecord(g->pooled, s));
+        if ((rc = pn_fps_tables(g->pool_xyz.as<float>(), N, N, g->pool_fps1.as<int>(), g->pool_fps2.as<int>(), g->pool_flags.as<int>(), s, n_objects)))
+            return rc;
         for (int i = 0; i < n_objects; ++i) {
             ObjectTables &t = *g->tables[i];
             t.xyz = g->pool_xyz.as<float>() + (size_t)i * N * 3; t.fps1 = g->pool_fps1.as<int>() + (size_t)i * N * 512;
@@ -371,7 +378,7 @@
         }
         {
             hipStream_t ls = g->bstream[0];
-            DGDM_HIP_CHECK(hipStreamWaitEvent(ls, g->fstart, 0));
+            DGDM_HIP_CHECK(hipStreamWaitEvent(ls, g->pooled, 0));
             const PnWeights w = g->m->pn();
             if ((rc = pn_crowd(g->pool_xyz.as<float>(), N, w, g->pool_crowded.as<int>(), g->pool_clist.as<int>(), g->pool_clist.as<int>() + N,
                                g->pool_off.as<int>(), g->pool_pairs.as<int>(), g->pool_rank.as<short>(), ls, g->pool_ncr.as<int>(), n_objects)))
@@ -399,7 +406,6 @@
             DGDM_HIP_CHECK(hipEventRecord(g->bev[i], g->bstream[i]));
             DGDM_HIP_CHECK(hipStreamWaitEvent(s, g->bev[i], 0));
         }
-        DGDM_HIP_CHECK(hipStreamWaitEvent(s, g->fdone, 0));
         prof_end(s, DGDM_STAGE_TABLES, 0.0);
         const size_t need = no * N + no;
         if (need > g->ro_ints) {
@@ -549,7 +555,8 @@
     return pn_xidx(xidxchains.as<XidxChain>(), starts.as<int>(), rows, n_chains, xidx.as<int>(), s);
 }
 
-int DgdmGuidance::run_xobj(const int *objidx_host, int n_chains, int64_t rows, bool want16, bool *used16, hipStream_t s) {
+int DgdmGuidance::run_xobj(const int *objidx_host, int n_chains, int64_t rows, bool want16, bool *used16, bool *via_tab, hipStream_t s) {
+    *via_tab = false;
     std::vector<XobjChain> ch(n_chains);
     for (int i = 0; i < n_chains; ++i) {
         const ObjectTables &t = *tables[objidx_host[i]];
@@ -581,12 +588,28 @@
     }
     DGDM_HIP_CHECK(hipMemcpyAsync(xchains.p, ch.data(), sizeof(XobjChain) * n_chains, hipMemcpyHostToDevice, s));
     if (groups) {
-        xp.group_off = groupoff.as<int>(); xp.nchain = n_chains; xp.group_N = cfg.num_object_points; xp.total_items = n_chains * xp.group_N; xp.use_table = 1;
-        std::vector<int> rank(n_chains);
-        for (int i = 0; i < n_chains; ++i) rank[i] = i;
+        const bool by_index = tables_wanted() && (want16 || !bf16);
+        std::vector<int> rank;
+        std::vector<XidxChain> xc(n_chains);
+        std::vector<const void *> base(n_chains);
+        for (int i = 0; i < n_chains; ++i) {
+            const ObjectTables &t = *tables[objidx_host[i]];
+            const bool m0_only = by_index && t.ncr == 0 && t.fast_ok;
+            if (!m0_only) rank.push_back(i);
+            xc[i].fps1 = m0_only ? t.fps1 : nullptr; xc[i].N = cfg.num_object_points; xc[i].m0_only = 1;
+            base[i] = m0_only ? (want16 ? (const void *)t.M0_16.p : (const void *)t.M0.p)
+                              : (want16 ? (const void *)(xobj16.as<uint32_t>() + (size_t)i * rows * 128) : (const void *)(xobj.as<float>() + (size_t)i * rows * 256));
+        }
+        xp.group_off = groupoff.as<int>(); xp.nchain = n_chains; xp.group_N = cfg.num_object_points; xp.use_table = 1;
+        xp.total_items = (int)rank.size() * xp.group_N;
         std::stable_sort(rank.begin(), rank.end(), [&](int a, int b) { return ch[a].ncr > ch[b].ncr; });
-        for (int i = 0; i < n_chains; ++i) xp.chain_of_rank[i] = (unsigned char)rank[i];
-        return pn_xobj_groups(xp, s);
+        for (size_t i = 0; i < rank.size(); ++i) xp.chain_of_rank[i] = (unsigned char)rank[i];
+        int rc = pn_xobj_groups(xp, s);
+        if (rc || !by_index) return rc;
+        *via_tab = true;
+        DGDM_HIP_CHECK(hipMemcpyAsync(xidxchains.p, xc.data(), sizeof(XidxChain) * n_chains, hipMemcpyHostToDevice, s));
+        DGDM_HIP_CHECK(hipMemcpyAsync(xtabptrs.p, base.data(), sizeof(void *) * n_chains, hipMemcpyHostToDevice, s));
+        return pn_xidx(xidxchains.as<XidxChain>(), starts.as<int>(), rows, n_chains, xidx.as<int>(), s);
     }
     return pn_xobj(xp, all_fast, s);
 }
@@ -600,7 +623,7 @@
     if ((rc = upload_starts(starts_host, n_chains, rows_per_call, s, !tab, n_calls, call_stride))) return rc;
     if ((rc = finish_objects())) return rc;
     e->tab = tab; e->used16 = want16; e->rows_per_chain = rt;
-    if ((rc = tab ? use_xtab(oidx, n_chains, rt, want16, s) : run_xobj(oidx, n_chains, rt, want16, &e->used16, s))) return rc;
+    if ((rc = tab ? use_xtab(oidx, n_chains, rt, want16, s) : run_xobj(oidx, n_chains, rt, want16, &e->used16, &e->tab, s))) return rc;
     DGDM_HIP_CHECK(hipEventRecord(up_consumed, s));
     consumed_recorded = true;
     return DGDM_OK;
diff --git a/dgdm_amd/csrc/pointnet.h b/dgdm_amd/csrc/pointnet.h
--- a/dgdm_amd/csrc/pointnet.h
+++ b/dgdm_amd/csrc/pointnet.h
@@ -82,19 +82,30 @@
 int pn_sqdist_rows(const float *src, const float *dst, int B, int S, int N, float *out, hipStream_t s);
 int pn_index_rows(const float *points, const int *idx, int B, int N, int M, int C, float *out, hipStream_t s);
 
+struct L2Share {
+    unsigned char *sel;
+    unsigned char *cnt;
+    short *rep;
+    int   *items;
+    int   *coff, *ccnt;
+    int   *nitems;
+};
 int pn_fps_table(const float *xyz, int N, int nv, int npoint, int *out, int *flags, hipStream_t s, int nobj = 1);
+int pn_fps_tables(const float *xyz, int N, int nv, int *fps1, int *fps2, int *flags, hipStream_t s, int nobj = 1);
 int pn_sa1(const float *xyz, int N, const PnWeights &w, float *F1, hipStream_t s, int nobj = 1);
 int pn_crowd(const float *xyz, int N, const PnWeights &w, int *crowded, int *clist, int *ncr, int *off, int *pairs, short *rank, hipStream_t s,
              int *ncr_copy = nullptr, int nobj = 1);
 int pn_pairs(const float *xyz, int N, const float *U, const PnWeights &w, const int *pairs, const int *off, float *Y, uint32_t *Y16, hipStream_t s);
 int pn_l2(const float *xyz, int N, const PnWeights &w, const int *fps1, const int *vlist, int nv, const float *Y, float *L2,
           const int *clist, const int *ncr, const int *off, const short *rank, bool bf16 , hipStream_t s,
-          int crowded_mode = 0);
+          int crowded_mode = 0, const L2Share *share = nullptr);
 int pn_z16(const float *xyz, int N, int nv, const PnWeights &w, const uint32_t *L2_16, float *Z, uint32_t *Z16, const int *clist, const int *ncr,
            hipStream_t s);
 int pn_sa1_64(const float *xyz, int N, float r1sq, const PnWeights64 &w, double *F1_64, hipStream_t s, int nobj = 1);
 int pn_pairs64(const float *xyz, int N, const double *U64, const PnWeights64 &w, const int *pairs, const int *off, float *Y, hipStream_t s);
-int pn_z64(const float *xyz, int N, int nv, const PnWeights64 &w, const float *L2, float *Z, const int *clist, const int *ncr, hipStream_t s);
+int pn_z64(const float *xyz, int N, int nv, const PnWeights64 &w, const float *L2, float *Z, const int *clist, const int *ncr, hipStream_t s,
+           const int *items = nullptr, const int *nitems = nullptr);
+int pn_zfill(int N, int nv, float *Z, const int *clist, const int *ncr, const short *rep, hipStream_t s);
 int pn_m0(const int *fps2, const int *crowded, int N, const float *Z0, float *M0, int *cl2, int *cnt2, const uint32_t *Z0_16, uint32_t *M0_16,
           const int *clist, const int *ncr, int *cl2s, unsigned short *cl2o, hipStream_t s);
 __host__ __device__ inline int xobj_rows_lpr(int ncr, bool bf16) {
diff --git a/dgdm_amd/csrc/pointnet.hip b/dgdm_amd/csrc/pointnet.hip
--- a/dgdm_amd/csrc/pointnet.hip
+++ b/dgdm_amd/csrc/pointnet.hip
@@ -31,8 +31,9 @@
     v = m;
 }
 
-template <int PPL, bool TIES>
-__device__ bool fps_wave(const float *lx, const float *ly, const float *lz, int M, int start, int npoint, int *out, int lane) {
+template <int PPL, bool TIES, bool DUAL = false>
+__device__ bool fps_wave(const float *lx, const float *ly, const float *lz, int M, int start, int npoint, int *out, int lane,
+                         int *out2 = nullptr, int npoint2 = 0) {
     float px[PPL], py[PPL], pz[PPL], dist[PPL];
 #pragma unroll
     for (int i = 0; i < PPL; ++i) {
@@ -44,7 +45,10 @@
     int far = start;
     bool ambiguous = false;
     for (int it = 0; it < npoint; ++it) {
-        if (lane == 0) out[it] = far;
+        if (lane == 0) {
+            out[it] = far;
+            if (DUAL && it < npoint2) out2[it] = far;
+        }
         const float cx = lx[far], cy = ly[far], cz = lz[far];
         float bv = -2.f;
         int bi = 0;
@@ -56,7 +60,7 @@
         }
         wave_argmax(bv, bi);
         far = bi;
-        if (TIES && it + 1 < npoint) {
+        if (TIES && it + 1 < (DUAL ? npoint2 : npoint)) {
             const float wx = lx[far], wy = ly[far], wz = lz[far];
             bool t = bv == 0.f;
 #pragma unroll
@@ -68,18 +72,23 @@
 }
 
 __global__ __launch_bounds__(256) void fps_table_kernel(const float *__restrict__ xyz, int N, int nv, int npoint, int *__restrict__ out,
-                                                        int *__restrict__ flags) {
+                                                        int *__restrict__ flags, int *__restrict__ out2, int npoint2) {
     extern __shared__ float lds[];
     float *lx = lds, *ly = lds + N, *lz = lds + 2 * N;
     xyz += (size_t)blockIdx.y * N * 3;
     out += (size_t)blockIdx.y * nv * npoint;
     if (flags) flags += (size_t)blockIdx.y * nv;
+    if (out2) out2 += (size_t)blockIdx.y * nv * npoint2;
     for (int i = threadIdx.x; i < N; i += blockDim.x) { lx[i] = xyz[3 * i]; ly[i] = xyz[3 * i + 1]; lz[i] = xyz[3 * i + 2]; }
     __syncthreads();
     const int v = blockIdx.x * 4 + (threadIdx.x >> 6), lane = threadIdx.x & 63;
     if (v >= nv) return;
     bool amb;
-    if (flags) {
+    if (out2) {
+        amb = N <= 512 ? fps_wave<8, true, true>(lx, ly, lz, N, v, npoint, out + (size_t)v * npoint, lane, out2 + (size_t)v * npoint2, npoint2)
+                       : fps_wave<16, true, true>(lx, ly, lz, N, v, npoint, out + (size_t)v * npoint, lane, out2 + (size_t)v * npoint2, npoint2);
+        if (lane == 0) flags[v] = amb ? 1 : 0;
+    } else if (flags) {
         amb = N <= 512 ? fps_wave<8, true>(lx, ly, lz, N, v, npoint, out + (size_t)v * npoint, lane)
                        : fps_wave<16, true>(lx, ly, lz, N, v, npoint, out + (size_t)v * npoint, lane);
         if (lane == 0) flags[v] = amb ? 1 : 0;
@@ -374,10 +383,113 @@
     if (sg == 0) *reinterpret_cast<u4 *>(dst + fl * 4) = best;
 }
 
-template <bool BF16>
-__device__ __forceinline__ void l2c_centre(int c, int N, const int *__restrict__ fps1 , int nv, const uint32_t *__restrict__ Y,
+constexpr int L2S_THREADS = 1024;
+__global__ __launch_bounds__(L2S_THREADS) void l2sel_kernel(int N, const int *__restrict__ fps1 , int nv, const int *__restrict__ clist,
+                                                            const int *__restrict__ ncr, const int *__restrict__ off,
+                                                            const short *__restrict__ rank, const L2Share sh) {
+    __shared__ short rks[1024];
+    __shared__ uint32_t mask[512][8];
+    __shared__ uint32_t hash[512];
+    __shared__ int selw[L2S_THREADS / 64][64];
+    __shared__ int wsum[L2S_THREADS / 64], base_s;
+    const int tid = threadIdx.x, lane = tid & 63, wave = tid >> 6, nwave = L2S_THREADS / 64;
+    const int n = *ncr;
+    for (int ci = blockIdx.x; ci < n; ci += gridDim.x) {
+        const int c = clist[ci];
+        const int K = off[c + 1] - off[c];
+        short *repg = sh.rep + (size_t)ci * nv;
+        if (K > 255) {
+            for (int v = tid; v < nv; v += L2S_THREADS) repg[v] = (short)v;
+            if (tid == 0) {
+                base_s = atomicAdd(sh.nitems, nv - 1);
+                sh.coff[ci] = base_s; sh.ccnt[ci] = nv - 1;
+            }
+            __syncthreads();
+            for (int v = 1 + tid; v < nv; v += L2S_THREADS) sh.items[base_s + v - 1] = (ci << 16) | v;
+            __syncthreads();
+            continue;
+        }
+        for (int i = tid; i < N; i += L2S_THREADS) rks[i] = rank[(size_t)c * N + i];
+        __syncthreads();
+        int pv[8], pn[8];
+#pragma unroll
+        for (int i = 0; i < 8; ++i) pn[i] = wave < nv ? fps1[(size_t)wave * 512 + 64 * i + lane] : 0;
+        for (int v = wave; v < nv; v += nwave) {
+#pragma unroll
+            for (int i = 0; i < 8; ++i) pv[i] = pn[i];
+            const int vn = v + nwave;
+            if (vn < nv) {
+#pragma unroll
+                for (int i = 0; i < 8; ++i) pn[i] = fps1[(size_t)vn * 512 + 64 * i + lane];
+            }
+            if (lane < 8) mask[v][lane] = 0u;
+            int cnt = 0;
+#pragma unroll
+            for (int i = 0; i < 8; ++i) {
+                if (cnt >= 64) break;
+                const int r = rks[pv[i]];
+                const bool in = r >= 0;
+                const unsigned long long m = __ballot(in);
+                const int pos = cnt + __popcll(m & ((1ull << lane) - 1ull));
+                if (in && pos < 64) selw[wave][pos] = r;
+                cnt += __popcll(m);
+            }
+            cnt = min(cnt, 64);
+            __builtin_amdgcn_wave_barrier();
+            const int r = selw[wave][lane < cnt ? lane : max(cnt - 1, 0)] & 255;
+            if (lane < cnt) atomicOr(&mask[v][r >> 5], 1u << (r & 31));
+            sh.sel[((size_t)ci * nv + v) * 64 + lane] = (unsigned char)r;
+            if (lane == 0) sh.cnt[(size_t)ci * nv + v] = (unsigned char)cnt;
+            __builtin_amdgcn_wave_barrier();
+        }
+        __syncthreads();
+        uint32_t mine[8];
+        const int v = tid;
+        if (v < nv) {
+            uint32_t h = 0x811c9dc5u;
+#pragma unroll
+            for (int i = 0; i < 8; ++i) { mine[i] = mask[v][i]; h = (h ^ mine[i]) * 0x01000193u; }
+            hash[v] = h;
+        }
+        __syncthreads();
+        bool isrep = false;
+        if (v < nv) {
+            const uint32_t hv = hash[v];
+            int rep = v;
+            for (int u = 0; u < v; ++u) {
+                if (hash[u] == hv && rep == v) {
+                    bool eq = true;
+#pragma unroll
+                    for (int i = 0; i < 8; ++i) eq = eq && mask[u][i] == mine[i];
+                    if (eq) rep = u;
+                }
+            }
+            repg[v] = (short)rep;
+            isrep = rep == v && v >= 1;
+        }
+        const unsigned long long m = __ballot(isrep);
+        if (lane == 0) wsum[wave] = __popcll(m);
+        __syncthreads();
+        if (tid == 0) {
+            int tot = 0;
+            for (int w = 0; w < nwave; ++w) tot += wsum[w];
+            base_s = atomicAdd(sh.nitems, tot);
+            sh.coff[ci] = base_s; sh.ccnt[ci] = tot;
+        }
+        __syncthreads();
+        if (isrep) {
+            int pre = 0;
+            for (int w = 0; w < wave; ++w) pre += wsum[w];
+            sh.items[base_s + pre + __popcll(m & ((1ull << lane) - 1ull))] = (ci << 16) | v;
+        }
+        __syncthreads();
+    }
+}
+
+template <bool BF16, bool REPS>
+__device__ __forceinline__ void l2c_centre(int c, int ci, int N, const int *__restrict__ fps1 , int nv, const uint32_t *__restrict__ Y,
                                            uint32_t *__restrict__ L2 , const int *__restrict__ off, const short *__restrict__ rank,
-                                           int (*selw)[64]) {
+                                           int (*selw)[64], const L2Share &sh) {
     constexpr int W = BF16 ? 128 : 256;
     extern __shared__ uint32_t l2c_lds[];
     short *rks = reinterpret_cast<short *>(l2c_lds);
@@ -386,12 +498,23 @@
     uint32_t *ych = l2c_lds + 512 + 512 * 16 + 128;
     const int K = off[c + 1] - off[c];
     const int lane = threadIdx.x & 63, wave = threadIdx.x >> 6, nwave = L2C_THREADS / 64;
-    const int vlo = 1 + (int)(((int64_t)(nv - 1) * blockIdx.y) / gridDim.y), vhi = 1 + (int)(((int64_t)(nv - 1) * (blockIdx.y + 1)) / gridDim.y);
+    const int *vl = nullptr;
+    int vlo, vhi;
+    if (REPS) {
+        const int nrep = sh.ccnt[ci];
+        vl = sh.items + sh.coff[ci];
+        vlo = (int)(((int64_t)nrep * blockIdx.y) / gridDim.y); vhi = (int)(((int64_t)nrep * (blockIdx.y + 1)) / gridDim.y);
+        if (vhi <= vlo) return;
+    } else {
+        vlo = 1 + (int)(((int64_t)(nv - 1) * blockIdx.y) / gridDim.y); vhi = 1 + (int)(((int64_t)(nv - 1) * (blockIdx.y + 1)) / gridDim.y);
+    }
+    auto variant = [&](int k) { return REPS ? (vl[k] & 0xffff) : k; };
     for (int i = threadIdx.x; i < N; i += L2C_THREADS) rks[i] = rank[(size_t)c * N + i];
     __syncthreads();
     if (K > 255) {
         constexpr int D = W / 64;
-        for (int v = vlo + wave; v < vhi; v += nwave) {
+        for (int k = vlo + wave; k < vhi; k += nwave) {
+            const int v = variant(k);
             const int cnt = l2_select(rks, fps1 + (size_t)v * 512, 512, selw[wave], lane);
             uint32_t best[D];
 #pragma unroll
@@ -409,7 +532,13 @@
         }
         return;
     }
-    {
+    if (REPS) {
+        for (int i = threadIdx.x; i < (vhi - vlo) * 16; i += L2C_THREADS) {
+            const int v = variant(vlo + i / 16), part = i % 16;
+            reinterpret_cast<uint32_t *>(sel)[v * 16 + part] = reinterpret_cast<const uint32_t *>(sh.sel)[((size_t)ci * nv + v) * 16 + part];
+        }
+        for (int k = vlo + threadIdx.x; k < vhi; k += L2C_THREADS) { const int v = variant(k); cnts[v] = sh.cnt[(size_t)ci * nv + v]; }
+    } else {
         int pv[8], pn[8];
         const int v0 = vlo + wave;
 #pragma unroll
@@ -449,7 +578,8 @@
         for (int i = threadIdx.x; i < pieces; i += L2C_THREADS)
             *reinterpret_cast<uint4 *>(ych + (size_t)i * 4) = *reinterpret_cast<const uint4 *>(Yc + (size_t)(i / lpr) * W + f0 + (i % lpr) * 4);
         __syncthreads();
-        for (int v = vlo + wave; v < vhi; v += nwave) {
+        for (int k = vlo + wave; k < vhi; k += nwave) {
+            const int v = variant(k);
             uint32_t *dst = L2 + ((size_t)v * N + c) * W + f0;
             const unsigned char *sv = sel + (size_t)v * 64;
             const int cnt = cnts[v];
@@ -463,15 +593,15 @@
     }
 }
 
-template <bool BF16>
+template <bool BF16, bool REPS>
 __global__ __launch_bounds__(L2C_THREADS, 1) void l2c_kernel(int N, const int *__restrict__ fps1 , int nv, const uint32_t *__restrict__ Y,
                                                              uint32_t *__restrict__ L2 , const int *__restrict__ clist,
                                                              const int *__restrict__ ncr, const int *__restrict__ off,
-                                                             const short *__restrict__ rank) {
+                                                             const short *__restrict__ rank, const L2Share sh) {
     __shared__ int selw[L2C_THREADS / 64][64];
     const int n = *ncr;
     for (int ci = blockIdx.x; ci < n; ci += gridDim.x) {
-        l2c_centre<BF16>(clist[ci], N, fps1, nv, Y, L2, off, rank, selw);
+        l2c_centre<BF16, REPS>(clist[ci], ci, N, fps1, nv, Y, L2, off, rank, selw, sh);
         __syncthreads();
     }
 }
@@ -1117,6 +1247,7 @@
     if (w >= total) return;
     const int chain = (int)(w / R);
     const XidxChain ch = chains[chain];
+    if (!ch.fps1) { idx[w] = (int)(w - (int64_t)chain * R); return; }
     const int s1 = starts[2 * w], s2 = starts[2 * w + 1];
     const int q = ch.fps1[(size_t)s1 * 512 + s2];
     idx[w] = ch.m0_only ? q : s1 * ch.N + q;
@@ -1220,7 +1351,14 @@
 }
 
 int pn_fps_table(const float *xyz, int N, int nv, int npoint, int *out, int *flags, hipStream_t s, int nobj) {
-    hipLaunchKernelGGL(fps_table_kernel, dim3((nv + 3) / 4, nobj), dim3(256), (size_t)3 * N * sizeof(float), s, xyz, N, nv, npoint, out, flags);
+    hipLaunchKernelGGL(fps_table_kernel, dim3((nv + 3) / 4, nobj), dim3(256), (size_t)3 * N * sizeof(float), s, xyz, N, nv, npoint, out, flags,
+                       (int *)nullptr, 0);
+    DGDM_HIP_CHECK(hipGetLastError());
+    return DGDM_OK;
+}
+
+int pn_fps_tables(const float *xyz, int N, int nv, int *fps1, int *fps2, int *flags, hipStream_t s, int nobj) {
+    hipLaunchKernelGGL(fps_table_kernel, dim3((nv + 3) / 4, nobj), dim3(256), (size_t)3 * N * sizeof(float), s, xyz, N, nv, 512, fps1, flags, fps2, 128);
     DGDM_HIP_CHECK(hipGetLastError());
     return DGDM_OK;
 }
@@ -1247,32 +1385,56 @@
 }
 
 int pn_l2c(int N, const int *fps1, int nv, const float *Y, float *L2, const int *clist, const int *ncr, const int *off, const short *rank, bool bf16,
-           hipStream_t s) {
+           hipStream_t s, const L2Share *share) {
     static bool attr_set = false;
     const size_t lds = (size_t)(512 + 512 * 16 + 128) * 4 + L2C_YBYTES;
     if (!attr_set) {
-        DGDM_HIP_CHECK(hipFuncSetAttribute((const void *)l2c_kernel<false>, hipFuncAttributeMaxDynamicSharedMemorySize, (int)lds));
-        DGDM_HIP_CHECK(hipFuncSetAttribute((const void *)l2c_kernel<true>, hipFuncAttributeMaxDynamicSharedMemorySize, (int)lds));
+        DGDM_HIP_CHECK(hipFuncSetAttribute((const void *)l2c_kernel<false, true>, hipFuncAttributeMaxDynamicSharedMemorySize, (int)lds));
+        DGDM_HIP_CHECK(hipFuncSetAttribute((const void *)l2c_kernel<true, false>, hipFuncAttributeMaxDynamicSharedMemorySize, (int)lds));
         attr_set = true;
     }
+    DGDM_REQUIRE(bf16 || share, DGDM_EINVAL, "pn_l2: the float32 crowded mode needs the selection stage's buffers");
     constexpr int split = 4, gx = 64;
     const dim3 grid(std::min(N, gx), std::min(split, std::max(nv - 1, 1)));
-    if (bf16) hipLaunchKernelGGL(l2c_kernel<true>, grid, dim3(L2C_THREADS), lds, s, N, fps1, nv, reinterpret_cast<const uint32_t *>(Y),
-                                 reinterpret_cast<uint32_t *>(L2), clist, ncr, off, rank);
-    else hipLaunchKernelGGL(l2c_kernel<false>, grid, dim3(L2C_THREADS), lds, s, N, fps1, nv, reinterpret_cast<const uint32_t *>(Y),
-                            reinterpret_cast<uint32_t *>(L2), clist, ncr, off, rank);
+    if (bf16) {
+        hipLaunchKernelGGL((l2c_kernel<true, false>), grid, dim3(L2C_THREADS), lds, s, N, fps1, nv, reinterpret_cast<const uint32_t *>(Y),
+                           reinterpret_cast<uint32_t *>(L2), clist, ncr, off, rank, L2Share{});
+    } else {
+        DGDM_HIP_CHECK(hipMemsetAsync(share->nitems, 0, sizeof(int), s));
+        hipLaunchKernelGGL(l2sel_kernel, dim3(std::min(N, 512)), dim3(L2S_THREADS), 0, s, N, fps1, nv, clist, ncr, off, rank, *share);
+        hipLaunchKernelGGL((l2c_kernel<false, true>), grid, dim3(L2C_THREADS), lds, s, N, fps1, nv, reinterpret_cast<const uint32_t *>(Y),
+                           reinterpret_cast<uint32_t *>(L2), clist, ncr, off, rank, *share);
+    }
+    DGDM_HIP_CHECK(hipGetLastError());
+    return DGDM_OK;
+}
+
+__global__ __launch_bounds__(256) void zfill_kernel(int N, int nv, float *__restrict__ Z, const int *__restrict__ clist, const int *__restrict__ ncr,
+                                                    const short *__restrict__ rep) {
+    const int lane = threadIdx.x & 63, wave = threadIdx.x >> 6;
+    const int64_t total = (int64_t)*ncr * nv;
+    for (int64_t w = (int64_t)blockIdx.x * 4 + wave; w < total; w += (int64_t)gridDim.x * 4) {
+        const int v = (int)(w % nv), r = rep[w];
+        if (r == v) continue;
+        const int c = clist[w / nv];
+        reinterpret_cast<float4 *>(Z + ((size_t)v * N + c) * 256)[lane] = reinterpret_cast<const float4 *>(Z + ((size_t)r * N + c) * 256)[lane];
+    }
+}
+
+int pn_zfill(int N, int nv, float *Z, const int *clist, const int *ncr, const short *rep, hipStream_t s) {
+    hipLaunchKernelGGL(zfill_kernel, dim3(2048), dim3(256), 0, s, N, nv, Z, clist, ncr, rep);
     DGDM_HIP_CHECK(hipGetLastError());
     return DGDM_OK;
 }
 
 int pn_l2(const float *xyz, int N, const PnWeights &w, const int *fps1, const int *vlist, int nv, const float *Y, float *L2,
-          const int *clist, const int *ncr, const int *off, const short *rank, bool bf16, hipStream_t s, int crowded_mode) {
+          const int *clist, const int *ncr, const int *off, const short *rank, bool bf16, hipStream_t s, int crowded_mode, const L2Share *share) {
     const dim3 g0(1, (N + 3) / 4), g1((unsigned)(((nv - 1 + 3) / 4) * ((N + 7) / 8) * 8));
     if (crowded_mode == 1 && N <= 1024 && nv <= 512) {
         if (bf16) hipLaunchKernelGGL(l2_kernel<true>, g0, dim3(256), 0, s, xyz, N, w.r2sq, fps1, vlist, nv, Y, L2, 0, clist, ncr, off, rank);
         else hipLaunchKernelGGL(l2_kernel<false>, g0, dim3(256), 0, s, xyz, N, w.r2sq, fps1, vlist, nv, Y, L2, 0, clist, ncr, off, rank);
         DGDM_HIP_CHECK(hipGetLastError());
-        return nv > 1 ? pn_l2c(N, fps1, nv, Y, L2, clist, ncr, off, rank, bf16, s) : DGDM_OK;
+        return nv > 1 ? pn_l2c(N, fps1, nv, Y, L2, clist, ncr, off, rank, bf16, s, share) : DGDM_OK;
     }
     if (bf16) {
         hipLaunchKernelGGL(l2_kernel<true>, g0, dim3(256), 0, s, xyz, N, w.r2sq, fps1, vlist, nv, Y, L2, 0, clist, ncr, off, rank);
diff --git a/dgdm_amd/csrc/pointnet64.hip b/dgdm_amd/csrc/pointnet64.hip
--- a/dgdm_amd/csrc/pointnet64.hip
+++ b/dgdm_amd/csrc/pointnet64.hip
@@ -146,11 +146,12 @@
 __global__ __launch_bounds__(256, 2) void z64_kernel(const float *__restrict__ xyz, int N, int nv, const float *__restrict__ L2,
                                                   const double *__restrict__ img, const double *__restrict__ w3x ,
                                                   const double *__restrict__ bias, float *__restrict__ Z,
-                                                  const int *__restrict__ clist, const int *__restrict__ ncr) {
+                                                  const int *__restrict__ clist, const int *__restrict__ ncr,
+                                                  const int *__restrict__ list, const int *__restrict__ nlist) {
     const int lane = threadIdx.x & 63, n = lane & 15, kq = lane >> 4;
     const int wave = __builtin_amdgcn_readfirstlane(threadIdx.x >> 6);
     const int ncrv = nv > 1 ? *ncr : 0;
-    const int items = N + (nv - 1) * ncrv;
+    const int items = N + (list ? (nv > 1 ? *nlist : 0) : (nv - 1) * ncrv);
     struct D2 { double lo, hi; };
     const wrsrc_t rs = weight_rsrc(reinterpret_cast<const float4 *>(img), 512 * 1024);
 #pragma nounroll
@@ -158,8 +159,9 @@
         asm volatile("" ::: "memory");
         const int item = min(tile * 16 + n, items - 1);
         const int j = item - N;
-        const int c = j < 0 ? item : clist[j % ncrv];
-        const int row = j < 0 ? c : (1 + j / ncrv) * N + c;
+        const int pk = (j >= 0 && list) ? list[j] : 0;
+        const int c = j < 0 ? item : clist[list ? pk >> 16 : j % ncrv];
+        const int row = j < 0 ? c : (list ? (pk & 0xffff) : 1 + j / ncrv) * N + c;
         const double x = xyz[3 * c], y = xyz[3 * c + 1], z = xyz[3 * c + 2];
         const float4 *src = reinterpret_cast<const float4 *>(L2 + (size_t)row * 256 + kq * 64);
         f64x4 acc[16];
@@ -224,10 +226,11 @@
     return DGDM_OK;
 }
 
-int pn_z64(const float *xyz, int N, int nv, const PnWeights64 &w, const float *L2, float *Z, const int *clist, const int *ncr, hipStream_t s) {
+int pn_z64(const float *xyz, int N, int nv, const PnWeights64 &w, const float *L2, float *Z, const int *clist, const int *ncr, hipStream_t s,
+           const int *items, const int *nitems) {
     const int64_t tiles = ((int64_t)nv * N + 15) / 16;
     hipLaunchKernelGGL(z64_kernel, dim3((unsigned)std::min<int64_t>((tiles + 3) / 4, PN64_GRID)), dim3(256), 0, s, xyz, N, nv, L2, w.sa3_w_img, w.sa3_wx,
-                       w.sa3_b, Z, clist, ncr);
+                       w.sa3_b, Z, clist, ncr, items, nitems);
     DGDM_HIP_CHECK(hipGetLastError());
     return DGDM_OK;
 }
```
